# Alexander-H-Liu/End-to-end-ASR-Pytorch

Measured on AMD Instinct MI355X. Metric: audio frames/sec training (LAS+CTC, LibriSpeech 80-mel), higher is better.
Workload: dtype f32; 1 GPU; cfg3: {"B": 32, "T": 1600, "D": 80, "V": 5000, "L": 64}; global_batch=32, parallelism=dp1

## Files before the change

### end-to-end-asr-pytorch_amd/_lib.py

```python
import ctypes
import os

_HERE = os.path.dirname(os.path.abspath(__file__))
LIB_PATH = os.path.join(_HERE, "csrc", "libasrk.so")

c_int, c_i64, c_f32, c_vp, c_sz = (ctypes.c_int, ctypes.c_int64, ctypes.c_float, ctypes.c_void_p,
                                   ctypes.c_size_t)
c_f64 = ctypes.c_double

SIGNATURES = {
    "asrk_version": (c_int, []),
    "asrk_strerror": (ctypes.c_char_p, [c_int]),
    "asrk_init": (c_int, [c_int]),
    "asrk_profile_enable": (None, [c_int]),
    "asrk_profile_families": (None, [ctypes.c_uint]),
    "asrk_profile_reset": (None, []),
    "asrk_profile_get": (c_int, [c_int, ctypes.POINTER(ctypes.c_double), ctypes.POINTER(c_i64)]),
    "asrk_profile_get_work": (c_int, [c_int, ctypes.POINTER(ctypes.c_double)]),
    "asrk_gemm_f32": (c_int, [c_int, c_int, c_int, c_int, c_int, c_f32, c_vp, c_int, c_vp, c_int,
                              c_f32, c_vp, c_int, c_vp, c_vp, c_int, c_int, c_vp, c_sz, c_vp]),
    "asrk_gemm_ws_bytes": (c_sz, [c_int, c_int, c_int, c_int]),
    "asrk_gemm_takes_split": (c_int, [c_int, c_int, c_int, c_int]),
    "asrk_split_panel_bytes": (ctypes.c_size_t, [c_int, c_int, c_int]),
    "asrk_split_panel_f32": (c_int, [c_vp, c_int, c_int, c_int, c_int, c_vp, c_int, c_vp]),
    "asrk_gemm_panels_f32": (c_int, [c_int, c_int, c_int, c_f32, c_vp, c_int, c_int, c_int, c_int,
                                     c_vp, c_int, c_int, c_int, c_int, c_f32, c_vp, c_int, c_vp, c_vp, c_int, c_vp]),
    "asrk_copy3d_f32": (c_int, [c_vp, c_vp, c_int, c_int, c_int, c_i64, c_i64, c_i64, c_i64, c_int,
                                c_vp]),
    "asrk_colsum_f32": (c_int, [c_vp, c_int, c_int, c_int, c_vp, c_int, c_vp]),
    "asrk_tanh_fwd_f32": (c_int, [c_vp, c_vp, c_i64, c_vp]),
    "asrk_tanh_bwd_f32": (c_int, [c_vp, c_vp, c_vp, c_i64, c_vp]),
    "asrk_log_softmax_fwd_f32": (c_int, [c_vp, c_vp, c_int, c_int, c_int, c_vp]),
    "asrk_log_softmax_bwd_f32": (c_int, [c_vp, c_vp, c_vp, c_int, c_int, c_int, c_vp]),
    "asrk_cross_entropy_fwd_f32": (c_int, [c_vp, c_int, c_int, c_int, c_vp, c_int, c_vp, c_vp, c_vp]),
    "asrk_cross_entropy_bwd_f32": (c_int, [c_vp, c_int, c_int, c_int, c_vp, c_int, c_vp, c_vp, c_vp,
                                           c_vp]),
    "asrk_ctc_prefix_score_f32": (c_int, [c_vp, c_vp, c_vp, c_vp, c_vp, c_vp, c_vp, c_int, c_int, c_int,
                                          c_int, c_int, c_int, c_f32, c_vp]),
    "asrk_ctc_prefix_score_multi_f32": (c_int, [c_vp, c_vp, c_vp, c_vp, c_vp, c_vp, c_vp, c_vp, c_vp, c_int, c_int,
                                                c_int, c_int, c_int, c_int, c_int, c_f32, c_vp]),
    "asrk_ctc_prefix_beam_ws_bytes": (c_sz, [c_int, c_int]),
    "asrk_ctc_prefix_beam_ws_offsets": (c_int, [c_int, c_int, c_int] + [ctypes.POINTER(c_i64)] * 6),
    "asrk_ctc_prefix_beam_f32": (c_int, [c_vp, c_int, c_int, c_vp, c_int, c_int, c_vp, c_f32, c_int, c_int, c_int,
                                         c_int, c_int, c_vp, c_sz, c_vp]),
    "asrk_fbank_frames_f32": (c_int, [c_vp, c_i64, c_vp, c_vp, c_int, c_int, c_int, c_int, c_f32, c_int,
                                      c_vp]),
    "asrk_power_spectrum_f32": (c_int, [c_vp, c_vp, c_i64, c_int, c_vp]),
    "asrk_log_floor_f32": (c_int, [c_vp, c_i64, c_f32, c_vp]),
    "asrk_delta_f32": (c_int, [c_vp, c_vp, c_vp, c_int, c_int, c_int, c_int, c_vp]),
    "asrk_cmvn_f32": (c_int, [c_vp, c_vp, c_int, c_int, c_f32, c_vp]),
    "asrk_transpose_f32": (c_int, [c_vp, c_vp, c_int, c_int, c_vp]),
    "asrk_fbank_frames_batch_f32": (c_int, [c_vp, c_int, c_i64, c_vp, c_vp, c_int, c_int, c_vp, c_vp, c_int, c_int,
                                            c_int, c_f32, c_f32, c_int, c_vp]),
    "asrk_delta_cmvn_batch_f32": (c_int, [c_vp, c_vp, c_int, c_int, c_vp, c_int, c_int, c_int, c_f32, c_vp, c_int,
                                          c_vp]),
    "asrk_fbank_logmel_batch_f32": (c_int, [c_vp, c_int, c_i64, c_vp, c_vp, c_int, c_int, c_vp, c_vp, c_vp, c_vp, c_vp,
                                            c_int, c_int, c_vp, c_int, c_int, c_int, c_f32, c_f32, c_int, c_f32, c_vp]),
    "asrk_lstm_ws_bytes": (c_sz, []),
    "asrk_lstm_xchg_bytes": (c_sz, [c_int, c_int, c_int, c_int, c_int, c_int]),
    "asrk_lstm_plan_workgroups": (c_int, [c_int, c_int, c_int, c_int, c_int, c_int]),
    "asrk_lstm_rec_fwd_f32": (c_int, [c_vp, c_vp, c_vp, c_vp, c_vp, c_int, c_int, c_int, c_int,
                                      c_vp, c_int, c_vp, c_int, c_vp]),
    "asrk_lstm_rec_bwd_f32": (c_int, [c_vp, c_vp, c_vp, c_vp, c_vp, c_int, c_int, c_int, c_int,
                                      c_vp, c_int, c_vp, c_vp, c_int, c_vp]),
    "asrk_lstm_rec_fwd_pyr_f32": (c_int, [c_vp, c_vp, c_vp, c_vp, c_vp, c_int, c_int, c_int, c_int,
                                          c_vp, c_int, c_vp, c_vp, c_int, c_int, c_int, c_vp]),
    "asrk_lstm_rec_fwd_len_f32": (c_int, [c_vp, c_vp, c_vp, c_vp, c_vp, c_vp, c_int, c_int, c_int, c_int,
                                          c_vp, c_int, c_vp, c_vp, c_int, c_int, c_int, c_vp]),
    "asrk_lstm_rec_bwd_pyr_f32": (c_int, [c_vp, c_vp, c_vp, c_vp, c_vp, c_int, c_int, c_int, c_int,
                                          c_vp, c_int, c_vp, c_vp, c_int, c_int, c_int, c_vp]),
    "asrk_lstm_plan_is_bf": (c_int, [c_int, c_int, c_int, c_int, c_int, c_int]),
    "asrk_lstm_rec_fwd_pyr_panel_f32": (c_int, [c_vp, c_vp, c_vp, c_vp, c_vp, c_int, c_int, c_int, c_int,
                                                c_vp, c_int, c_vp, c_vp, c_int, c_int, c_vp, c_int, c_vp]),
    "asrk_lstm_rec_bwd_pyr_panel_f32": (c_int, [c_vp, c_vp, c_vp, c_vp, c_vp, c_int, c_int, c_int, c_int,
                                                c_vp, c_int, c_vp, c_vp, c_int, c_int, c_vp, c_vp, c_int, c_vp]),
    "asrk_gru_rec_fwd_f32": (c_int, [c_vp, c_vp, c_vp, c_vp, c_int, c_int, c_int, c_int,
                                     c_vp, c_int, c_vp, c_vp, c_int, c_int, c_int, c_vp]),
    "asrk_gru_rec_bwd_f32": (c_int, [c_vp, c_vp, c_vp, c_vp, c_vp, c_int, c_int, c_int, c_int,
                                     c_vp, c_int, c_vp, c_vp, c_int, c_int, c_int, c_vp]),
    "asrk_lstm_check_error": (c_int, [c_vp, c_vp]),
    "asrk_loc_conv_fwd_f32": (c_int, [c_vp, c_vp, c_vp, c_int, c_int, c_int, c_int, c_int, c_vp]),
    "asrk_loc_conv_bwd_f32": (c_int, [c_vp, c_vp, c_vp, c_vp, c_vp, c_int, c_int, c_int, c_int, c_int,
                                      c_vp]),
    "asrk_attn_energy_fwd_f32": (c_int, [c_int, c_vp, c_vp, c_vp, c_vp, c_vp, c_vp, c_vp, c_vp, c_vp,
                                         c_int, c_int, c_int, c_int, c_int, c_f32, c_vp]),
    "asrk_attn_energy_bwd_f32": (c_int, [c_int, c_vp, c_vp, c_vp, c_vp, c_vp, c_vp, c_vp, c_vp, c_vp,
                                         c_vp, c_vp, c_vp, c_vp, c_vp, c_int, c_int, c_int, c_int,
                                         c_int, c_f32, c_vp]),
    "asrk_attn_context_fwd_f32": (c_int, [c_vp, c_vp, c_vp, c_int, c_int, c_int, c_i64, c_vp]),
    "asrk_attn_context_bwd_f32": (c_int, [c_vp, c_vp, c_vp, c_int, c_int, c_int, c_i64, c_vp]),
    "asrk_lstm_cell_fwd_f32": (c_int, [c_vp, c_vp, c_vp, c_vp, c_int, c_int, c_vp]),
    "asrk_lstm_cell_bwd_f32": (c_int, [c_vp, c_vp, c_vp, c_vp, c_vp, c_vp, c_int, c_int, c_vp]),
    "asrk_gru_cell_fwd_f32": (c_int, [c_vp, c_vp, c_i64, c_i64, c_vp, c_i64, c_vp, c_i64, c_int, c_int, c_vp]),
    "asrk_gru_cell_bwd_f32": (c_int, [c_vp, c_vp, c_i64, c_i64, c_vp, c_i64, c_vp, c_i64, c_vp, c_vp, c_i64,
                                      c_int, c_int, c_vp]),
    "asrk_embedding_fwd_f32": (c_int, [c_vp, c_vp, c_vp, c_i64, c_int, c_int, c_vp]),
    "asrk_embedding_bwd_f32": (c_int, [c_vp, c_vp, c_vp, c_i64, c_int, c_int, c_vp]),
    "asrk_layer_norm_fwd_f32": (c_int, [c_vp, c_vp, c_vp, c_vp, c_vp, c_vp, c_int, c_int, c_f32, c_vp]),
    "asrk_layer_norm_bwd_f32": (c_int, [c_vp, c_vp, c_vp, c_vp, c_vp, c_vp, c_vp, c_vp, c_int, c_int,
                                        c_vp]),
    "asrk_dropout_f32": (c_int, [c_vp, c_vp, c_i64, c_f32, ctypes.c_uint64, ctypes.c_uint64, c_vp]),
    "asrk_adadelta_step_f32": (c_int, [c_vp, c_vp, c_vp, c_vp, c_i64, c_f64, c_f64, c_f64, c_vp, c_vp]),
    "asrk_adadelta_multi_f32": (c_int, [c_int, c_vp, c_vp, c_vp, c_vp, c_vp, c_f64, c_f64, c_f64, c_vp, c_vp]),
    "asrk_adam_multi_f32": (c_int, [c_int, c_vp, c_vp, c_vp, c_vp, c_vp, c_f64, c_f64, c_f64, c_f64, c_i64,
                                    c_vp, c_vp]),
    "asrk_adam_step_f32": (c_int, [c_vp, c_vp, c_vp, c_vp, c_i64, c_f64, c_f64, c_f64, c_f64, c_i64, c_vp,
                                   c_vp]),
    "asrk_token_crop_i64": (c_int, [c_vp, c_i64, c_int, c_int, c_i64, c_i64, c_int, c_vp, c_i64, c_vp, c_vp]),
    "asrk_edit_distance_i64": (c_int, [c_vp, c_i64, c_vp, c_vp, c_i64, c_vp, c_int, c_int, c_vp, c_vp]),
    "asrk_grad_norm_ws_bytes": (c_sz, [c_int, c_vp]),
    "asrk_grad_norm_multi_f32": (c_int, [c_int, c_vp, c_vp, c_f32, c_vp, c_vp, c_vp, c_sz, c_vp]),
    "asrk_fill_f32": (c_int, [c_vp, c_i64, c_f32, c_vp]),
    "asrk_topk_f32": (c_int, [c_vp, c_int, c_int, c_int, c_int, c_vp, c_vp, c_vp]),
    "asrk_beam_select_f32": (c_int, [c_vp] * 4 + [c_int] * 6 + [c_vp] * 19 + [c_vp]),
    "asrk_gather_rows_multi_f32": (c_int, [c_int, c_vp, c_vp, c_vp, c_vp, c_vp, c_vp, c_vp, c_int, c_vp]),
    "asrk_conv_out_size": (c_int, [c_int, c_int, c_int, c_int]),
    "asrk_im2col_f32": (c_int, [c_vp, c_vp] + [c_int] * 10 + [c_i64] * 4 + [c_vp]),
    "asrk_im2col_ld_f32": (c_int, [c_vp, c_vp] + [c_int] * 11 + [c_i64] * 4 + [c_vp]),
    "asrk_col2im_f32": (c_int, [c_vp, c_vp] + [c_int] * 10 + [c_i64] * 4 + [c_vp]),
    "asrk_im2col_cl_f32": (c_int, [c_vp, c_vp] + [c_int] * 10 + [c_i64] * 4 + [c_vp]),
    "asrk_col2im_cl_f32": (c_int, [c_vp, c_vp] + [c_int] * 10 + [c_i64] * 4 + [c_vp]),
    "asrk_conv_weight_reorder_f32": (c_int, [c_vp, c_vp, c_int, c_int, c_int, c_int, c_vp]),
    "asrk_conv3x3_supported": (c_int, [c_int] * 4),
    "asrk_conv3x3_weight_f32": (c_int, [c_vp, c_vp, c_int, c_int, c_int, c_vp]),
    "asrk_conv3x3_f32": (c_int, [c_vp] * 5 + [c_int] * 6 + [c_vp]),
    "asrk_conv3x3_wgrad_ws_bytes": (c_sz, [c_int] * 5),
    "asrk_conv3x3_wgrad_f32": (c_int, [c_vp] * 5 + [c_int] * 5 + [c_vp, c_sz, c_vp]),
    "asrk_conv3x3_first_supported": (c_int, [c_int] * 4),
    "asrk_conv3x3_first_f32": (c_int, [c_vp] * 4 + [c_int] * 5 + [c_i64] * 4 + [c_int, c_vp]),
    "asrk_conv3x3_first_wgrad_ws_bytes": (c_sz, [c_int] * 5),
    "asrk_conv3x3_first_wgrad_f32": (c_int, [c_vp] * 5 + [c_int] * 5 + [c_i64] * 4 + [c_vp, c_sz, c_vp]),
    "asrk_relu_fwd_f32": (c_int, [c_vp, c_i64, c_vp]),
    "asrk_relu_bwd_f32": (c_int, [c_vp, c_vp, c_vp, c_i64, c_vp]),
    "asrk_maxpool2x2_fwd_f32": (c_int, [c_vp, c_vp, c_vp] + [c_int] * 4 + [c_i64] * 4 + [c_vp]),
    "asrk_maxpool2x2_bwd_f32": (c_int, [c_vp, c_vp, c_vp] + [c_int] * 4 + [c_i64] * 4 + [c_vp]),
    "asrk_speller_plan": (c_int, [c_vp, ctypes.POINTER(c_int), ctypes.POINTER(c_int)]),
    "asrk_speller_fwd_f32": (c_int, [c_vp, c_vp]),
    "asrk_speller_bwd_f32": (c_int, [c_vp, c_vp, c_vp]),
    "asrk_speller_step_f32": (c_int, [c_vp, c_int, c_vp, c_i64, c_vp, c_vp]),
    "asrk_speller_dvalue_f32": (c_int, [c_vp, c_i64, c_i64, c_vp, c_i64, c_i64, c_vp, c_int, c_int, c_int,
                                        c_int, c_vp]),
    "asrk_joint_score_f32": (c_int, [c_vp, c_vp, c_vp, c_vp, c_vp, c_vp, c_int, c_int, c_int, c_f64, c_f64,
                                     c_f64, c_vp]),
    "asrk_lstm_cell_fused_f32": (c_int, [c_vp, c_i64, c_int, c_vp, c_vp, c_vp, c_vp, c_vp, c_vp, c_vp, c_vp, c_int,
                                         c_int, c_vp]),
    "asrk_transpose_ld_f32": (c_int, [c_vp, c_i64, c_vp, c_i64, c_int, c_int, c_vp]),
    "asrk_flac_info": (c_int, [ctypes.c_char_p, ctypes.POINTER(c_int), ctypes.POINTER(c_int), ctypes.POINTER(c_int),
                               ctypes.POINTER(c_i64), c_vp]),
    "asrk_flac_decode_i32": (c_int, [ctypes.c_char_p, c_vp, c_i64, ctypes.POINTER(c_i64)]),
    "asrk_ctc_loss_fwd_f32": (c_int, [c_vp, c_i64, c_i64, c_int, c_int, c_int, c_vp, c_i64, c_int,
                                      c_vp, c_vp, c_int, c_vp, c_vp, c_vp, c_vp, c_vp]),
    "asrk_ctc_loss_bwd_f32": (c_int, [c_vp, c_i64, c_i64, c_int, c_int, c_int, c_vp, c_i64, c_int,
                                      c_vp, c_vp, c_int, c_vp, c_vp, c_vp, c_vp, c_vp, c_vp, c_i64,
                                      c_i64, c_vp]),
}

_lib = None


class AsrkError(RuntimeError):
    pass


def load():
    global _lib
    if _lib is not None:
        return _lib
    if not os.path.exists(LIB_PATH):
        raise AsrkError(
            "libasrk.so not found at %s - build it with `python __graft_entry__.py` "
            "(hipcc --offload-arch=gfx950). There is no CPU fallback for the product path." % LIB_PATH)
    try:
        import torch
    except ImportError:
        pass
    lib = ctypes.CDLL(LIB_PATH)
    for name, (res, args) in SIGNATURES.items():
        fn = getattr(lib, name)
        fn.restype = res
        fn.argtypes = args
    _lib = lib
    return lib


def strerror(rc):
    return load().asrk_strerror(int(rc)).decode()


def check(rc, what=""):
    if rc != 0:
        raise AsrkError("%s failed: %s (rc=%d)" % (what or "asrk call", strerror(rc), rc))
```

### end-to-end-asr-pytorch_amd/csrc/gemm_split.hip

```cpp
#include "common.h"
#include "knobs.h"
#include <algorithm>

extern "C" int asrk_cu_count_(void);

namespace {

typedef __bf16 bf16x8 __attribute__((ext_vector_type(8)));

constexpr int PIECE = 1024;

struct SplitGemmArgs {
    const unsigned char *Ap, *Bp;
    float *C;
    const float *bias, *bias2;
    int M, N, ldc;
    int KC;
    size_t rb_stride_a, rb_stride_b;
    int nk;
    int tiles_m, tiles_n;
    float alpha, beta;
};

__device__ __forceinline__ void split8(const float (&v)[8], u32x4 (&w)[3]) {
    unsigned h[3][8];
#pragma unroll
    for (int e = 0; e < 8; ++e) {
        const float a = v[e];
        const __bf16 b0 = (__bf16)a;
        const float r1 = a - (float)b0;
        const __bf16 b1 = (__bf16)r1;
        const float r2 = r1 - (float)b1;
        const __bf16 b2 = (__bf16)r2;
        h[0][e] = __builtin_bit_cast(unsigned short, b0);
        h[1][e] = __builtin_bit_cast(unsigned short, b1);
        h[2][e] = __builtin_bit_cast(unsigned short, b2);
    }
#pragma unroll
    for (int p = 0; p < 3; ++p)
#pragma unroll
        for (int q = 0; q < 4; ++q) w[p][q] = h[p][2 * q] | (h[p][2 * q + 1] << 16);
}

template <bool VEC>
__global__ __launch_bounds__(256) void split_panel_kernel(const float *__restrict__ src, int ld, int R, int K,
                                                          unsigned char *__restrict__ dst, int KC, int RB,
                                                          size_t rb_stride) {
    constexpr int CHUNK = 3 * PIECE;
    const int lane = threadIdx.x & 63;
    const int KG = KC >> 2;
    const int64_t item = (int64_t)blockIdx.x * 4 + (threadIdx.x >> 6);
    if (item >= (int64_t)RB * KG) return;
    const int rb = (int)(item / KG), c0 = (int)(item - (int64_t)rb * KG) * 4;
    unsigned char *drb = dst + (size_t)rb * rb_stride;
    const int c = c0 + (lane & 3), k0 = c * 8;
#pragma unroll
    for (int it = 0; it < 4; ++it) {
        const int rl = it * 16 + (lane >> 2), row = rb * 64 + rl;
        float v[8];
        const float *s = src + (size_t)row * ld + k0;
        if (VEC && row < R && k0 + 8 <= K) {
            const f32x4 lo = *reinterpret_cast<const f32x4 *>(s), hi = *reinterpret_cast<const f32x4 *>(s + 4);
            v[0] = lo[0]; v[1] = lo[1]; v[2] = lo[2]; v[3] = lo[3];
            v[4] = hi[0]; v[5] = hi[1]; v[6] = hi[2]; v[7] = hi[3];
        } else {
#pragma unroll
            for (int e = 0; e < 8; ++e) v[e] = (row < R && k0 + e < K) ? s[e] : 0.f;
        }
        u32x4 w[3];
        split8(v, w);
        unsigned char *d = drb + (size_t)c * CHUNK + rl * 16;
#pragma unroll
        for (int p = 0; p < 3; ++p) *reinterpret_cast<u32x4 *>(d + p * PIECE) = w[p];
    }
}

template <int NCG>
__global__ __launch_bounds__(256) void split_panel_t_kernel(const float *__restrict__ src, int ld, int R, int K,
                                                            unsigned char *__restrict__ dst, int KC, int RB,
                                                            size_t rb_stride) {
    constexpr int CHUNK = 3 * PIECE;
    const int lane = threadIdx.x & 63, wave = __builtin_amdgcn_readfirstlane(threadIdx.x >> 6);
    const int64_t item = (int64_t)blockIdx.x * 4 + wave;
    const int KGn = KC / NCG;
    if (item >= (int64_t)RB * KGn) return;
    const int g = (int)(item / RB), rb = (int)(item - (int64_t)g * RB);
    const int c0 = g * NCG, k0 = c0 * 8, row = rb * 64 + lane;
    float v[NCG][8];
    const float *s = src + (size_t)k0 * ld + row;
    if (k0 + 8 * NCG <= K && rb * 64 + 64 <= R) {
#pragma unroll
        for (int cc = 0; cc < NCG; ++cc)
#pragma unroll
            for (int e = 0; e < 8; ++e) v[cc][e] = s[(size_t)(cc * 8 + e) * ld];
    } else {
#pragma unroll
        for (int cc = 0; cc < NCG; ++cc)
#pragma unroll
            for (int e = 0; e < 8; ++e)
                v[cc][e] = (row < R && k0 + cc * 8 + e < K) ? s[(size_t)(cc * 8 + e) * ld] : 0.f;
    }
    unsigned char *d = dst + (size_t)rb * rb_stride + (size_t)c0 * CHUNK + lane * 16;
#pragma unroll
    for (int cc = 0; cc < NCG; ++cc) {
        u32x4 w[3];
        split8(v[cc], w);
#pragma unroll
        for (int p = 0; p < 3; ++p) *reinterpret_cast<u32x4 *>(d + (size_t)cc * CHUNK + p * PIECE) = w[p];
    }
}

template <int N>
__device__ __forceinline__ void glds16_run(const unsigned char *g, unsigned voff, unsigned char *l) {
    static_assert(N >= 1 && N <= 4, "immediate offset range");
    const auto *gp = (const __attribute__((address_space(1))) unsigned char *)g + voff;
    auto *lp = (__attribute__((address_space(3))) void *)l;
    __builtin_amdgcn_global_load_lds(gp, lp, 16, 0, 0);
    if constexpr (N > 1) __builtin_amdgcn_global_load_lds(gp, lp, 16, PIECE, 0);
    if constexpr (N > 2) __builtin_amdgcn_global_load_lds(gp, lp, 16, 2 * PIECE, 0);
    if constexpr (N > 3) __builtin_amdgcn_global_load_lds(gp, lp, 16, 3 * PIECE, 0);
}

template <int N>
__device__ __forceinline__ void wait_vm() {
    static_assert(N >= 0 && N < 64, "vmcnt is a 6-bit field");
    __builtin_amdgcn_s_waitcnt((N & 15) | 0x70 | 0xF00 | (((N >> 4) & 3) << 14));
}
__device__ __forceinline__ void wait_lgkm0() { __builtin_amdgcn_s_waitcnt(0xC07F); }

template <int NC, int NST, bool SPEC, int WM>
__global__ __launch_bounds__(SPEC ? (WM == 2 ? 512 : 704) : 256) void gemm_bf16x6_kernel(SplitGemmArgs p) {
    extern __shared__ __attribute__((aligned(1024))) unsigned char lds[];
    static_assert(WM == 2 || (WM == 4 && SPEC), "256-row tiles only with DMA waves");
    constexpr int NPL = 3, CHUNK = NPL * PIECE;
    constexpr int NCW = 2 * WM;
    constexpr int NRG = WM + 2;
    constexpr int RPD = WM == 2 ? 1 : 2;
    constexpr int REGION = NC * CHUNK;
    constexpr int STAGE = NRG * REGION;
    constexpr int LPT = NC * NPL * RPD;
    const int tid = threadIdx.x, lane = tid & 63;
    const int wave = __builtin_amdgcn_readfirstlane(tid >> 6);
    const int ntiles = p.tiles_m * p.tiles_n, bid = blockIdx.x;
    const int q8 = ntiles >> 3, r8 = ntiles & 7, xcd = bid & 7, loc = bid >> 3;
    const int tile = (xcd < r8 ? xcd * (q8 + 1) : r8 * (q8 + 1) + (xcd - r8) * q8) + loc;
    constexpr int BAND = 8;
    const int band = tile / (BAND * p.tiles_m);
    const int band_w = min(BAND, p.tiles_n - band * BAND);
    const int in_band = tile - band * BAND * p.tiles_m;
    const int tm = in_band / band_w, tn = band * BAND + in_band % band_w;

    const bool loader = !SPEC || wave >= NCW, worker = !SPEC || wave < NCW;
    const int wr = worker ? wave >> 1 : 0, wc = wave & 1;
    const int ltm = tm, ltn = tn;
    const int r0 = (SPEC ? wave - NCW : wave) * RPD;
    const unsigned char *gsrc[RPD];
#pragma unroll
    for (int q = 0; q < RPD; ++q) {
        const int r = r0 + q;
        gsrc[q] = (r < WM ? p.Ap + (size_t)(ltm * WM + r) * p.rb_stride_a
                          : p.Bp + (size_t)(ltn * 2 + r - WM) * p.rb_stride_b);
    }
    const unsigned voff = lane * 16;
    unsigned char *ldst = lds + r0 * REGION;
    static_assert((NC * NPL) % 4 == 0, "a region is issued as runs of four pieces");
    auto issue = [&](int kt, int stage) {
        unsigned char *l = ldst + stage * STAGE;
#pragma unroll
        for (int q = 0; q < RPD; ++q) {
            const unsigned char *g = gsrc[q] + (size_t)kt * REGION;
#pragma unroll
            for (int j = 0; j < NC * NPL; j += 4) glds16_run<4>(g + j * PIECE, voff, l + q * REGION + j * PIECE);
        }
    };

    f32x16 acc[2][2];
#pragma unroll
    for (int i = 0; i < 2; ++i)
#pragma unroll
        for (int j = 0; j < 2; ++j)
#pragma unroll
            for (int r = 0; r < 16; ++r) acc[i][j][r] = 0.f;

    const int nk = p.nk;
    const int frag_off = ((lane >> 5) * NPL) * PIECE + (lane & 31) * 16;
    const unsigned char *abase = lds + wr * REGION + frag_off;
    const unsigned char *bbase = lds + (WM + wc) * REGION + frag_off;
    constexpr int S = NC / 2;

    bf16x8 fa[2][2][NPL], fb[2][2][NPL];
    auto load_frags = [&](int buf, int stage, int ks) {
        const unsigned char *a_st = abase + stage * STAGE + ks * 2 * NPL * PIECE;
        const unsigned char *b_st = bbase + stage * STAGE + ks * 2 * NPL * PIECE;
#pragma unroll
        for (int i = 0; i < 2; ++i)
#pragma unroll
            for (int pl = 0; pl < NPL; ++pl) {
                fa[buf][i][pl] = *reinterpret_cast<const bf16x8 *>(a_st + pl * PIECE + i * 512);
                fb[buf][i][pl] = *reinterpret_cast<const bf16x8 *>(b_st + pl * PIECE + i * 512);
            }
        __builtin_amdgcn_sched_barrier(0);
    };
    auto step = [&](int buf, bool load, int lstage, int lks) {
        constexpr int NT = 6;
        constexpr int PA[6] = {2, 1, 0, 1, 0, 0};
        constexpr int PB[6] = {0, 1, 2, 0, 1, 0};
        constexpr int RPL[6] = {2, 0, 1, 1, 0, 2};
        const unsigned char *a_st = abase + lstage * STAGE + lks * 2 * NPL * PIECE;
        const unsigned char *b_st = bbase + lstage * STAGE + lks * 2 * NPL * PIECE;
        const int nb = buf ^ 1;
#pragma unroll
        for (int m = 0; m < 4 * NT; ++m) {
            const int t = m >> 2, i = (m >> 1) & 1, j = m & 1;
            acc[i][j] = __builtin_amdgcn_mfma_f32_32x32x16_bf16(fa[buf][i][PA[t]], fb[buf][j][PB[t]], acc[i][j], 0, 0, 0);
            __builtin_amdgcn_sched_barrier(0);
            if (load && m < 4 * NPL) {
                const int g = m >> 1, h = m & 1, pl = RPL[g];
                if ((g & 1) == 0) fa[nb][h][pl] = *reinterpret_cast<const bf16x8 *>(a_st + pl * PIECE + h * 512);
                else fb[nb][h][pl] = *reinterpret_cast<const bf16x8 *>(b_st + pl * PIECE + h * 512);
                __builtin_amdgcn_sched_barrier(0);
            }
        }
    };

    if (loader) {
#pragma unroll
        for (int s = 0; s < NST; ++s)
            if (s < nk) issue(s, s);
        const int later = min(NST - 1, nk - 1);
        if (NST > 3 && later >= 3) wait_vm<(NST > 3 ? 3 * LPT : 0)>();
        else if (NST > 2 && later == 2) wait_vm<(NST > 2 ? 2 * LPT : 0)>();
        else if (later == 1) wait_vm<LPT>();
        else wait_vm<0>();
    }
    __builtin_amdgcn_s_barrier();
    if (SPEC && !worker) {
        int stage = 0;
        for (int kt = 0; kt + 1 < nk; ++kt) {
            const int later = min(NST - 2, nk - 2 - kt);
            if (NST > 3 && later >= 2) wait_vm<(NST > 3 ? 2 * LPT : 0)>();
            else if (NST > 2 && later == 1) wait_vm<(NST > 2 ? LPT : 0)>();
            else wait_vm<0>();
            __builtin_amdgcn_s_barrier();
            if (kt + NST < nk) issue(kt + NST, stage);
            if (++stage == NST) stage = 0;
        }
        return;
    }
    load_frags(0, 0, 0);

    int stage = 0;
    static_assert(S >= 2 && S % 2 == 0, "fragment double buffer assumes an even number of steps per tile");
    for (int kt = 0; kt + 1 < nk; ++kt) {
#pragma unroll
        for (int ks = 0; ks < S - 1; ++ks) {
            wait_lgkm0();
            step(ks & 1, true, stage, ks + 1);
        }
        int nstage = stage + 1;
        if (nstage == NST) nstage = 0;
        const int later = min(NST - 2, nk - 2 - kt);
        wait_lgkm0();
        if (!SPEC) {
            if (NST > 3 && later >= 2) wait_vm<(NST > 3 ? 2 * LPT : 0)>();
            else if (NST > 2 && later == 1) wait_vm<(NST > 2 ? LPT : 0)>();
            else wait_vm<0>();
        }
        __builtin_amdgcn_s_barrier();
        if (!SPEC && kt + NST < nk) issue(kt + NST, stage);
        step((S - 1) & 1, true, nstage, 0);
        stage = nstage;
    }
    {
#pragma unroll
        for (int ks = 0; ks < S - 1; ++ks) {
            wait_lgkm0();
            step(ks & 1, true, stage, ks + 1);
        }
        wait_lgkm0();
        step((S - 1) & 1, false, 0, 0);
    }

    const int row0 = tm * 64 * WM + wr * 64 + 4 * (lane >> 5), col0 = tn * 128 + wc * 64 + (lane & 31);
#pragma unroll
    for (int j = 0; j < 2; ++j) {
        const int col = col0 + j * 32;
        if (col >= p.N) continue;
        float bsum = 0.f;
        if (p.bias) bsum += p.bias[col];
        if (p.bias2) bsum += p.bias2[col];
#pragma unroll
        for (int i = 0; i < 2; ++i)
#pragma unroll
            for (int r = 0; r < 16; ++r) {
                const int row = row0 + i * 32 + (r & 3) + 8 * (r >> 2);
                if (row >= p.M) continue;
                float *c = p.C + (size_t)row * p.ldc + col;
                float v = p.alpha * acc[i][j][r] + bsum;
                if (p.beta != 0.f) v += p.beta * *c;
                *c = v;
            }
    }
}

template <int NST, int NDW>
__global__ __launch_bounds__((4 + NDW) * 64) void gemm_bf16x6_w256_kernel(SplitGemmArgs p, int rb_b, int BAND) {
    extern __shared__ __attribute__((aligned(1024))) unsigned char lds[];
    constexpr int NPL = 3, NC = 2, CHUNK = NPL * PIECE;
    constexpr int REGION = NC * CHUNK;
    constexpr int NRG = 6;
    constexpr int STAGE = NRG * REGION;
    constexpr int LPT = NRG * NC * NPL / NDW;
    static_assert(LPT * NDW == NRG * NC * NPL && (NDW == 3 || NDW == 4), "36 pieces per stage over 3 or 4 DMA waves");
    const int tid = threadIdx.x, lane = tid & 63;
    const int wave = __builtin_amdgcn_readfirstlane(tid >> 6);
    const int ntiles = p.tiles_m * p.tiles_n, bid = blockIdx.x;
    const int q8 = ntiles >> 3, r8 = ntiles & 7, xcd = bid & 7, loc = bid >> 3;
    const int tile = (xcd < r8 ? xcd * (q8 + 1) : r8 * (q8 + 1) + (xcd - r8) * q8) + loc;
    const int band = tile / (BAND * p.tiles_m);
    const int band_w = min(BAND, p.tiles_n - band * BAND);
    const int in_band = tile - band * BAND * p.tiles_m;
    const int tm = in_band / band_w, tn = band * BAND + in_band % band_w;
    const int nk = p.nk;

    if (wave >= 4) {
        const int d = wave - 4, first = d * LPT;
        constexpr int NRUN = LPT / 3;
        static_assert(NRUN * 3 == LPT, "runs of three pieces");
        const unsigned char *run_g[NRUN];
#pragma unroll
        for (int k = 0; k < NRUN; ++k) {
            const int idx = first + 3 * k, r = idx / (NC * NPL), j = idx - r * (NC * NPL);
            run_g[k] = (r < 2 ? p.Ap + (size_t)(tm * 2 + r) * p.rb_stride_a
                              : p.Bp + (size_t)min(tn * 4 + r - 2, rb_b - 1) * p.rb_stride_b) + j * PIECE;
        }
        const unsigned voff = lane * 16;
        unsigned char *ldst = lds + first * PIECE;
        auto issue = [&](int kt, int stage) {
            unsigned char *l = ldst + stage * STAGE;
            const size_t gk = (size_t)kt * REGION;
#pragma unroll
            for (int k = 0; k < NRUN; ++k) glds16_run<3>(run_g[k] + gk, voff, l + 3 * k * PIECE);
        };
#pragma unroll
        for (int s = 0; s < NST; ++s)
            if (s < nk) issue(s, s);
        {
            const int later = min(NST - 2, nk - 2);
            if (later >= 2) wait_vm<2 * LPT>();
            else if (later == 1) wait_vm<LPT>();
            else wait_vm<0>();
        }
        __builtin_amdgcn_s_barrier();
        int stage = 0;
        for (int kt = 0; kt < nk; ++kt) {
            const int later = min(NST - 2, nk - 2 - kt);
            if (later >= 2) wait_vm<2 * LPT>();
            else if (later == 1) wait_vm<LPT>();
            else wait_vm<0>();
            __builtin_amdgcn_s_barrier();
            if (kt + NST < nk) issue(kt + NST, stage);
            if (++stage == NST) stage = 0;
        }
        return;
    }

    const int wr = wave >> 1, wc = wave & 1;
    f32x16 acc[2][4];
#pragma unroll
    for (int i = 0; i < 2; ++i)
#pragma unroll
        for (int j = 0; j < 4; ++j)
#pragma unroll
            for (int r = 0; r < 16; ++r) acc[i][j][r] = 0.f;
    const int frag_off = ((lane >> 5) * NPL) * PIECE + (lane & 31) * 16;
    const unsigned char *abase = lds + wr * REGION + frag_off;
    const unsigned char *bbase = lds + (2 + wc * 2) * REGION + frag_off;
    bf16x8 fa1[2], fa2[2], fb1[4], fb2[4], fa0[2][2], fb0[2][4];
    auto rd_a1 = [&](bf16x8 &dst, int stage, int pl, int i) {
        dst = *reinterpret_cast<const bf16x8 *>(abase + stage * STAGE + pl * PIECE + i * 512);
    };
    auto rd_b1 = [&](bf16x8 &dst, int stage, int pl, int j) {
        dst = *reinterpret_cast<const bf16x8 *>(bbase + stage * STAGE + (j >> 1) * REGION + pl * PIECE + (j & 1) * 512);
    };
    auto rd_a = [&](bf16x8 (&dst)[2], int stage, int pl) {
#pragma unroll
        for (int i = 0; i < 2; ++i) rd_a1(dst[i], stage, pl, i);
    };
    auto rd_b = [&](bf16x8 (&dst)[4], int stage, int pl) {
#pragma unroll
        for (int j = 0; j < 4; ++j) rd_b1(dst[j], stage, pl, j);
    };
#define ASRK_TERM8(FA, FB)                                                                                 \
    do {                                                                                                   \
        _Pragma("unroll") for (int i = 0; i < 2; ++i) _Pragma("unroll") for (int j = 0; j < 4; ++j)         \
            acc[i][j] = __builtin_amdgcn_mfma_f32_32x32x16_bf16(FA[i], FB[j], acc[i][j], 0, 0, 0);          \
        __builtin_amdgcn_sched_barrier(0);                                                                 \
    } while (0)
#define ASRK_TERM8_RD(FA, FB, RD)                                                                          \
    do {                                                                                                   \
        _Pragma("unroll") for (int m = 0; m < 8; ++m) {                                                    \
            acc[m >> 2][m & 3] =                                                                           \
                __builtin_amdgcn_mfma_f32_32x32x16_bf16(FA[m >> 2], FB[m & 3], acc[m >> 2][m & 3], 0, 0, 0); \
            __builtin_amdgcn_sched_barrier(0);                                                             \
            RD(m);                                                                                         \
            __builtin_amdgcn_sched_barrier(0);                                                             \
        }                                                                                                  \
    } while (0)
#define ASRK_STEP(P)                                                                                       \
    do {                                                                                                   \
        int nstage = stage + 1;                                                                            \
        if (nstage == NST) nstage = 0;                                                                     \
        ASRK_TERM8(fa2, fb0[P]);                                                                           \
        wait_lgkm0();                                                                                      \
        __builtin_amdgcn_s_barrier();                                           \
        auto rd2 = [&](int m) {                                                                            \
            if (m == 0) rd_a1(fa2[0], nstage, 2, 0);                                                       \
            else if (m == 2) rd_a1(fa2[1], nstage, 2, 1);                                                  \
            else if (m == 4) rd_b1(fb0[1 - (P)][0], nstage, 0, 0);                                         \
            else if (m == 6) rd_b1(fb0[1 - (P)][1], nstage, 0, 1);                                         \
        };                                                                                                 \
        ASRK_TERM8_RD(fa0[P], fb2, rd2);                                                                   \
        auto rd3 = [&](int m) {                                                                            \
            if ((m & 1) == 0) rd_b1(fb2[m >> 1], nstage, 2, m >> 1);                                       \
        };                                                                                                 \
        ASRK_TERM8_RD(fa0[P], fb1, rd3);                                                                   \
        auto rd4 = [&](int m) {                                                                            \
            if (m == 0) rd_b1(fb0[1 - (P)][2], nstage, 0, 2);                                              \
            else if (m == 2) rd_b1(fb0[1 - (P)][3], nstage, 0, 3);                                         \
            else if (m == 4) rd_a1(fa0[1 - (P)][0], nstage, 0, 0);                                         \
            else if (m == 6) rd_a1(fa0[1 - (P)][1], nstage, 0, 1);                                         \
        };                                                                                                 \
        ASRK_TERM8_RD(fa1, fb1, rd4);                                                                      \
        auto rd5 = [&](int m) {                                                                            \
            if ((m & 1) == 0) rd_b1(fb1[m >> 1], nstage, 1, m >> 1);                                       \
        };                                                                                                 \
        ASRK_TERM8_RD(fa1, fb0[P], rd5);                                                                   \
        auto rd6 = [&](int m) {                                                                            \
            if (m == 1) rd_a1(fa1[0], nstage, 1, 0);                                                       \
            else if (m == 4) rd_a1(fa1[1], nstage, 1, 1);                                                  \
        };                                                                                                 \
        ASRK_TERM8_RD(fa0[P], fb0[P], rd6);                                                                \
        stage = nstage;                                                                                    \
    } while (0)

    __builtin_amdgcn_s_barrier();
    rd_a(fa2, 0, 2); rd_b(fb0[0], 0, 0); rd_a(fa0[0], 0, 0); rd_b(fb2, 0, 2); rd_b(fb1, 0, 1); rd_a(fa1, 0, 1);
    int stage = 0;
    for (int kt = 0; kt < nk; kt += 2) {
        ASRK_STEP(0);
        ASRK_STEP(1);
    }
#undef ASRK_STEP
#undef ASRK_TERM8_RD
#undef ASRK_TERM8

    const int row0 = tm * 128 + wr * 64 + 4 * (lane >> 5), col0 = tn * 256 + wc * 128 + (lane & 31);
#pragma unroll
    for (int j = 0; j < 4; ++j) {
        const int col = col0 + j * 32;
        if (col >= p.N) continue;
        float bsum = 0.f;
        if (p.bias) bsum += p.bias[col];
        if (p.bias2) bsum += p.bias2[col];
#pragma unroll
        for (int i = 0; i < 2; ++i)
#pragma unroll
            for (int r = 0; r < 16; ++r) {
                const int row = row0 + i * 32 + (r & 3) + 8 * (r >> 2);
                if (row >= p.M) continue;
                float *c = p.C + (size_t)row * p.ldc + col;
                float v = p.alpha * acc[i][j][r] + bsum;
                if (p.beta != 0.f) v += p.beta * *c;
                *c = v;
            }
    }
}

template <int NST, int NDW>
int launch_split_gemm_w256(const SplitGemmArgs &a, int rb_b, hipStream_t s) {
    constexpr int lds = NST * 6 * 2 * 3 * PIECE;
    auto kern = gemm_bf16x6_w256_kernel<NST, NDW>;
    static AsrkLdsLatch latch;
    ASRK_HIP(asrk_max_lds_once(latch, reinterpret_cast<const void *>(kern), lds));
    const int band = 2;
    hipLaunchKernelGGL(kern, dim3(a.tiles_m * a.tiles_n), dim3((4 + NDW) * 64), lds, s, a, rb_b, band);
    ASRK_LAUNCH_CHECK();
    return ASRK_OK;
}

template <int NC, int NST, bool SPEC, int WM>
int launch_split_gemm(const SplitGemmArgs &a, hipStream_t s) {
    constexpr int lds = NST * (WM + 2) * NC * 3 * PIECE;
    auto kern = gemm_bf16x6_kernel<NC, NST, SPEC, WM>;
    static AsrkLdsLatch latch;
    ASRK_HIP(asrk_max_lds_once(latch, reinterpret_cast<const void *>(kern), lds));
    hipLaunchKernelGGL(kern, dim3(a.tiles_m * a.tiles_n), dim3(SPEC ? (WM == 2 ? 512 : 704) : 256), lds, s, a);
    ASRK_LAUNCH_CHECK();
    return ASRK_OK;
}

}

namespace {
constexpr int SPLIT_NC = 4;
constexpr int NPL = 3;

struct PanelGeom {
    int KC, rb;
    size_t rb_stride, bytes;
};
PanelGeom panel_geom(int rows, int K, bool slack = false) {
    PanelGeom g;
    g.KC = (asrk_div_up(K, 8 * SPLIT_NC) + (slack ? 1 : 0)) * SPLIT_NC;
    g.rb = asrk_div_up(rows, 128) * 2;
    g.rb_stride = (size_t)g.KC * NPL * PIECE + 4352;
    g.bytes = (size_t)g.rb * g.rb_stride;
    return g;
}

int run_split(const float *src, int ld, int rows, int K, bool trans, unsigned char *dstp, const PanelGeom &g,
              hipStream_t s) {
    const dim3 grid((unsigned)asrk_div_up64((int64_t)g.rb * (g.KC / 4), 4));
    asrk_prof_work_(PROF_SPLIT, 4.0 * (double)rows * (double)K + 6.0 * (double)g.rb * 64.0 * (double)g.KC * 8.0);
    asrk_prof_begin_(PROF_SPLIT, s);
    if (trans) {
        hipLaunchKernelGGL((split_panel_t_kernel<4>), grid, dim3(256), 0, s, src, ld, rows, K, dstp, g.KC, g.rb, g.rb_stride);
    } else {
        const bool vec = (reinterpret_cast<uintptr_t>(src) & 15) == 0 && ld % 4 == 0;
        if (vec) hipLaunchKernelGGL((split_panel_kernel<true>), grid, dim3(256), 0, s, src, ld, rows, K, dstp, g.KC, g.rb, g.rb_stride);
        else hipLaunchKernelGGL((split_panel_kernel<false>), grid, dim3(256), 0, s, src, ld, rows, K, dstp, g.KC, g.rb, g.rb_stride);
    }
    asrk_prof_end_(PROF_SPLIT, s);
    ASRK_LAUNCH_CHECK();
    return ASRK_OK;
}

int run_panel_gemm(int M, int N, int nk, float alpha, const unsigned char *Ap, size_t stride_a,
                   const unsigned char *Bp, size_t stride_b, float beta, float *C, int ldc, const float *bias,
                   const float *bias2, hipStream_t s) {
    const AsrkKnobs &kn = asrk_knobs_();
    SplitGemmArgs a;
    a.Ap = Ap; a.Bp = Bp; a.C = C; a.bias = bias; a.bias2 = bias2;
    a.M = M; a.N = N; a.ldc = ldc; a.KC = 0; a.nk = nk; a.rb_stride_a = stride_a; a.rb_stride_b = stride_b;
    a.tiles_m = asrk_div_up(M, 128); a.tiles_n = asrk_div_up(N, 128);
    a.alpha = alpha; a.beta = beta;
    const int w256 = kn.get(kn.split_w256, 1);
    if (w256 && N >= 512) {
        const int tm = asrk_div_up(M, 128), tn = asrk_div_up(N, 256);
        const int ncu = asrk_cu_count_() > 0 ? asrk_cu_count_() : 256;
        if (w256 == 2 || (long)tm * tn >= 2L * ncu) {
            SplitGemmArgs b = a;
            b.tiles_m = tm; b.tiles_n = tn; b.nk = 2 * nk;
            const long tiles = (long)tm * tn, rem = tiles % ncu;
            const int tm1 = (int)((tiles - rem) / tn);
            if (w256 == 1 && rem > 0 && rem * 10 < 6L * ncu && tm1 > 0 && tm1 < tm && kn.get(kn.split_tail, 1)) {
                b.tiles_m = tm1; b.M = tm1 * 128;
                int rc = launch_split_gemm_w256<4, 4>(b, 2 * asrk_div_up(N, 128), s);
                if (rc != ASRK_OK) return rc;
                SplitGemmArgs c = a;
                c.Ap = a.Ap + (size_t)tm1 * 2 * a.rb_stride_a;
                c.C = a.C + (size_t)tm1 * 128 * ldc;
                c.M = M - tm1 * 128;
                c.tiles_m = asrk_div_up(c.M, 128);
                return launch_split_gemm<4, 3, true, 2>(c, s);
            }
            return launch_split_gemm_w256<4, 4>(b, 2 * asrk_div_up(N, 128), s);
        }
    }
    return launch_split_gemm<4, 3, true, 2>(a, s);
}
}

extern "C" size_t asrk_split_panel_stride_(int rows, int K) { return panel_geom(rows, K, true).rb_stride; }

extern "C" int asrk_gemm_takes_split(int M, int N, int K, int flags) {
    const int mode = flags & 3;
    if (mode == ASRK_GEMM_SPLIT_OFF || mode == 3 || K < 8 || M < 1 || N < 1) return 0;
    if (mode == ASRK_GEMM_SPLIT_AUTO) {
        const double hm = 2.0 * (double)M * (double)N / ((double)M + (double)N);
        const bool shallow_ok = K >= 64 && (double)M * (double)N >= 134217728.0;
        if (hm < 1500.0 || (K < 256 && !shallow_ok) || M < 256 || N < 256) return 0;
    }
    return 1;
}

extern "C" size_t asrk_gemm_ws_bytes(int M, int N, int K, int flags) {
    if (!asrk_gemm_takes_split(M, N, K, flags)) return 0;
    return panel_geom(M, K).bytes + panel_geom(N, K).bytes;
}

extern "C" int asrk_gemm_split_run_(int transA, int transB, int M, int N, int K, float alpha, const float *A,
                                    int lda, const float *B, int ldb, float beta, float *C, int ldc,
                                    const float *bias, const float *bias2, void *wsp, int flags, hipStream_t s) {
    const PanelGeom ga = panel_geom(M, K), gb = panel_geom(N, K);
    unsigned char *ws = reinterpret_cast<unsigned char *>(wsp);
    unsigned char *Ap = ws, *Bp = ws + ga.bytes;
    int rc = run_split(A, lda, M, K, transA != 0, Ap, ga, s);
    if (rc != ASRK_OK) return rc;
    rc = run_split(B, ldb, N, K, transB == 0, Bp, gb, s);
    if (rc != ASRK_OK) return rc;
    return run_panel_gemm(M, N, ga.KC / SPLIT_NC, alpha, Ap, ga.rb_stride, Bp, gb.rb_stride, beta, C, ldc, bias,
                          bias2, s);
}

extern "C" size_t asrk_split_panel_bytes(int rows, int K, int flags) {
    if (rows <= 0 || K <= 0 || flags != 0) return 0;
    return panel_geom(rows, K, true).bytes;
}

extern "C" int asrk_split_panel_f32(const float *src, int ld, int rows, int K, int trans, void *panel, int flags,
                                    void *stream) {
    if (!src || !panel || rows <= 0 || K <= 0 || ld < (trans ? rows : K) || flags != 0) return ASRK_EINVAL;
    if ((reinterpret_cast<uintptr_t>(panel) & 15) != 0) return ASRK_EINVAL;
    asrk_prof_begin_(PROF_GEMM, (hipStream_t)stream);
    const int rc = run_split(src, ld, rows, K, trans != 0, reinterpret_cast<unsigned char *>(panel),
                             panel_geom(rows, K, true), (hipStream_t)stream);
    asrk_prof_end_(PROF_GEMM, (hipStream_t)stream);
    return rc;
}

extern "C" int asrk_gemm_panels_f32(int M, int N, int K, float alpha, const void *A_panel, int a_rows, int a_K,
                                    int a_row0, int a_k0, const void *B_panel, int b_rows, int b_K, int b_row0,
                                    int b_k0, float beta, float *C, int ldc, const float *bias,
                                    const float *bias2, int flags, void *stream) {
    if (M <= 0 || N <= 0 || K <= 0 || !A_panel || !B_panel || !C || ldc < N || flags != 0) return ASRK_EINVAL;
    if (a_row0 < 0 || b_row0 < 0 || a_k0 < 0 || b_k0 < 0 || a_row0 % 128 || b_row0 % 128 || a_k0 % 8 || b_k0 % 8)
        return ASRK_EINVAL;
    if (a_row0 + M > a_rows || b_row0 + N > b_rows || a_k0 + K > a_K || b_k0 + K > b_K) return ASRK_EINVAL;
    if (K % 32 != 0 && a_k0 + K != a_K && b_k0 + K != b_K) return ASRK_ESHAPE;
    const PanelGeom ga = panel_geom(a_rows, a_K, true), gb = panel_geom(b_rows, b_K, true);
    const int nk = asrk_div_up(K, 32);
    if (a_k0 / 8 + nk * SPLIT_NC > ga.KC || b_k0 / 8 + nk * SPLIT_NC > gb.KC) return ASRK_ESHAPE;
    hipStream_t s = (hipStream_t)stream;
    asrk_prof_work_(PROF_GEMM, 2.0 * (double)M * (double)N * (double)K);
    asrk_prof_begin_(PROF_GEMM, s);
    const unsigned char *A0 = reinterpret_cast<const unsigned char *>(A_panel);
    const unsigned char *B0 = reinterpret_cast<const unsigned char *>(B_panel);
    const unsigned char *Ap = A0 + (size_t)(a_row0 / 64) * ga.rb_stride + (size_t)(a_k0 / 8) * NPL * PIECE;
    const unsigned char *Bp = B0 + (size_t)(b_row0 / 64) * gb.rb_stride + (size_t)(b_k0 / 8) * NPL * PIECE;
    const int rc = run_panel_gemm(M, N, nk, alpha, Ap, ga.rb_stride, Bp, gb.rb_stride, beta, C, ldc, bias, bias2, s);
    asrk_prof_end_(PROF_GEMM, s);
    return rc;
}
```

### end-to-end-asr-pytorch_amd/csrc/lstm_rec.hip

```cpp
#include "lstm_rec_common.h"

extern "C" int asrk_cu_count_(void);
extern "C" size_t asrk_split_panel_stride_(int rows, int K);

using namespace asrk_rec;

namespace {

__global__ __launch_bounds__(256) void sentinel_fill_kernel(u32x4 *__restrict__ p, size_t n16) {
    const u32x4 v = {0xFFFFFFFFu, 0xFFFFFFFFu, 0xFFFFFFFFu, 0xFFFFFFFFu};
    for (size_t base = (size_t)blockIdx.x * 1024; base < n16; base += (size_t)gridDim.x * 1024) {
#pragma unroll
        for (int u = 0; u < 4; ++u) {
            const size_t i = base + u * 256 + threadIdx.x;
            if (i < n16) p[i] = v;
        }
    }
}

inline int sentinel_fill(void *xchg, size_t floats, hipStream_t s) {
    const size_t n16 = floats / 4;
    if (n16 * 4 != floats || (reinterpret_cast<uintptr_t>(xchg) & 15) != 0)
        return (int)hipMemsetAsync(xchg, 0xFF, floats * 4, s);
    hipLaunchKernelGGL(sentinel_fill_kernel, dim3(2048), dim3(256), 0, s, reinterpret_cast<u32x4 *>(xchg), n16);
    return (int)hipGetLastError();
}

__global__ __launch_bounds__(256) void sentinel_fill_tail_kernel(u32x4 *__restrict__ x, int groups, int T, int r0,
                                                                 unsigned step16) {
    const u32x4 v = {0xFFFFFFFFu, 0xFFFFFFFFu, 0xFFFFFFFFu, 0xFFFFFFFFu};
    const unsigned n = (unsigned)(T - r0) * step16;
    const int g = blockIdx.y;
    u32x4 *q = x + ((size_t)g * T + r0) * step16;
    for (unsigned i = blockIdx.x * 256 + threadIdx.x; i < n; i += gridDim.x * 256) q[i] = v;
}

inline int sentinel_fill_tail(void *xchg, int groups, int T, size_t step_floats, hipStream_t s) {
    const int r0 = std::max(0, T - 2);
    const unsigned step16 = (unsigned)(step_floats / 4);
    const unsigned n = (unsigned)(T - r0) * step16;
    hipLaunchKernelGGL(sentinel_fill_tail_kernel, dim3(std::max(1u, std::min(64u, (n + 1023) / 1024)), groups), dim3(256),
                       0, s, reinterpret_cast<u32x4 *>(xchg), groups, T, r0, step16);
    return (int)hipGetLastError();
}

inline int canary_words(int nwg) { return ((4 * nwg + 63) / 64) * 64; }

unsigned long long *g_dbg_buf = nullptr;
int g_dbg_steps = 0;

inline void chunk_groups(int ndir, int nbg, int gmax, int &ndir_l, int &nbg_l, int &launches) {
    ndir_l = gmax >= ndir ? ndir : 1;
    nbg_l = std::max(1, std::min(nbg, gmax / ndir_l));
    launches = ((ndir + ndir_l - 1) / ndir_l) * ((nbg + nbg_l - 1) / nbg_l);
}

FwdPlan plan_fwd(int T, int B, int H, int ndir, int ncu, int flags) {
    const AsrkKnobs &kn = asrk_knobs_();
    FwdPlan best{};
    best.ok = false;
    long best_cost = -1;
    const int kg = (H + 15) / 16;
    const int kgw_need = (kg + 3) / 4;
    const int KGW = kgw_need <= 4 ? 4 : kgw_need <= 8 ? 8 : kgw_need <= 16 ? 16 : 0;
    if (!KGW) return best;
    const int HP = KGW * 4 * 16 + 8;
    static const int combos[6][2] = {{1, 1}, {1, 2}, {2, 1}, {2, 2}, {1, 4}, {4, 1}};
    const int oc = 1;
    for (auto &c : combos) {
        const int MT = c[0], NT = c[1];
        if (kn.is_set(kn.fwd_mt) && kn.fwd_mt != MT) continue;
        if (kn.is_set(kn.fwd_nt) && kn.fwd_nt != NT) continue;
        const int U = 4 * MT, BG = 16 * NT;
        const int nwg = (H + U - 1) / U, nbg = (B + BG - 1) / BG;
        const long wgs = (long)ndir * nbg * nwg;
        if (wgs > (long)ncu * oc) continue;
        const size_t red1 = (size_t)4 * MT * NT * RED_PITCH * 16;
        size_t lds = (size_t)MT * 16 * HP * 4 + 2 * red1 + 16;
        int db = 1;
        const size_t lds_cap = (size_t)158 * 1024 / (wgs > ncu ? oc : 1);
        if (lds > lds_cap) {
            lds -= red1;
            db = 0;
        }
        if (lds > lds_cap) continue;
        const long cost = (long)MT * NT * 1000 - nbg;
        if (best_cost < 0 || cost < best_cost) {
            best_cost = cost;
            best = FwdPlan{MT, NT, KGW, U, nwg, nbg, BG, HP, kg, db, lds,
                           (size_t)ndir * nbg * T * ((size_t)kg * NT * 256 + canary_words(nwg)), true,
                           ndir, nbg};
        }
    }
    if (best.ok) {
        const bool no_bf = (flags & ASRK_REC_F32_MFMA) != 0;
        if (!no_bf && best.MT == 2 && (H == 512 || H == 1024)) {
            const size_t wl = (size_t)2 * 2 * (H / 32) * 1024;
            const size_t red1 = (size_t)4 * 2 * best.NT * RED_PITCH * 16;
            size_t lds = wl + 2 * red1 + 16;
            int db = 1;
            if (lds > (size_t)158 * 1024) { lds -= red1; db = 0; }
            if (lds <= (size_t)158 * 1024) {
                best.bf = 1;
                best.db = db;
                best.lds = lds;
                best.xfloats = (size_t)ndir * best.nbg * T *
                               ((size_t)(H / 32) * best.NT * 3 * 256 + canary_words(best.nwg));
            }
            const bool no16 = kn.get(kn.rec_bf_mt4, 1) == 0;
            const int nbg16 = (B + 15) / 16;
            if (best.bf && !no16 && H == 1024 && (long)ndir * nbg16 * (H / 16) <= ncu) {
                best.MT = 4; best.NT = 1; best.U = 16; best.BG = 16;
                best.nwg = H / 16; best.nbg = nbg16; best.ndir_l = ndir; best.nbg_l = nbg16;
                best.db = 0;
                best.lds = (size_t)4 * (H / 32) * 1024 + (size_t)4 * 4 * RED_PITCH * 16 + 16;
                best.xfloats = (size_t)ndir * nbg16 * T * ((size_t)(H / 32) * 3 * 256 + canary_words(best.nwg));
            }
        }
        return best;
    }
    for (auto &c : combos) {
        const int MT = c[0], NT = c[1];
        const int U = 4 * MT, BG = 16 * NT;
        const int nwg = (H + U - 1) / U, nbg = (B + BG - 1) / BG;
        if (nwg > ncu) continue;
        const size_t red1 = (size_t)4 * MT * NT * RED_PITCH * 16;
        size_t lds = (size_t)MT * 16 * HP * 4 + 2 * red1 + 16;
        int db = 1;
        if (lds > (size_t)158 * 1024) { lds -= red1; db = 0; }
        if (lds > (size_t)158 * 1024) continue;
        int ndir_l, nbg_l, launches;
        chunk_groups(ndir, nbg, ncu / nwg, ndir_l, nbg_l, launches);
        const long cost = (long)launches * MT * NT * 1000;
        if (best_cost < 0 || cost < best_cost) {
            best_cost = cost;
            best = FwdPlan{MT, NT, KGW, U, nwg, nbg, BG, HP, kg, db, lds,
                           (size_t)ndir_l * nbg_l * T * ((size_t)kg * NT * 256 + canary_words(nwg)), true,
                           ndir_l, nbg_l};
        }
    }
    return best;
}


inline size_t bwd_lds(int kg, int UB, int NT, int RK, int &HPb, int &KP) {
    const int CH = bwd_ring_kgroups(NT, RK);
    HPb = ((kg - RK + CH - 1) / CH) * CH * 16;
    KP = 4 * HPb + 8;
    return (size_t)UB * KP * 4 + (size_t)HPb * 4 + (size_t)2 * 4 * NT * RED_PITCH * 16 + 16;
}
inline int bwd_rk_options(int kg, int H, int NT, int (&opts)[2]) {
    opts[0] = 0;
    const int kg_plain = (H & 15) ? kg - 1 : kg;
    if (NT == 1 && 32 + bwd_ring_kgroups(1, 32) <= kg_plain) {
        opts[1] = 32;
        return 2;
    }
    return 1;
}

BwdPlan plan_bwd(int T, int B, int H, int ndir, int ncu, int flags) {
    const AsrkKnobs &kn = asrk_knobs_();
    BwdPlan best{};
    best.ok = false;
    const int kg = (H + 15) / 16;
    static const int ubs[3] = {16, 8, 4};
    static const int nts[3] = {1, 2, 4};
    const int oc = 1;
    for (int UB : ubs) {
        if (kn.is_set(kn.bwd_ub) && kn.bwd_ub != UB) continue;
        for (int NT : nts) {
            if (kn.is_set(kn.bwd_nt) && kn.bwd_nt != NT) continue;
            int rks[2];
            const int nrk = bwd_rk_options(kg, H, NT, rks);
            for (int ri = 0; ri < nrk; ++ri) {
                const int RK = rks[ri];
                int HPb, KP;
                const size_t lds = bwd_lds(kg, UB, NT, RK, HPb, KP);
                const int BG = 16 * NT;
                const int nwg = (H + UB - 1) / UB, nbg = (B + BG - 1) / BG;
                const long wgs = (long)ndir * nbg * nwg;
                if (wgs > (long)ncu * oc) continue;
                if (lds > (size_t)158 * 1024 / (wgs > ncu ? oc : 1)) continue;
                best = BwdPlan{NT, UB, nwg, nbg, BG, HPb, KP, kg, lds,
                               (size_t)ndir * nbg * T * ((size_t)4 * kg * NT * 256 + canary_words(nwg)),
                               true, ndir, nbg, RK};
                const bool no_bf = (flags & ASRK_REC_F32_MFMA) != 0;
                if (!no_bf && NT == 1 && UB == 16 && BG == 16 && (H == 512 || H == 1024)) {
                    const int KS = H / 32, KL = H == 1024 ? 11 : 0;
                    best.bf = 1;
                    best.lds = (size_t)4 * KL * 3 * 1024 + (size_t)2 * 4 * RED_PITCH * 16 + 2 * 6144 + 16;
                    best.xfloats = (size_t)ndir * nbg * T * ((size_t)4 * KS * 3 * 256 + canary_words(nwg));
                }
                return best;
            }
        }
    }
    long best_cost = -1;
    for (int UB : ubs) {
        for (int NT : nts) {
            int rks[2];
            const int nrk = bwd_rk_options(kg, H, NT, rks);
            for (int ri = 0; ri < nrk; ++ri) {
                const int RK = rks[ri];
                int HPb, KP;
                const size_t lds = bwd_lds(kg, UB, NT, RK, HPb, KP);
                const int BG = 16 * NT;
                const int nwg = (H + UB - 1) / UB, nbg = (B + BG - 1) / BG;
                if (nwg > ncu || lds > (size_t)158 * 1024) continue;
                int ndir_l, nbg_l, launches;
                chunk_groups(ndir, nbg, ncu / nwg, ndir_l, nbg_l, launches);
                const long cost = (long)launches * NT * 1000 + (16 / UB);
                if (best_cost < 0 || cost < best_cost) {
                    best_cost = cost;
                    best = BwdPlan{NT, UB, nwg, nbg, BG, HPb, KP, kg, lds,
                                   (size_t)ndir_l * nbg_l * T * ((size_t)4 * kg * NT * 256 + canary_words(nwg)),
                                   true, ndir_l, nbg_l, RK};
                }
            }
        }
    }
    return best;
}

int rec_fwd_impl(bool gru, float *G, const float *whh_f, const float *whh_r, float *Y, float *C, int T, int B,
                 int H, int ndir, void *xchg, int xchg_prefilled, void *ws, float *Y2, int pyr_mode,
                 int pyr_rate, int flags, void *stream, const int64_t *lens = nullptr, void *x2_panel = nullptr);
int rec_bwd_impl(bool gru, float *gates, const float *whh_f, const float *whh_r, const float *C,
                 const float *dY, int T, int B, int H, int ndir, void *xchg, int xchg_prefilled, void *ws,
                 float *db, int pyr_mode, int pyr_rate, int flags, void *stream, void *dg_panel = nullptr,
                 void *dgt_panel = nullptr);

}


extern "C" void asrk_lstm_set_debug_(void *buf, int steps) {
    g_dbg_buf = reinterpret_cast<unsigned long long *>(buf);
    g_dbg_steps = steps;
}

extern "C" size_t asrk_lstm_ws_bytes(void) { return WS_WORDS * sizeof(unsigned); }

extern "C" int asrk_lstm_plan_workgroups(int T, int B, int H, int ndir, int backward, int flags) {
    if (flags < 0 || T <= 0 || B <= 0 || H <= 0 || (ndir != 1 && ndir != 2) || H % 4 != 0) return 0;
    const int ncu = asrk_cu_count_();
    if (ncu <= 0) return 0;
    if (backward) {
        BwdPlan pl = plan_bwd(T, B, H, ndir, ncu, flags);
        return pl.ok ? pl.ndir_l * pl.nbg_l * pl.nwg : 0;
    }
    FwdPlan pl = plan_fwd(T, B, H, ndir, ncu, flags);
    return pl.ok ? pl.ndir_l * pl.nbg_l * pl.nwg : 0;
}

extern "C" size_t asrk_lstm_xchg_bytes(int T, int B, int H, int ndir, int backward, int flags) {
    if (flags < 0 || T <= 0 || B <= 0 || H <= 0 || (ndir != 1 && ndir != 2)) return 0;
    const int ncu = asrk_cu_count_();
    if (ncu <= 0) return 0;
    if (backward) {
        BwdPlan pl = plan_bwd(T, B, H, ndir, ncu, flags);
        return pl.ok ? pl.xfloats * 4 : 0;
    }
    FwdPlan pl = plan_fwd(T, B, H, ndir, ncu, flags);
    return pl.ok ? pl.xfloats * 4 : 0;
}

extern "C" int asrk_lstm_rec_fwd_f32(float *G, const float *whh_f, const float *whh_r, float *Y,
                                     float *C, int T, int B, int H, int ndir, void *xchg,
                                     int xchg_prefilled, void *ws, int flags, void *stream) {
    return asrk_lstm_rec_fwd_pyr_f32(G, whh_f, whh_r, Y, C, T, B, H, ndir, xchg, xchg_prefilled, ws, nullptr,
                                     0, 1, flags, stream);
}

extern "C" int asrk_lstm_rec_fwd_pyr_f32(float *G, const float *whh_f, const float *whh_r, float *Y,
                                         float *C, int T, int B, int H, int ndir, void *xchg,
                                         int xchg_prefilled, void *ws, float *Y2, int pyr_mode,
                                         int pyr_rate, int flags, void *stream) {
    if (!C) return ASRK_EINVAL;
    return rec_fwd_impl(false, G, whh_f, whh_r, Y, C, T, B, H, ndir, xchg, xchg_prefilled, ws, Y2, pyr_mode,
                        pyr_rate, flags, stream);
}

extern "C" int asrk_lstm_rec_fwd_pyr_panel_f32(float *G, const float *whh_f, const float *whh_r, float *Y,
                                               float *C, int T, int B, int H, int ndir, void *xchg,
                                               int xchg_prefilled, void *ws, float *Y2, int pyr_mode,
                                               int pyr_rate, void *x2_panel, int flags, void *stream) {
    if (!C || !x2_panel) return ASRK_EINVAL;
    return rec_fwd_impl(false, G, whh_f, whh_r, Y, C, T, B, H, ndir, xchg, xchg_prefilled, ws, Y2, pyr_mode,
                        pyr_rate, flags, stream, nullptr, x2_panel);
}

extern "C" int asrk_lstm_plan_is_bf(int T, int B, int H, int ndir, int backward, int flags) {
    if (flags < 0 || T <= 0 || B <= 0 || H <= 0 || (ndir != 1 && ndir != 2) || H % 4 != 0) return 0;
    const int ncu = asrk_cu_count_();
    if (ncu <= 0) return 0;
    if (backward) {
        BwdPlan pl = plan_bwd(T, B, H, ndir, ncu, flags);
        return pl.ok && pl.bf ? 1 : 0;
    }
    FwdPlan pl = plan_fwd(T, B, H, ndir, ncu, flags);
    return pl.ok && pl.bf ? 1 : 0;
}

extern "C" int asrk_lstm_rec_fwd_len_f32(float *G, const float *whh_f, const float *whh_r, float *Y,
                                         float *C, const int64_t *lens, int T, int B, int H, int ndir, void *xchg,
                                         int xchg_prefilled, void *ws, float *Y2, int pyr_mode,
                                         int pyr_rate, int flags, void *stream) {
    if (!C || !lens) return ASRK_EINVAL;
    return rec_fwd_impl(false, G, whh_f, whh_r, Y, C, T, B, H, ndir, xchg, xchg_prefilled, ws, Y2, pyr_mode,
                        pyr_rate, flags, stream, lens);
}

extern "C" int asrk_gru_rec_fwd_f32(float *G, const float *whh_f, const float *whh_r, float *Y, int T, int B,
                                    int H, int ndir, void *xchg, int xchg_prefilled, void *ws, float *Y2,
                                    int pyr_mode, int pyr_rate, int flags, void *stream) {
    return rec_fwd_impl(true, G, whh_f, whh_r, Y, nullptr, T, B, H, ndir, xchg, xchg_prefilled, ws, Y2,
                        pyr_mode, pyr_rate, flags, stream);
}

extern "C" int asrk_gru_rec_bwd_f32(float *gates, const float *whh_f, const float *whh_r, const float *Y,
                                    const float *dY, int T, int B, int H, int ndir, void *xchg,
                                    int xchg_prefilled, void *ws, float *db, int pyr_mode, int pyr_rate,
                                    int flags, void *stream) {
    return rec_bwd_impl(true, gates, whh_f, whh_r, Y, dY, T, B, H, ndir, xchg, xchg_prefilled, ws, db,
                        pyr_mode, pyr_rate, flags, stream);
}

namespace {
int rec_fwd_impl(bool gru, float *G, const float *whh_f, const float *whh_r, float *Y, float *C, int T, int B,
                 int H, int ndir, void *xchg, int xchg_prefilled, void *ws, float *Y2, int pyr_mode,
                 int pyr_rate, int flags, void *stream, const int64_t *lens, void *x2_panel) {
    const AsrkKnobs &kn = asrk_knobs_();
    if (flags < 0 || pyr_mode < 0 || pyr_mode > 2 || pyr_rate < 1) return ASRK_EINVAL;
    const bool y2_empty = pyr_mode == 1 && T / pyr_rate == 0;
    if (pyr_mode != 0 && !Y2 && !y2_empty) return ASRK_EINVAL;
    if (T < 0 || B <= 0 || H <= 0 || (ndir != 1 && ndir != 2)) return ASRK_EINVAL;
    if (T == 0) return ASRK_OK;
    if (!G || !whh_f || (ndir == 2 && !whh_r) || !Y || (!gru && !C) || !ws || !xchg) return ASRK_EINVAL;
    if (H % 4 != 0) return ASRK_ESHAPE;
    if ((reinterpret_cast<uintptr_t>(xchg) & 15) != 0) return ASRK_EINVAL;
    const int ncu = asrk_cu_count_();
    if (ncu <= 0) return ASRK_EDEVICE;
    FwdPlan pl = plan_fwd(T, B, H, ndir, ncu, flags);
    if (!pl.ok) return ASRK_ESHAPE;
    hipStream_t s = (hipStream_t)stream;
    RecFwdArgs a;
    a.G = G; a.whh[0] = whh_f; a.whh[1] = ndir == 2 ? whh_r : whh_f;
    a.Y = Y; a.C = C; a.X = reinterpret_cast<float *>(xchg);
    a.err = reinterpret_cast<unsigned *>(ws);
    a.T = T; a.B = B; a.H = H; a.ldg = ndir * 4 * H; a.ldy = ndir * H;
    a.U = pl.U; a.nwg = pl.nwg; a.BG = pl.BG; a.HP = pl.HP; a.kgp = pl.kgp;
    a.canw = canary_words(pl.nwg);
    a.poll_mode = kn.get(kn.fwd_poll, 0);
    a.poll_mode |= (kn.get(kn.fwd_presleep, 8) & 0xff) << 8;
    a.dbg = g_dbg_buf; a.dbg_steps = kn.is_set(kn.dbg_noload) ? -1 : g_dbg_steps;
    a.Y2 = pyr_mode ? Y2 : nullptr; a.pyr_mode = pyr_mode; a.pyr_rate = pyr_rate;
    a.lens = lens;
    a.P2 = nullptr; a.p2_stride = 0;
    if (x2_panel) {
        if (!pl.bf || pyr_mode == 2 || lens || (ndir * H) % 8 != 0 || (reinterpret_cast<uintptr_t>(x2_panel) & 15))
            return ASRK_ESHAPE;
        const int r = pyr_mode == 1 ? pyr_rate : 1;
        a.P2 = reinterpret_cast<unsigned char *>(x2_panel);
        a.p2_stride = asrk_split_panel_stride_((T / r) * B, r * ndir * H);
        if (pyr_mode == 0) { a.pyr_rate = 1; }
    }
    const bool one_launch = pl.ndir_l >= ndir && pl.nbg_l >= pl.nbg;
    a.rearm = (flags & ASRK_REC_REARM) && one_launch ? 1 : 0;
    asrk_prof_begin_(PROF_LSTM_FWD, s);
    int rc = ASRK_OK;
    bool first = true;
    for (int d0 = 0; d0 < ndir && rc == ASRK_OK; d0 += pl.ndir_l)
        for (int g0 = 0; g0 < pl.nbg && rc == ASRK_OK; g0 += pl.nbg_l) {
            a.ndir = std::min(pl.ndir_l, ndir - d0);
            a.nbg = std::min(pl.nbg_l, pl.nbg - g0);
            a.dir0 = d0; a.bg0 = g0;
            if (!(first && xchg_prefilled)) { const int frc = sentinel_fill(xchg, pl.xfloats, s); if (frc) return frc; }
            first = false;
            const int grid = a.ndir * a.nbg * pl.nwg;
            rc = pl.bf ? launch_fwd_bf(gru, a, pl, H, grid, s) : launch_fwd_f32(gru, a, pl, grid, s);
        }
    if (rc == ASRK_OK && (flags & ASRK_REC_REARM)) {
        const int frc = a.rearm ? sentinel_fill_tail(xchg, ndir * pl.nbg, T, pl.xfloats / ((size_t)ndir * pl.nbg * T), s)
                                : sentinel_fill(xchg, pl.xfloats, s);
        if (frc) rc = frc;
    }
    asrk_prof_end_(PROF_LSTM_FWD, s);
    return rc;
}
}

extern "C" int asrk_lstm_rec_bwd_f32(float *gates, const float *whh_f, const float *whh_r,
                                     const float *C, const float *dY, int T, int B, int H, int ndir,
                                     void *xchg, int xchg_prefilled, void *ws, float *db, int flags, void *stream) {
    return asrk_lstm_rec_bwd_pyr_f32(gates, whh_f, whh_r, C, dY, T, B, H, ndir, xchg, xchg_prefilled, ws, db,
                                     0, 1, flags, stream);
}

extern "C" int asrk_lstm_rec_bwd_pyr_f32(float *gates, const float *whh_f, const float *whh_r,
                                         const float *C, const float *dY, int T, int B, int H, int ndir,
                                         void *xchg, int xchg_prefilled, void *ws, float *db,
                                         int pyr_mode, int pyr_rate, int flags, void *stream) {
    return rec_bwd_impl(false, gates, whh_f, whh_r, C, dY, T, B, H, ndir, xchg, xchg_prefilled, ws, db,
                        pyr_mode, pyr_rate, flags, stream);
}

extern "C" int asrk_lstm_rec_bwd_pyr_panel_f32(float *gates, const float *whh_f, const float *whh_r,
                                               const float *C, const float *dY, int T, int B, int H, int ndir,
                                               void *xchg, int xchg_prefilled, void *ws, float *db,
                                               int pyr_mode, int pyr_rate, void *dg_panel, void *dgt_panel, int flags,
                                               void *stream) {
    if (!dg_panel && !dgt_panel) return ASRK_EINVAL;
    return rec_bwd_impl(false, gates, whh_f, whh_r, C, dY, T, B, H, ndir, xchg, xchg_prefilled, ws, db,
                        pyr_mode, pyr_rate, flags, stream, dg_panel, dgt_panel);
}

namespace {
int rec_bwd_impl(bool gru, float *gates, const float *whh_f, const float *whh_r, const float *C,
                 const float *dY, int T, int B, int H, int ndir, void *xchg, int xchg_prefilled, void *ws,
                 float *db, int pyr_mode, int pyr_rate, int flags, void *stream, void *dg_panel, void *dgt_panel) {
    const AsrkKnobs &kn = asrk_knobs_();
    if (flags < 0 || pyr_mode < 0 || pyr_mode > 2 || pyr_rate < 1) return ASRK_EINVAL;
    const bool dy_empty = pyr_mode == 1 && T / pyr_rate == 0;
    if (T < 0 || B <= 0 || H <= 0 || (ndir != 1 && ndir != 2)) return ASRK_EINVAL;
    if (T == 0) return ASRK_OK;
    if (!gates || !whh_f || (ndir == 2 && !whh_r) || !C || (!dY && !dy_empty) || !ws || !xchg) return ASRK_EINVAL;
    if (H % 4 != 0) return ASRK_ESHAPE;
    if ((reinterpret_cast<uintptr_t>(xchg) & 15) != 0) return ASRK_EINVAL;
    const int ncu = asrk_cu_count_();
    if (ncu <= 0) return ASRK_EDEVICE;
    BwdPlan pl = plan_bwd(T, B, H, ndir, ncu, flags);
    if (!pl.ok) return ASRK_ESHAPE;
    hipStream_t s = (hipStream_t)stream;
    RecBwdArgs a;
    a.G = gates; a.whh[0] = whh_f; a.whh[1] = ndir == 2 ? whh_r : whh_f;
    a.C = C; a.dY = dY; a.X = reinterpret_cast<float *>(xchg);
    a.err = reinterpret_cast<unsigned *>(ws);
    a.T = T; a.B = B; a.H = H; a.ldg = ndir * 4 * H; a.ldy = ndir * H;
    a.UB = pl.UB; a.nwg = pl.nwg; a.BG = pl.BG; a.HPb = pl.HPb; a.KP = pl.KP;
    a.kgp = pl.kgp; a.canw = canary_words(pl.nwg);
    a.poll_mode = kn.get(kn.bwd_poll, 1);
    if (kn.is_set(kn.bwd_presleep)) a.poll_mode |= (kn.bwd_presleep & 0xff) << 8;
    a.dbg = g_dbg_buf; a.dbg_steps = kn.is_set(kn.dbg_noload) ? -1 : g_dbg_steps;
    a.db = db;
    a.pyr_mode = pyr_mode; a.pyr_rate = pyr_rate;
    a.PG = nullptr; a.pg_stride = 0;
    if (dg_panel) {
        if (!pl.bf || gru || (reinterpret_cast<uintptr_t>(dg_panel) & 15)) return ASRK_ESHAPE;
        a.PG = reinterpret_cast<unsigned char *>(dg_panel);
        a.pg_stride = asrk_split_panel_stride_(T * B, ndir * 4 * H);
    }
    a.PT = nullptr; a.pt_stride = 0;
    if (dgt_panel) {
        if (!pl.bf || gru || B % 16 != 0 || (reinterpret_cast<uintptr_t>(dgt_panel) & 15)) return ASRK_ESHAPE;
        a.PT = reinterpret_cast<unsigned char *>(dgt_panel);
        a.pt_stride = asrk_split_panel_stride_(ndir * 4 * H, T * B);
    }
    const bool one_launch = pl.ndir_l >= ndir && pl.nbg_l >= pl.nbg;
    a.rearm = (flags & ASRK_REC_REARM) && one_launch ? 1 : 0;
    if (db) ASRK_HIP(hipMemsetAsync(db, 0, (size_t)ndir * 4 * H * sizeof(float), s));
    asrk_prof_begin_(PROF_LSTM_BWD, s);
    int rc = ASRK_OK;
    bool first = true;
    for (int d0 = 0; d0 < ndir && rc == ASRK_OK; d0 += pl.ndir_l)
        for (int g0 = 0; g0 < pl.nbg && rc == ASRK_OK; g0 += pl.nbg_l) {
            a.ndir = std::min(pl.ndir_l, ndir - d0);
            a.nbg = std::min(pl.nbg_l, pl.nbg - g0);
            a.dir0 = d0; a.bg0 = g0;
            if (!(first && xchg_prefilled)) { const int frc = sentinel_fill(xchg, pl.xfloats, s); if (frc) return frc; }
            first = false;
            const int grid = a.ndir * a.nbg * pl.nwg;
            rc = pl.bf ? launch_bwd_bf(gru, a, pl, grid, s) : launch_bwd_f32(gru, a, pl, grid, s);
        }
    if (rc == ASRK_OK && (flags & ASRK_REC_REARM)) {
        const int frc = a.rearm ? sentinel_fill_tail(xchg, ndir * pl.nbg, T, pl.xfloats / ((size_t)ndir * pl.nbg * T), s)
                                : sentinel_fill(xchg, pl.xfloats, s);
        if (frc) rc = frc;
    }
    asrk_prof_end_(PROF_LSTM_BWD, s);
    return rc;
}
}

extern "C" int asrk_lstm_check_error(void *ws, void *stream) {
    if (!ws) return ASRK_EINVAL;
    hipStream_t s = (hipStream_t)stream;
    unsigned e = 0;
    unsigned *errp = reinterpret_cast<unsigned *>(ws);
    ASRK_HIP(hipMemcpyAsync(&e, errp, sizeof(unsigned), hipMemcpyDeviceToHost, s));
    ASRK_HIP(hipStreamSynchronize(s));
    if (e != 0) {
        ASRK_HIP(hipMemsetAsync(errp, 0, sizeof(unsigned), s));
        return ASRK_ETIMEOUT;
    }
    return ASRK_OK;
}
```

### end-to-end-asr-pytorch_amd/csrc/lstm_rec_bwd_bf.hip

```cpp
#include "lstm_rec_common.h"

namespace asrk_rec {
namespace {

template <bool GRU, int KS, int NREG>
__global__ __launch_bounds__(256) void lstm_rec_bwd_bf_kernel(RecBwdArgs p) {
    extern __shared__ __attribute__((aligned(16))) float smem[];
    constexpr int CH = 8;
    constexpr int KL = KS - NREG;
    static_assert(KS >= CH, "ring longer than the slice");
    const int tid = threadIdx.x, lane = tid & 63, wave = __builtin_amdgcn_readfirstlane(tid >> 6);
    const int ngroups = p.ndir * p.nbg;
    const int group = blockIdx.x % ngroups, wg = blockIdx.x / ngroups;
    const int dir = p.dir0 + group % p.ndir, bg = p.bg0 + group / p.ndir;
    const int u0 = wg * 16, b0 = bg * 16;
    const int nb = min(16, p.B - b0);
    const int H = p.H;

    unsigned char *Wl = reinterpret_cast<unsigned char *>(smem);
    f32x4 *red = reinterpret_cast<f32x4 *>(Wl + (size_t)4 * KL * 3 * 1024);
    unsigned char *stage = reinterpret_cast<unsigned char *>(red + 2 * 4 * RED_PITCH);
    unsigned char *stage_t = stage + 4 * 3 * 2 * 16 * 16;
    int *abort_flag = reinterpret_cast<int *>(stage_t + 4 * 3 * 2 * 16 * 16);

    const int m16 = lane & 15, q4 = lane >> 4;
    bf16x8_t areg[NREG > 0 ? NREG : 1][3];
    {
        const float *W = p.whh[dir];
        const bool live = !GRU || wave < 3;
#pragma unroll
        for (int js = 0; js < KS; ++js) {
            unsigned h0[8], h1[8], h2[8];
#pragma unroll
            for (int e = 0; e < 8; ++e) {
                const int j = js * 32 + q4 * 8 + e;
                split3(live ? W[((size_t)wave * H + j) * H + u0 + m16] : 0.f, h0[e], h1[e], h2[e]);
            }
            u32x4 w0, w1, w2;
#pragma unroll
            for (int q = 0; q < 4; ++q) {
                w0[q] = h0[2 * q] | (h0[2 * q + 1] << 16);
                w1[q] = h1[2 * q] | (h1[2 * q + 1] << 16);
                w2[q] = h2[2 * q] | (h2[2 * q + 1] << 16);
            }
            if (js < NREG) {
                areg[js][0] = __builtin_bit_cast(bf16x8_t, w0);
                areg[js][1] = __builtin_bit_cast(bf16x8_t, w1);
                areg[js][2] = __builtin_bit_cast(bf16x8_t, w2);
            } else {
                unsigned char *d = Wl + ((size_t)((wave * KL + (js - NREG)) * 3) * 64 + lane) * 16;
                *reinterpret_cast<u32x4 *>(d) = w0;
                *reinterpret_cast<u32x4 *>(d + 1024) = w1;
                *reinterpret_cast<u32x4 *>(d + 2048) = w2;
            }
        }
        if (tid == 0) *abort_flag = 0;
    }
    __syncthreads();
    const unsigned char *a_lds = Wl + ((size_t)(wave * KL * 3) * 64 + lane) * 16;

    const int ul = tid & 15, bl = tid >> 4;
    const int c_unit = u0 + ul, c_b = b0 + bl;
    const bool c_valid = bl < nb;
    const int c_red = (red_slot((ul >> 2) * 16 + bl)) * 4 + (ul & 3);
    float dc_carry = 0.f;
    float dbsum[4] = {0.f, 0.f, 0.f, 0.f};

    const size_t gate_floats = (size_t)KS * 3 * 256;
    const size_t data_floats = 4 * gate_floats;
    const size_t step_floats = data_floats + (size_t)p.canw;
    float *xgroup = p.X + (size_t)group * p.T * step_floats;
    const unsigned voff = (m16 < nb && p.dbg_steps != -1) ? (unsigned)(lane * 16) : 0x7ff00000u;
    const unsigned gate_base = (unsigned)(wave * gate_floats * 4);
    unsigned char *st_w = stage + (ul >> 3) * 256 + bl * 16 + (ul & 7) * 2;
    unsigned char *st_t = stage_t + (bl >> 3) * 256 + ul * 16 + (bl & 7) * 2;
    int pt_src[2];
    size_t pt_dst[2];
    int pt_half[2];
    bool pt_on[2];
#pragma unroll
    for (int i = 0; i < 2; ++i) {
        const int idx = tid + 256 * i;
        const int u = idx & 15, rest = idx >> 4, hb = rest & 1, gp = rest >> 1;
        const int r = gp / 3, pl = gp - r * 3;
        pt_on[i] = idx < 384;
        pt_src[i] = ((gp * 2 + hb) * 16 + u) * 16;
        const int row = (dir * 4 + r) * H + u0 + u;
        pt_dst[i] = (size_t)(row >> 6) * p.pt_stride + (size_t)pl * 1024 + (row & 63) * 16;
        pt_half[i] = hb;
    }
    const int xks = u0 >> 5, xq4 = (u0 & 31) >> 3;
    int ch_src[2], pg_row[2];
    unsigned ch_dst[2];
    size_t pg_col[2];
    bool ch_on[2];
#pragma unroll
    for (int i = 0; i < 2; ++i) {
        const int idx = lane + 64 * i;
        const int nl = idx / 24, c = idx - nl * 24, n = wave * 4 + nl;
        const int r = c / 6, pl = (c % 6) >> 1, half = c & 1;
        ch_on[i] = idx < 96 && n < nb;
        ch_src[i] = ((r * 3 + pl) * 2 + half) * 256 + n * 16;
        ch_dst[i] = (unsigned)((((r * KS + xks) * 3 + pl) * 64 + (xq4 + half) * 16 + n) * 16);
        pg_row[i] = b0 + n;
        pg_col[i] = (size_t)((((dir * 4 + r) * H + u0 + half * 8) >> 3) * 3 + pl) * 1024;
    }

    for (int s = 0; s < p.T; ++s) {
        const int t = dir == 0 ? p.T - 1 - s : s;
        const int tp = dir == 0 ? t - 1 : t + 1;

        float vi = 0.f, vf = 0.f, vg = 0.f, vo = 0.f, vc = 0.f, vcp = 0.f, vdy = 0.f;
        if (c_valid) {
            const size_t row = (size_t)t * p.B + c_b;
            const float *g = p.G + row * p.ldg + dir * 4 * H + c_unit;
            vi = g[0];
            vf = g[(size_t)H];
            vg = g[(size_t)2 * H];
            vo = g[(size_t)3 * H];
            vc = p.C[row * p.ldy + dir * H + c_unit];
            if (p.pyr_mode == 0) {
                vdy = p.dY[row * p.ldy + dir * H + c_unit];
            } else {
                const int r = p.pyr_rate, tq = t / r, tr = t - tq * r;
                if (p.pyr_mode == 1 ? tq < p.T / r : tr == 0) {
                    const size_t ld2 = p.pyr_mode == 1 ? (size_t)r * p.ldy : (size_t)p.ldy;
                    const size_t off = p.pyr_mode == 1 ? (size_t)tr * p.ldy : 0;
                    vdy = p.dY[((size_t)tq * p.B + c_b) * ld2 + off + dir * H + c_unit];
                }
            }
            if (tp >= 0 && tp < p.T) vcp = p.C[((size_t)tp * p.B + c_b) * p.ldy + dir * H + c_unit];
        }

        f32x4 acc[3];
        acc[0] = acc[1] = acc[2] = f32x4{0.f, 0.f, 0.f, 0.f};

        auto mfma6 = [&](const bf16x8_t (&a)[3], const u32x4 (&b)[3]) {
            acc[0] = __builtin_amdgcn_mfma_f32_16x16x32_bf16(a[2], __builtin_bit_cast(bf16x8_t, b[0]), acc[0], 0, 0, 0);
            acc[1] = __builtin_amdgcn_mfma_f32_16x16x32_bf16(a[1], __builtin_bit_cast(bf16x8_t, b[1]), acc[1], 0, 0, 0);
            acc[2] = __builtin_amdgcn_mfma_f32_16x16x32_bf16(a[0], __builtin_bit_cast(bf16x8_t, b[2]), acc[2], 0, 0, 0);
            acc[0] = __builtin_amdgcn_mfma_f32_16x16x32_bf16(a[1], __builtin_bit_cast(bf16x8_t, b[0]), acc[0], 0, 0, 0);
            acc[1] = __builtin_amdgcn_mfma_f32_16x16x32_bf16(a[0], __builtin_bit_cast(bf16x8_t, b[1]), acc[1], 0, 0, 0);
            acc[2] = __builtin_amdgcn_mfma_f32_16x16x32_bf16(a[0], __builtin_bit_cast(bf16x8_t, b[0]), acc[2], 0, 0, 0);
        };
        auto a_frag = [&](bf16x8_t (&a)[3], int js) {
            if (js < NREG) {
                a[0] = areg[js][0]; a[1] = areg[js][1]; a[2] = areg[js][2];
            } else {
                const unsigned char *q = a_lds + (size_t)(js - NREG) * 3 * 1024;
                a[0] = *reinterpret_cast<const bf16x8_t *>(q);
                a[1] = *reinterpret_cast<const bf16x8_t *>(q + 1024);
                a[2] = *reinterpret_cast<const bf16x8_t *>(q + 2048);
            }
        };

        REC_STAMP(0);
        if (s > 0) {
            __amdgpu_buffer_rsrc_t rs = __builtin_amdgcn_make_buffer_rsrc(
                (void *)(xgroup + (size_t)(s - 1) * step_floats), 0, (int)(step_floats * 4), 0x00020000);
            u32x4 bf[CH][3];
            unsigned spins = 0;
            unsigned long long t0 = 0;
            bool ok = true;
            for (int z = (p.poll_mode >> 8) & 0xff; z > 0; z -= 8) __builtin_amdgcn_s_sleep(8);
            ok = wait_canaries(reinterpret_cast<const unsigned *>(
                                   xgroup + (size_t)(s - 1) * step_floats + data_floats),
                               4 * p.nwg, p.err, lane, p.poll_mode);
            REC_STAMP(7);
            bool bad = false;
            if (ok) {
#pragma unroll
                for (int c = 0; c < CH; ++c)
#pragma unroll
                    for (int pl = 0; pl < 3; ++pl)
                        bf[c][pl] = __builtin_amdgcn_raw_buffer_load_b128(
                            rs, voff, gate_base + (unsigned)((c * 3 + pl) * 1024), 0);
                __builtin_amdgcn_sched_barrier(0);
                REC_STAMP(1);
#pragma unroll
                for (int js = 0; js < KS; ++js) {
                    bf16x8_t a[3];
                    a_frag(a, js);
                    mfma6(a, bf[js % CH]);
                    __builtin_amdgcn_sched_barrier(0);
                    if (js + CH < KS) {
#pragma unroll
                        for (int pl = 0; pl < 3; ++pl)
                            bf[js % CH][pl] = __builtin_amdgcn_raw_buffer_load_b128(
                                rs, voff, gate_base + (unsigned)(((js + CH) * 3 + pl) * 1024), 0);
                        __builtin_amdgcn_sched_barrier(0);
                    }
                }
            }
            bad = any_nan(acc[0] + acc[1] + acc[2]);
            if (ok && __any(bad)) {
                acc[0] = acc[1] = acc[2] = f32x4{0.f, 0.f, 0.f, 0.f};
#pragma unroll
                for (int c0 = 0; c0 < KS; c0 += CH) {
                    while (ok) {
#pragma unroll
                        for (int c = 0; c < CH; ++c)
#pragma unroll
                            for (int pl = 0; pl < 3; ++pl)
                                bf[c][pl] = __builtin_amdgcn_raw_buffer_load_b128(
                                    rs, voff, gate_base + (unsigned)(((c0 + c) * 3 + pl) * 1024), 16);
                        __builtin_amdgcn_sched_barrier(0);
                        bool b2 = false;
#pragma unroll
                        for (int c = 0; c < CH; ++c)
#pragma unroll
                            for (int pl = 0; pl < 3; ++pl) b2 |= has_sentinel(__builtin_bit_cast(f32x4, bf[c][pl]));
                        if (!__any(b2)) break;
                        if (!spin_ok(spins, t0, p.err, lane)) ok = false;
                    }
                    if (ok) {
#pragma unroll
                        for (int c = 0; c < CH; ++c) {
                            bf16x8_t a[3];
                            a_frag(a, c0 + c);
                            mfma6(a, bf[c]);
                        }
                    }
                }
            }
            if (!ok && lane == 0) *abort_flag = 1;
        }
        REC_STAMP(2);
        f32x4 *redw = red + (s & 1) * 4 * RED_PITCH;
        redw[wave * RED_PITCH + red_slot(lane)] = acc[0] + acc[1] + acc[2];
        REC_STAMP(3);
        __syncthreads();
        if (*abort_flag) break;
        REC_STAMP(4);

        const float *redf = reinterpret_cast<const float *>(redw);
        float *xstep = xgroup + (size_t)s * step_floats;
        float dgs[4] = {0.f, 0.f, 0.f, 0.f}, xg[4] = {0.f, 0.f, 0.f, 0.f};
        if (c_valid) {
            float rec = 0.f;
#pragma unroll
            for (int w = 0; w < 4; ++w) rec += redf[w * RED_PITCH * 4 + c_red];
            if (GRU) {
                const float dh = vdy + rec + dc_carry;
                const float r = vi, z = vf, n = vg, hn = vo, hp = vcp;
                const float dn = dh * (1.f - z) * (1.f - n * n);
                const float dz = dh * (hp - n) * z * (1.f - z);
                const float dr = dn * hn * r * (1.f - r);
                dc_carry = dh * z;
                dgs[0] = dr; dgs[1] = dz; dgs[2] = dn; dgs[3] = dn * r;
                xg[0] = dr; xg[1] = dz; xg[2] = dn * r; xg[3] = 0.f;
            } else {
                const float dh = vdy + rec;
                const float tc = fast_tanh(vc);
                const float dcell = dh * vo * (1.f - tc * tc) + dc_carry;
                dc_carry = dcell * vf;
                dgs[0] = dcell * vg * vi * (1.f - vi);
                dgs[1] = dcell * vcp * vf * (1.f - vf);
                dgs[2] = dcell * vi * (1.f - vg * vg);
                dgs[3] = dh * tc * vo * (1.f - vo);
#pragma unroll
                for (int r = 0; r < 4; ++r) xg[r] = dgs[r];
            }
#pragma unroll
            for (int r = 0; r < 4; ++r) dbsum[r] += dgs[r];
        }
#pragma unroll
        for (int r = 0; r < 4; ++r) {
            unsigned h0, h1, h2;
            split3(xg[r], h0, h1, h2);
            *reinterpret_cast<unsigned short *>(st_w + (r * 3 + 0) * 512) = (unsigned short)h0;
            *reinterpret_cast<unsigned short *>(st_w + (r * 3 + 1) * 512) = (unsigned short)h1;
            *reinterpret_cast<unsigned short *>(st_w + (r * 3 + 2) * 512) = (unsigned short)h2;
            if (!GRU && p.PT) {
                *reinterpret_cast<unsigned short *>(st_t + (r * 3 + 0) * 512) = (unsigned short)h0;
                *reinterpret_cast<unsigned short *>(st_t + (r * 3 + 1) * 512) = (unsigned short)h1;
                *reinterpret_cast<unsigned short *>(st_t + (r * 3 + 2) * 512) = (unsigned short)h2;
            }
        }
        __builtin_amdgcn_fence(__ATOMIC_RELEASE, "wavefront");
        __builtin_amdgcn_wave_barrier();
        __builtin_amdgcn_fence(__ATOMIC_ACQUIRE, "wavefront");
        {
            __amdgpu_buffer_rsrc_t xrs = __builtin_amdgcn_make_buffer_rsrc(
                (void *)xstep, 0, (int)(step_floats * 4), 0x00020000);
            u32x4 v[2];
#pragma unroll
            for (int i = 0; i < 2; ++i)
                if (ch_on[i]) {
                    v[i] = *reinterpret_cast<const u32x4 *>(stage + ch_src[i]);
                    __builtin_amdgcn_raw_buffer_store_b128(v[i], xrs, ch_dst[i], 0, 16);
                }
            if (lane == 0)
                __hip_atomic_store(reinterpret_cast<unsigned *>(xstep + data_floats) + 4 * wg + wave,
                                   (unsigned)(s + 1), RLX_AGENT);
            if (!GRU && p.PG) {
#pragma unroll
                for (int i = 0; i < 2; ++i)
                    if (ch_on[i]) {
                        const int m = t * p.B + pg_row[i];
                        *reinterpret_cast<u32x4 *>(p.PG + (size_t)(m >> 6) * p.pg_stride + pg_col[i] + (m & 63) * 16) = v[i];
                    }
            }
        }
        REC_STAMP(5);
        if (c_valid) {
            float *g = p.G + ((size_t)t * p.B + c_b) * p.ldg + dir * 4 * H + c_unit;
#pragma unroll
            for (int r = 0; r < 4; ++r) g[(size_t)r * H] = dgs[r];
        }
        if (!GRU && p.PT) {
            __syncthreads();
#pragma unroll
            for (int i = 0; i < 2; ++i)
                if (pt_on[i]) {
                    const int c = (t * p.B + b0 + pt_half[i] * 8) >> 3;
                    *reinterpret_cast<u32x4 *>(p.PT + pt_dst[i] + (size_t)c * 3072) =
                        *reinterpret_cast<const u32x4 *>(stage_t + pt_src[i]);
                }
        }
        if (p.rearm && s >= 2)
            rearm_region(xgroup + (size_t)(s - 2) * step_floats, step_floats, wg, p.nwg, tid, (int)blockDim.x);
        REC_STAMP(6);
    }
    if (p.db && !*abort_flag) {
        __syncthreads();
        float *sdb = reinterpret_cast<float *>(red);
#pragma unroll
        for (int r = 0; r < 4; ++r) sdb[tid * 4 + r] = c_valid ? dbsum[r] : 0.f;
        __syncthreads();
        if (tid < 64) {
            const int u = tid & 15, r = tid >> 4;
            float a = 0.f;
            for (int b = 0; b < 16; ++b) a += sdb[(b * 16 + u) * 4 + r];
            unsafeAtomicAdd(p.db + (size_t)dir * 4 * H + (size_t)r * H + u0 + u, a);
        }
    }
}

template <bool GRU, int KS, int NREG>
int launch_bwd_bf(const RecBwdArgs &a, int grid, size_t lds, hipStream_t s) {
    auto kern = lstm_rec_bwd_bf_kernel<GRU, KS, NREG>;
    ASRK_HIP(hipFuncSetAttribute(reinterpret_cast<const void *>(kern),
                                 hipFuncAttributeMaxDynamicSharedMemorySize, (int)lds));
    hipLaunchKernelGGL(kern, dim3(grid), dim3(256), lds, s, a);
    ASRK_LAUNCH_CHECK();
    return ASRK_OK;
}

}

int launch_bwd_bf(bool gru, const RecBwdArgs &a, const BwdPlan &pl, int grid, hipStream_t s) {
    if (a.H == 1024) return gru ? launch_bwd_bf<true, 32, 21>(a, grid, pl.lds, s) : launch_bwd_bf<false, 32, 21>(a, grid, pl.lds, s);
    return gru ? launch_bwd_bf<true, 16, 16>(a, grid, pl.lds, s) : launch_bwd_bf<false, 16, 16>(a, grid, pl.lds, s);
}

}
```

### end-to-end-asr-pytorch_amd/csrc/lstm_rec_common.h

```cpp
#pragma once
#include "common.h"
#include "knobs.h"
#include <algorithm>
#include <cstdlib>

namespace asrk_rec {

constexpr int WS_WORDS = 1024;
constexpr unsigned SENT = 0xFFFFFFFFu;
constexpr unsigned long long TIMEOUT_TICKS = 300000000ull;

struct RecFwdArgs {
    float *G;
    const float *whh[2];
    float *Y, *C;
    float *X;
    unsigned *err;
    int T, B, H, ndir, ldg, ldy;
    int U, nwg, nbg, BG, HP, kgp, canw, poll_mode;
    int dir0, bg0;
    unsigned long long *dbg;
    int dbg_steps;
    float *Y2;
    int pyr_mode, pyr_rate;
    const int64_t *lens;
    int rearm;
    unsigned char *P2;
    size_t p2_stride;
};

struct RecBwdArgs {
    float *G;
    const float *whh[2];
    const float *C, *dY;
    float *X;
    unsigned *err;
    int T, B, H, ndir, ldg, ldy;
    int UB, nwg, nbg, BG, HPb, KP, kgp, canw, poll_mode;
    int dir0, bg0;
    unsigned long long *dbg;
    int dbg_steps;
    float *db;
    int pyr_mode, pyr_rate;
    int rearm;
    unsigned char *PG;
    size_t pg_stride;
    unsigned char *PT;
    size_t pt_stride;
};

#define REC_STAMP_W(ph)                                                                       \
    do {                                                                                      \
        if (p.dbg && blockIdx.x == 0 && lane == 0 && s < p.dbg_steps && wave < 4)             \
            p.dbg[((size_t)s * 4 + wave) * 8 + (ph)] = __builtin_readcyclecounter();          \
    } while (0)
#define REC_STAMP(ph)                                                                         \
    do {                                                                                      \
        if (p.dbg && blockIdx.x == 0 && lane == 0 && s < p.dbg_steps)                         \
            p.dbg[((size_t)s * 4 + wave) * 8 + (ph)] = __builtin_readcyclecounter();          \
    } while (0)

__device__ __forceinline__ bool has_sentinel(const f32x4 &v) {
    const u32x4 u = __builtin_bit_cast(u32x4, v);
    return (u[0] == SENT) | (u[1] == SENT) | (u[2] == SENT) | (u[3] == SENT);
}

__device__ __forceinline__ bool any_nan(const f32x4 &v) {
    return (v[0] != v[0]) | (v[1] != v[1]) | (v[2] != v[2]) | (v[3] != v[3]);
}

__device__ __forceinline__ bool spin_ok(unsigned &spins, unsigned long long &t0, unsigned *err,
                                        int lane) {
    __builtin_amdgcn_s_sleep(1);
    if ((++spins & 127u) == 0) {
        const unsigned long long now = wall_clock64();
        if (t0 == 0) t0 = now;
        const unsigned e = __hip_atomic_load(err, RLX_AGENT);
        if (e != 0 || now - t0 > TIMEOUT_TICKS) {
            if (lane == 0) __hip_atomic_store(err, 1u, RLX_AGENT);
            return false;
        }
    }
    return true;
}

__device__ __forceinline__ bool wait_canaries(const unsigned *cb, int cnt, unsigned *err, int lane,
                                              int mode) {
    const bool pipelined = mode & 1;
    unsigned spins = 0;
    unsigned long long t0 = 0;
    if (cnt > 128 || !pipelined) {
        for (;;) {
            bool good = true;
            for (int j = lane; j < cnt; j += 64) good &= (__hip_atomic_load(cb + j, RLX_AGENT) != SENT);
            if (__all(good)) return true;
            if (!spin_ok(spins, t0, err, lane)) return false;
        }
    }
    const bool a0 = lane < cnt, a1 = lane + 64 < cnt;
    const unsigned *p0 = cb + (a0 ? lane : 0), *p1 = cb + (a1 ? lane + 64 : 0);
    unsigned x0 = a0 ? __hip_atomic_load(p0, RLX_AGENT) : 0u, y0 = a1 ? __hip_atomic_load(p1, RLX_AGENT) : 0u;
    __builtin_amdgcn_s_sleep(3);
    unsigned x1 = a0 ? __hip_atomic_load(p0, RLX_AGENT) : 0u, y1 = a1 ? __hip_atomic_load(p1, RLX_AGENT) : 0u;
    __builtin_amdgcn_s_sleep(3);
    unsigned x2 = a0 ? __hip_atomic_load(p0, RLX_AGENT) : 0u, y2 = a1 ? __hip_atomic_load(p1, RLX_AGENT) : 0u;
    for (;;) {
        const bool good = (x0 != SENT) & (y0 != SENT);
        if (__all(good)) return true;
        x0 = x1; y0 = y1; x1 = x2; y1 = y2;
        if (!spin_ok(spins, t0, err, lane)) return false;
        __builtin_amdgcn_s_sleep(2);
        x2 = a0 ? __hip_atomic_load(p0, RLX_AGENT) : 0u;
        y2 = a1 ? __hip_atomic_load(p1, RLX_AGENT) : 0u;
    }
}

__host__ __device__ constexpr int bwd_ring_kgroups(int NT, int RK = 0) { return NT == 1 ? 8 : 16 / NT; }


__device__ __forceinline__ void rearm_region(float *region, size_t floats, int wg, int nwg, int tid, int nthreads) {
    const unsigned n16 = (unsigned)(floats >> 2);
    const unsigned per = (n16 + (unsigned)nwg - 1u) / (unsigned)nwg;
    const unsigned lo = (unsigned)wg * per, hi = min(lo + per, n16);
    u32x4 *q = reinterpret_cast<u32x4 *>(region);
    const u32x4 v = {SENT, SENT, SENT, SENT};
    for (unsigned i = lo + (unsigned)tid; i < hi; i += (unsigned)nthreads) q[i] = v;
}

__device__ __forceinline__ float fast_sigmoid(float x) {
    return __builtin_amdgcn_rcpf(1.0f + __expf(-x));
}
__device__ __forceinline__ float fast_tanh(float x) {
    return 1.0f - 2.0f * __builtin_amdgcn_rcpf(__expf(2.0f * x) + 1.0f);
}

constexpr int RED_PITCH = 72;
__device__ __forceinline__ int red_slot(int lane) { return lane + 2 * (lane >> 4); }

template <int ACC>
__device__ __forceinline__ f32x4 acc_sum(const f32x4 (&a)[ACC]) {
    f32x4 r = a[0];
#pragma unroll
    for (int i = 1; i < ACC; ++i) r += a[i];
    return r;
}


typedef __bf16 bf16x8_t __attribute__((ext_vector_type(8)));
typedef unsigned int u32x2 __attribute__((ext_vector_type(2)));

__device__ __forceinline__ void split3(float a, unsigned &b0, unsigned &b1, unsigned &b2) {
    const __bf16 h0 = (__bf16)a;
    const float r1 = a - (float)h0;
    const __bf16 h1 = (__bf16)r1;
    const __bf16 h2 = (__bf16)(r1 - (float)h1);
    b0 = __builtin_bit_cast(unsigned short, h0);
    b1 = __builtin_bit_cast(unsigned short, h1);
    b2 = __builtin_bit_cast(unsigned short, h2);
}

struct FwdPlan {
    int MT, NT, KGW, U, nwg, nbg, BG, HP, kgp, db;
    size_t lds, xfloats;
    bool ok;
    int ndir_l, nbg_l;
    int bf;
};


struct BwdPlan {
    int NT, UB, nwg, nbg, BG, HPb, KP, kgp;
    size_t lds, xfloats;
    bool ok;
    int ndir_l, nbg_l;
    int RK;
    int bf;
};


int launch_fwd_f32(bool gru, const RecFwdArgs &a, const FwdPlan &pl, int grid, hipStream_t s);
int launch_fwd_bf(bool gru, const RecFwdArgs &a, const FwdPlan &pl, int H, int grid, hipStream_t s);
int launch_bwd_f32(bool gru, const RecBwdArgs &a, const BwdPlan &pl, int grid, hipStream_t s);
int launch_bwd_bf(bool gru, const RecBwdArgs &a, const BwdPlan &pl, int grid, hipStream_t s);

}
```

### end-to-end-asr-pytorch_amd/ops.py

```python
import ctypes

import torch
from torch.autograd import Function

from . import _lib

_ws_cache = {}


def _L():
    return _lib.load()


def _require_gpu(t):
    if not t.is_cuda:
        raise _lib.AsrkError("asrk ops need tensors on the MI355X (got %s); the product path has no "
                             "CPU fallback" % t.device)


def _p(t):
    return ctypes.c_void_p(t.data_ptr()) if t is not None else ctypes.c_void_p(0)


_raw_stream = getattr(torch._C, "_cuda_getCurrentRawStream", None)
_raw_device = getattr(torch._C, "_cuda_getDevice", None)


def _stream():
    if _raw_stream is not None and _raw_device is not None:
        return ctypes.c_void_p(_raw_stream(_raw_device()))
    return ctypes.c_void_p(torch.cuda.current_stream().cuda_stream)


def _f32c(t):
    if t.dtype != torch.float32:
        t = t.float()
    return t if t.is_contiguous() else t.contiguous()


def lstm_workspace(device):
    key = (device.type, device.index if device.index is not None else torch.cuda.current_device())
    ws = _ws_cache.get(key)
    if ws is None:
        ws = torch.zeros(int(_L().asrk_lstm_ws_bytes()), dtype=torch.uint8, device=device)
        _ws_cache[key] = ws
    return ws


import os as _os
_GEMM_SPLIT_FLAG = {0: 1, 1: 0, 2: 2}
_gemm_state = {"split": max(0, min(2, int(_os.environ.get("ASRK_GEMM_SPLIT", "1")))), "lds_hint": 0}


def set_gemm_split(mode):
    _gemm_state["split"] = max(0, min(2, int(mode)))


def get_gemm_split():
    return _gemm_state["split"]


def gemm_flags():
    return _GEMM_SPLIT_FLAG[_gemm_state["split"]] | ((_gemm_state["lds_hint"] & 0xff) << 8)


def gemm_takes_split(M, N, K):
    return bool(_L().asrk_gemm_takes_split(M, N, K, gemm_flags()))


def rec_flags(backward):
    return 1 if _os.environ.get("ASRK_REC_BF_BWD" if backward else "ASRK_REC_BF", "1") == "0" else 0


ASRK_REC_REARM = 2
_XCHG_REARM = _os.environ.get("ASRK_XCHG_REARM", "1") != "0"
_XCHG_POOL_CAP = int(float(_os.environ.get("ASRK_XCHG_POOL_GB", "24")) * (1 << 30))
_xchg_pool = {"free": {}, "bytes": 0, "tick": 0, "stats": {"hit": 0, "miss": 0, "evicted": 0}}


def _size_class(n):
    if n <= 4096:
        return 4096
    q = 1 << (int(n - 1).bit_length() - 3)
    return (n + q - 1) // q * q


def _pool_evict(pool, need):
    while pool["bytes"] + need > _XCHG_POOL_CAP:
        victim = None
        for key, lst in pool["free"].items():
            for i, e in enumerate(lst):
                if victim is None or e[2] < victim[2][2]:
                    victim = (key, i, e)
        if victim is None:
            return
        key, i, e = victim
        pool["free"][key].pop(i)
        pool["bytes"] -= e[0].numel()
        pool["stats"]["evicted"] += 1


class _Exchange:

    __slots__ = ("buf", "prefilled", "flags", "key", "need", "armed")

    def __init__(self, L, T, B, H, ndir, backward, device):
        base = rec_flags(backward)
        n = int(L.asrk_lstm_xchg_bytes(T, B, H, ndir, backward, base))
        if n == 0:
            raise _lib.AsrkError("LSTM shape T=%d B=%d H=%d ndir=%d is not supported by the persistent "
                                 "gfx950 recurrence kernels" % (T, B, H, ndir))
        self.flags = base | (ASRK_REC_REARM if _XCHG_REARM else 0)
        self.need = n
        self.key = (device.index, torch.cuda.current_stream(device).cuda_stream)
        if not _XCHG_REARM:
            self.buf, self.prefilled, self.armed = torch.empty(n, dtype=torch.uint8, device=device), 0, 0
            return
        free = _xchg_pool["free"].get(self.key, ())
        best = None
        for i, e in enumerate(free):
            if e[0].numel() >= n:
                rank = (e[1] < n, e[0].numel())
                if best is None or rank < best[0]:
                    best = (rank, i)
        if best is not None:
            e = free.pop(best[1])
            _xchg_pool["bytes"] -= e[0].numel()
            self.buf, self.armed = e[0], e[1]
        else:
            self.buf, self.armed = torch.empty(_size_class(n), dtype=torch.uint8, device=device), 0
        self.prefilled = 1 if self.armed >= n else 0
        _xchg_pool["stats"]["hit" if self.prefilled else "miss"] += 1

    def done(self):
        if not _XCHG_REARM:
            return
        n = self.buf.numel()
        if n > _XCHG_POOL_CAP:
            return
        _pool_evict(_xchg_pool, n)
        _xchg_pool["tick"] += 1
        _xchg_pool["free"].setdefault(self.key, []).append([self.buf, max(self.armed, self.need), _xchg_pool["tick"]])
        _xchg_pool["bytes"] += n


def drop_exchange_pool():
    _xchg_pool["free"].clear()
    _xchg_pool["bytes"] = 0


def pool_stats():
    return {"exchange": dict(_xchg_pool["stats"], held_bytes=_xchg_pool["bytes"]),
            "panels": dict(_panel_pool["stats"], held_bytes=_panel_pool["bytes"])}


def check_errors(device=None):
    for key, ws in list(_ws_cache.items()):
        rc = _L().asrk_lstm_check_error(_p(ws), _stream())
        if rc != 0:
            drop_exchange_pool()
        _lib.check(rc, "lstm grid sync")


_defer = {"enabled": True, "side": {}, "pending": {}, "cb_armed": False, "release": []}


def set_deferred_weight_grads(flag):
    join_deferred()
    _defer["enabled"] = bool(flag)


def join_deferred():
    for dev, ev in list(_defer["pending"].items()):
        torch.cuda.current_stream(dev).wait_event(ev)
    _defer["pending"].clear()


def deferred_stream(device):
    dev = torch.device(device)
    if dev.index is None:
        dev = torch.device(dev.type, torch.cuda.current_device())
    return _defer["side"].get(dev) if dev in _defer["pending"] else None


def _end_of_backward():
    _defer["cb_armed"] = False
    join_deferred()
    rel, _defer["release"] = _defer["release"], []
    for pnl in rel:
        pnl.release()


def _can_defer(*weights):
    return _defer["enabled"] and all(w is None or (w.is_leaf and w.grad is None) for w in weights)


_BG_FORCED = _os.environ.get("ASRK_SIDE_BG")
_BG_HINT = int(_BG_FORCED) if _BG_FORCED is not None else 0


_gemm_phase_hooks = []


def on_gemm_phase(fn):
    _gemm_phase_hooks.append(fn)
    return fn


def remove_gemm_phase_hook(fn):
    if fn in _gemm_phase_hooks:
        _gemm_phase_hooks.remove(fn)


def _gemm_phase_begins():
    for fn in list(_gemm_phase_hooks):
        fn()


def _defer_beside_bptt():
    return _BG_HINT > 0 or _os.environ.get("ASRK_DEFER_WIDE", "0") == "1"


def _note_bptt_plan(L, T, B, H, ndir):
    global _BG_HINT
    if _BG_FORCED is None:
        wgs = int(L.asrk_lstm_plan_workgroups(T, B, H, ndir, 1, rec_flags(1)))
        cus = torch.cuda.get_device_properties(torch.cuda.current_device()).multi_processor_count
        _BG_HINT = 96 if 0 < 2 * wgs <= cus else 0


class _SideStream:

    def __init__(self, device, inputs, background=True):
        self.device = torch.device(device)
        self.inputs = inputs
        self.hint = _BG_HINT if background else 0

    def __enter__(self):
        dev = self.device
        side = _defer["side"].get(dev)
        if side is None:
            side = torch.cuda.Stream(device=dev)
            _defer["side"][dev] = side
        main = torch.cuda.current_stream(dev)
        ev = torch.cuda.Event()
        ev.record(main)
        side.wait_event(ev)
        for t in self.inputs:
            if t is not None:
                t.record_stream(side)
        self.main, self.side = main, side
        self.ctx = torch.cuda.stream(side)
        self.ctx.__enter__()
        self.prev_hint = _gemm_state["lds_hint"]
        if self.hint:
            _gemm_state["lds_hint"] = self.hint
        return self

    def keep(self, *outs):
        for t in outs:
            if t is not None:
                t.record_stream(self.main)

    def __exit__(self, *exc):
        _gemm_state["lds_hint"] = self.prev_hint
        self.ctx.__exit__(*exc)
        done = torch.cuda.Event()
        done.record(self.side)
        _defer["pending"][self.device] = done
        if not _defer["cb_armed"]:
            try:
                torch.autograd.Variable._execution_engine.queue_callback(_end_of_backward)
                _defer["cb_armed"] = True
            except RuntimeError:
                join_deferred()
        return False


_grad_dest = {"fn": None}


def set_grad_destination(fn):
    _grad_dest["fn"] = fn


def grad_out(weight, shape, device):
    fn = _grad_dest["fn"]
    if fn is not None and weight is not None:
        t = fn(weight, tuple(shape))
        if t is not None:
            return t
    return torch.empty(shape, dtype=torch.float32, device=device)


def grad_has_destination(*weights):
    fn = _grad_dest["fn"]
    return fn is not None and all(w is not None and fn(w, tuple(w.shape)) is not None for w in weights)


def gemm(transA, transB, M, N, K, A, lda, B, ldb, C, ldc, alpha=1.0, beta=0.0, bias=None, bias2=None,
         splitk=0):
    _require_gpu(C)
    ra, ca = (K, M) if transA else (M, K)
    rb, cb = (N, K) if transB else (K, N)
    for name, t, r, c, ld in (("A", A, ra, ca, lda), ("B", B, rb, cb, ldb), ("C", C, M, N, ldc)):
        avail = t.untyped_storage().nbytes() // t.element_size() - t.storage_offset()
        if r > 0 and c > 0 and (ld < c or avail < (r - 1) * ld + c):
            raise _lib.AsrkError("gemm: operand {} ({} elements behind the pointer) too small for {}x{} "
                                 "with ld {}".format(name, avail, r, c, ld))
    L = _L()
    flags = gemm_flags()
    nws = int(L.asrk_gemm_ws_bytes(M, N, K, flags)) if splitk <= 0 else 0
    ws = torch.empty((nws,), dtype=torch.uint8, device=C.device) if nws else None
    _lib.check(L.asrk_gemm_f32(int(transA), int(transB), M, N, K, alpha, _p(A), lda, _p(B), ldb,
                               beta, _p(C), ldc, _p(bias), _p(bias2), splitk, flags, _p(ws), nws, _stream()),
               "gemm")


class SplitPanel:

    def __init__(self, src, ld, rows, K, trans):
        _require_gpu(src)
        L = _L()
        need = (K - 1) * ld + rows if trans else (rows - 1) * ld + K
        avail = src.untyped_storage().nbytes() // src.element_size() - src.storage_offset()
        if ld < (rows if trans else K) or avail < need:
            raise _lib.AsrkError("split panel: source too small for {}x{} (trans={}) with ld {}".format(
                rows, K, trans, ld))
        self.rows, self.K = rows, K
        self.flags = 0
        self.buf = torch.empty((L.asrk_split_panel_bytes(rows, K, self.flags),), dtype=torch.uint8,
                               device=src.device)
        _lib.check(L.asrk_split_panel_f32(_p(src), ld, rows, K, int(trans), _p(self.buf), self.flags, _stream()),
                   "split_panel")


import weakref as _weakref
_REC_PANELS = _os.environ.get("ASRK_REC_PANELS", "1") != "0"
_panel_pool = {"free": {}, "bytes": 0, "tick": 0, "seen": {}, "stats": {"hit": 0, "miss": 0, "skipped": 0, "evicted": 0}}
_panel_state = {"hint": False, "handover": None, "stats": {"emitted": 0, "consumed": 0, "dg": 0}}


class _BlankPanel:
    __slots__ = ("buf", "rows", "K", "flags", "key")

    @staticmethod
    def take(rows, K, device):
        key = (device.index, torch.cuda.current_stream(device).cuda_stream, rows, K)
        free = _panel_pool["free"].get(key)
        if free:
            e = free.pop()
            _panel_pool["bytes"] -= e[0].numel()
            _panel_pool["stats"]["hit"] += 1
            return _BlankPanel(rows, K, key, e[0])
        seen = _panel_pool["seen"]
        if key not in seen:
            if len(seen) > 4096:
                seen.clear()
            seen[key] = 1
            _panel_pool["stats"]["skipped"] += 1
            return None
        _panel_pool["stats"]["miss"] += 1
        n = int(_L().asrk_split_panel_bytes(rows, K, 0))
        buf = torch.empty((n,), dtype=torch.uint8, device=device)
        _lib.check(_L().asrk_fill_f32(_p(buf), n // 4, 0.0, _stream()), "fill")
        return _BlankPanel(rows, K, key, buf)

    def __init__(self, rows, K, key, buf):
        self.rows, self.K, self.flags, self.key, self.buf = rows, K, 0, key, buf

    def release(self):
        n = self.buf.numel()
        if n > _XCHG_POOL_CAP:
            return
        _pool_evict(_panel_pool, n)
        _panel_pool["tick"] += 1
        _panel_pool["free"].setdefault(self.key, []).append([self.buf, 0, _panel_pool["tick"]])
        _panel_pool["bytes"] += n


def set_panel_hint(flag):
    _panel_state["hint"] = bool(flag)


def _take_handover(x):
    h, _panel_state["handover"] = _panel_state["handover"], None
    if h is None:
        return None
    ref, version, panel = h
    if ref() is x and x._version == version and panel.rows == x.shape[0] * x.shape[1] and panel.K == x.shape[2]:
        return panel
    panel.release()
    return None


def gemm_panels(M, N, K, A, a_row0, a_k0, B, b_row0, b_k0, C, ldc, alpha=1.0, beta=0.0, bias=None, bias2=None):
    _require_gpu(C)
    avail = C.untyped_storage().nbytes() // C.element_size() - C.storage_offset()
    if ldc < N or avail < (M - 1) * ldc + N:
        raise _lib.AsrkError("gemm_panels: C too small for {}x{} with ld {}".format(M, N, ldc))
    if A.flags != B.flags:
        raise _lib.AsrkError("gemm_panels: the two panels were built in different layouts")
    _lib.check(_L().asrk_gemm_panels_f32(M, N, K, alpha, _p(A.buf), A.rows, A.K, a_row0, a_k0, _p(B.buf), B.rows,
                                         B.K, b_row0, b_k0, beta, _p(C), ldc, _p(bias), _p(bias2), A.flags,
                                         _stream()), "gemm_panels")


def zeros(shape, device):
    t = torch.empty(shape, dtype=torch.float32, device=device)
    if t.numel():
        _lib.check(_L().asrk_fill_f32(_p(t), t.numel(), 0.0, _stream()), "fill")
    return t


def copy_flat(dst, src):
    n = src.numel()
    if n:
        copy3d(src, dst, 1, 1, n, 0, 0, 0, 0)


def copy3d(src, dst, n0, n1, n2, ss0, ss1, ds0, ds1, accumulate=False):
    _require_gpu(dst)
    _lib.check(_L().asrk_copy3d_f32(_p(src), _p(dst), n0, n1, n2, ss0, ss1, ds0, ds1,
                                    int(accumulate), _stream()), "copy3d")


def colsum(X, M, N, ldx, out, accumulate=False):
    _lib.check(_L().asrk_colsum_f32(_p(X), M, N, ldx, _p(out), int(accumulate), _stream()), "colsum")


class LinearFn(Function):

    @staticmethod
    def forward(ctx, x, weight, bias):
        _require_gpu(x)
        x2 = _f32c(x).reshape(-1, x.shape[-1])
        w = _f32c(weight)
        M, K = x2.shape
        N = w.shape[0]
        if w.dim() != 2 or w.shape[1] != K or (bias is not None and bias.numel() != N):
            raise RuntimeError("linear: input [..., {}] cannot be multiplied with weight {} (bias {})".format(
                K, tuple(w.shape), None if bias is None else tuple(bias.shape)))
        y = torch.empty((M, N), dtype=torch.float32, device=x.device)
        gemm(0, 1, M, N, K, x2, K, w, K, y, N, bias=bias)
        ctx.save_for_backward(x2, w)
        ctx.has_bias = bias is not None
        ctx.bias_ref = bias
        ctx.in_shape = x.shape
        return y.reshape(*x.shape[:-1], N)

    @staticmethod
    def backward(ctx, dy):
        x2, w = ctx.saved_tensors
        M, K = x2.shape
        N = w.shape[0]
        dy2 = _f32c(dy).reshape(M, N)
        dx = dw = db = None
        if ctx.needs_input_grad[0]:
            dx = torch.empty((M, K), dtype=torch.float32, device=dy.device)
            gemm(0, 0, M, K, N, dy2, N, w, K, dx, K)
            dx = dx.reshape(ctx.in_shape)
        def param_grads():
            dw_ = db_ = None
            if ctx.needs_input_grad[1]:
                dw_ = grad_out(w, (N, K), dy.device)
                gemm(1, 0, N, K, M, dy2, N, x2, K, dw_, K)
            if ctx.has_bias and ctx.needs_input_grad[2]:
                db_ = torch.empty((N,), dtype=torch.float32, device=dy.device)
                colsum(dy2, M, N, N, db_)
            return dw_, db_

        if M >= 1024 and _can_defer(w, ctx.bias_ref) and _defer_beside_bptt():
            with _SideStream(dy.device, (dy2, x2)) as side:
                dw, db = param_grads()
                side.keep(dw, db)
        else:
            dw, db = param_grads()
        return dx, dw, db


def linear(x, weight, bias=None):
    if not torch.is_grad_enabled():
        _require_gpu(x)
        x2 = _f32c(x).reshape(-1, x.shape[-1])
        w = _f32c(weight)
        M, K = x2.shape
        N = w.shape[0]
        if w.dim() != 2 or w.shape[1] != K or (bias is not None and bias.numel() != N):
            raise RuntimeError("linear: input [..., {}] cannot be multiplied with weight {} (bias {})".format(
                K, tuple(w.shape), None if bias is None else tuple(bias.shape)))
        y = torch.empty((M, N), dtype=torch.float32, device=x.device)
        gemm(0, 1, M, N, K, x2, K, w, K, y, N, bias=bias)
        return y.reshape(*x.shape[:-1], N)
    return LinearFn.apply(x, weight, bias)


class TanhFn(Function):
    @staticmethod
    def forward(ctx, x):
        _require_gpu(x)
        xc = _f32c(x)
        y = torch.empty_like(xc)
        _lib.check(_L().asrk_tanh_fwd_f32(_p(xc), _p(y), xc.numel(), _stream()), "tanh")
        ctx.save_for_backward(y)
        return y

    @staticmethod
    def backward(ctx, dy):
        (y,) = ctx.saved_tensors
        dyc = _f32c(dy)
        dx = torch.empty_like(y)
        _lib.check(_L().asrk_tanh_bwd_f32(_p(y), _p(dyc), _p(dx), y.numel(), _stream()), "tanh_bwd")
        return dx


def tanh(x):
    return TanhFn.apply(x)


def tanh_(x):
    _require_gpu(x)
    assert x.is_contiguous() and x.dtype == torch.float32
    _lib.check(_L().asrk_tanh_fwd_f32(_p(x), _p(x), x.numel(), _stream()), "tanh")
    return x


class LogSoftmaxFn(Function):

    @staticmethod
    def forward(ctx, x):
        _require_gpu(x)
        xc = _f32c(x)
        V = xc.shape[-1]
        rows = xc.numel() // V
        y = torch.empty_like(xc)
        _lib.check(_L().asrk_log_softmax_fwd_f32(_p(xc), _p(y), rows, V, V, _stream()), "log_softmax")
        ctx.save_for_backward(y)
        return y

    @staticmethod
    def backward(ctx, dy):
        (y,) = ctx.saved_tensors
        V = y.shape[-1]
        rows = y.numel() // V
        dyc = _f32c(dy)
        dx = torch.empty_like(y)
        _lib.check(_L().asrk_log_softmax_bwd_f32(_p(y), _p(dyc), _p(dx), rows, V, V, _stream()),
                   "log_softmax_bwd")
        return dx


def log_softmax(x):
    if not torch.is_grad_enabled():
        _require_gpu(x)
        xc = _f32c(x)
        V = xc.shape[-1]
        y = torch.empty_like(xc)
        _lib.check(_L().asrk_log_softmax_fwd_f32(_p(xc), _p(y), xc.numel() // V, V, V, _stream()), "log_softmax")
        return y
    return LogSoftmaxFn.apply(x)


def topk(x, k):
    _require_gpu(x)
    xc = _f32c(x.detach())
    V = xc.shape[-1]
    rows = xc.numel() // V
    vals = torch.empty(xc.shape[:-1] + (k,), dtype=torch.float32, device=x.device)
    idx = torch.empty(xc.shape[:-1] + (k,), dtype=torch.int64, device=x.device)
    _lib.check(_L().asrk_topk_f32(_p(xc), rows, V, V, k, _p(vals), _p(idx), _stream()), "topk")
    return vals, idx


def argmax(x):
    return topk(x, 1)[1].squeeze(-1)


def token_crop(ids, pad_idx=0, eos_idx=1, ignore_repeat=False):
    _require_gpu(ids)
    x = ids.to(torch.int64)
    if x.dim() != 2:
        raise _lib.AsrkError("token_crop expects [B, T] ids")
    if x.stride(1) != 1:
        x = x.contiguous()
    B, T = x.shape
    out = torch.zeros((B, max(T, 1)), dtype=torch.int64, device=x.device)
    n = torch.zeros((B,), dtype=torch.int32, device=x.device)
    _lib.check(_L().asrk_token_crop_i64(_p(x), x.stride(0) if B else T, B, T, pad_idx, eos_idx, int(ignore_repeat),
                                        _p(out), out.stride(0), _p(n), _stream()), "token_crop")
    return out, n


def edit_distance(a, a_len, b, b_len):
    _require_gpu(a)
    a, b = a.to(torch.int64).contiguous(), b.to(torch.int64).contiguous()
    a_len, b_len = a_len.to(torch.int32).contiguous(), b_len.to(torch.int32).contiguous()
    B = a.shape[0]
    if b.shape[0] != B or a_len.numel() != B or b_len.numel() != B:
        raise _lib.AsrkError("edit_distance: batch sizes differ")
    if b.shape[1] > 4096 and a.shape[1] <= 4096:
        a, a_len, b, b_len = b, b_len, a, a_len
    d = torch.empty((B,), dtype=torch.int32, device=a.device)
    _lib.check(_L().asrk_edit_distance_i64(_p(a), a.shape[1], _p(a_len), _p(b), b.shape[1], _p(b_len), B,
                                           b.shape[1], _p(d), _stream()), "edit_distance")
    return d


class SwapBTFn(Function):

    @staticmethod
    def forward(ctx, x):
        _require_gpu(x)
        xc = _f32c(x)
        A, B, F = xc.shape
        y = torch.empty((B, A, F), dtype=torch.float32, device=x.device)
        copy3d(xc, y, A, B, F, B * F, F, F, A * F)
        return y

    @staticmethod
    def backward(ctx, dy):
        return SwapBTFn.apply(dy)


def swap_bt(x):
    return SwapBTFn.apply(x)


class PyramidFn(Function):

    @staticmethod
    def forward(ctx, x, rate, style):
        _require_gpu(x)
        xc = _f32c(x)
        T, B, F = xc.shape
        ctx.meta = (T, B, F, rate, style)
        if style == "concat":
            To = T // rate
            y = torch.empty((To, B, rate * F), dtype=torch.float32, device=x.device)
            for j in range(rate):
                copy3d(xc[j:], y[:, :, j * F:], To, B, F, rate * B * F, F, B * rate * F, rate * F)
        else:
            To = (T + rate - 1) // rate
            y = torch.empty((To, B, F), dtype=torch.float32, device=x.device)
            copy3d(xc, y, To, B, F, rate * B * F, F, B * F, F)
        return y

    @staticmethod
    def backward(ctx, dy):
        T, B, F, rate, style = ctx.meta
        dyc = _f32c(dy)
        if style == "concat" and T % rate == 0:
            dx = torch.empty((T, B, F), dtype=torch.float32, device=dy.device)
        else:
            dx = zeros((T, B, F), dy.device)
        if style == "concat":
            To = T // rate
            for j in range(rate):
                copy3d(dyc[:, :, j * F:], dx[j:], To, B, F, B * rate * F, rate * F, rate * B * F, F)
        else:
            To = (T + rate - 1) // rate
            copy3d(dyc, dx, To, B, F, B * F, F, rate * B * F, F)
        return dx, None, None


def pyramid(x_tm, rate, style):
    return PyramidFn.apply(x_tm, rate, style)


class LSTMLayerFn(Function):

    @staticmethod
    def forward(ctx, x, w_ih_f, w_hh_f, b_ih_f, b_hh_f, w_ih_r, w_hh_r, b_ih_r, b_hh_r, pyr_rate=1,
                pyr_style=None):
        _require_gpu(x)
        L = _L()
        xc = _f32c(x)
        T, B, Din = xc.shape
        H = w_hh_f.shape[1]
        ndir = 2 if w_ih_r is not None else 1
        dev = x.device
        M = T * B
        G = torch.empty((M, ndir * 4 * H), dtype=torch.float32, device=dev)
        w_ih_f, w_hh_f = _f32c(w_ih_f), _f32c(w_hh_f)
        w_stack = None
        if ndir == 2:
            w_ih_r, w_hh_r = _f32c(w_ih_r), _f32c(w_hh_r)
        if ndir == 2 and H >= 768 and _os.environ.get("ASRK_STACK_DIRS", "1") != "0":
            if (w_ih_f.untyped_storage().data_ptr() == w_ih_r.untyped_storage().data_ptr()
                    and w_ih_r.storage_offset() == w_ih_f.storage_offset() + 4 * H * Din):
                w_stack = w_ih_f.as_strided((8 * H, Din), (Din, 1))
            else:
                w_stack = torch.empty((8 * H, Din), dtype=torch.float32, device=dev)
                copy_flat(w_stack[:4 * H], w_ih_f)
                copy_flat(w_stack[4 * H:], w_ih_r)
            if b_ih_f is not None:
                b1 = torch.empty((2, 8 * H), dtype=torch.float32, device=dev)
                for row, (bf_, br_) in enumerate(((b_ih_f, b_ih_r), (b_hh_f, b_hh_r))):
                    copy_flat(b1[row, :4 * H], _f32c(bf_.detach()))
                    copy_flat(b1[row, 4 * H:], _f32c(br_.detach()))
                b1, b2 = b1[0], b1[1]
            else:
                b1 = b2 = None
            x_panel = _take_handover(x) if x is xc else None
            if x_panel is not None and gemm_takes_split(M, 8 * H, Din):
                pW = SplitPanel(w_stack, Din, 8 * H, Din, False)
                gemm_panels(M, 8 * H, Din, x_panel, 0, 0, pW, 0, 0, G, 8 * H, bias=b1, bias2=b2)
                del pW
                _panel_state["stats"]["consumed"] += 1
            else:
                gemm(0, 1, M, 8 * H, Din, xc, Din, w_stack, Din, G, 8 * H, bias=b1, bias2=b2)
            if x_panel is not None:
                x_panel.release()
        else:
            gemm(0, 1, M, 4 * H, Din, xc, Din, w_ih_f, Din, G, ndir * 4 * H, bias=b_ih_f, bias2=b_hh_f)
            if ndir == 2:
                gemm(0, 1, M, 4 * H, Din, xc, Din, w_ih_r, Din, G[:, 4 * H:], ndir * 4 * H, bias=b_ih_r,
                     bias2=b_hh_r)
        Y = torch.empty((M, ndir * H), dtype=torch.float32, device=dev)
        C = torch.empty((M, ndir * H), dtype=torch.float32, device=dev)
        ws = lstm_workspace(dev)
        xc_ = _Exchange(L, T, B, H, ndir, 0, dev)
        mode = {None: 0, 'concat': 1, 'drop': 2}[pyr_style if pyr_rate > 1 else None]
        Y2 = None
        if mode == 1:
            Y2 = torch.empty((T // pyr_rate, B, pyr_rate * ndir * H), dtype=torch.float32, device=dev)
        elif mode == 2:
            Y2 = torch.empty(((T + pyr_rate - 1) // pyr_rate, B, ndir * H), dtype=torch.float32, device=dev)
        rate = max(1, pyr_rate)
        out_panel = None
        if (_REC_PANELS and _panel_state["hint"] and mode in (0, 1) and (mode == 0 or T // rate > 0) and
                (ndir * H) % 8 == 0 and L.asrk_lstm_plan_is_bf(T, B, H, ndir, 0, rec_flags(0))):
            r_ = rate if mode == 1 else 1
            out_panel = _BlankPanel.take((T // r_) * B, r_ * ndir * H, dev)
        if out_panel is not None:
            _panel_state["stats"]["emitted"] += 1
            _lib.check(L.asrk_lstm_rec_fwd_pyr_panel_f32(_p(G), _p(w_hh_f), _p(w_hh_r), _p(Y), _p(C), T, B, H, ndir,
                                                         _p(xc_.buf), xc_.prefilled, _p(ws), _p(Y2), mode, rate,
                                                         _p(out_panel.buf), xc_.flags, _stream()), "lstm_rec_fwd")
        else:
            _lib.check(L.asrk_lstm_rec_fwd_pyr_f32(_p(G), _p(w_hh_f), _p(w_hh_r), _p(Y), _p(C), T, B, H, ndir,
                                                   _p(xc_.buf), xc_.prefilled, _p(ws), _p(Y2), mode, rate,
                                                   xc_.flags, _stream()), "lstm_rec_fwd")
        xc_.done()
        ctx.pyr = (mode, max(1, pyr_rate))
        ctx.dims = (T, B, Din, H, ndir)
        ctx.has_bias = b_ih_f is not None
        ctx.bias_refs = (b_ih_f, b_hh_f, b_ih_r, b_hh_r)
        ctx.save_for_backward(xc, w_ih_f, w_hh_f, w_ih_r, w_hh_r, G, C, Y, w_stack)
        ctx.consumed = False
        out = Y2 if mode else Y.view(T, B, ndir * H)
        if _panel_state["handover"] is not None:
            _panel_state["handover"][2].release()
            _panel_state["handover"] = None
        if out_panel is not None:
            _panel_state["handover"] = (_weakref.ref(out), out._version, out_panel)
        return out

    @staticmethod
    def backward(ctx, dY):
        L = _L()
        xc, w_ih_f, w_hh_f, w_ih_r, w_hh_r, G, C, Y, w_stack = ctx.saved_tensors
        if ctx.consumed:
            raise RuntimeError("LSTMLayerFn: backward twice (the gate buffer is reused in place)")
        ctx.consumed = True
        T, B, Din, H, ndir = ctx.dims
        dev = dY.device
        M = T * B
        ldg, ldy = ndir * 4 * H, ndir * H
        mode, rate = ctx.pyr
        dYc = _f32c(dY)
        ws = lstm_workspace(dev)
        _note_bptt_plan(L, T, B, H, ndir)
        xc_ = _Exchange(L, T, B, H, ndir, 1, dev)
        db_all = torch.empty((ndir, 4 * H), dtype=torch.float32, device=dev) if ctx.has_bias else None
        db_in_kernel = ctx.has_bias and B <= 32
        bf_bwd = bool(_REC_PANELS and L.asrk_lstm_plan_is_bf(T, B, H, ndir, 1, rec_flags(1)))
        pG = pGT = None
        if (bf_bwd and ctx.needs_input_grad[0] and w_stack is not None and ndir * 4 * H == 8 * H and
                gemm_takes_split(M, Din, 8 * H)):
            pG = _BlankPanel.take(M, 8 * H, dev)
            _panel_state["stats"]["dg"] += pG is not None
        share0 = (_os.environ.get("ASRK_SHARE_PANELS", "1") != "0" and T > 1 and H % 128 == 0 and B % 8 == 0 and
                  gemm_takes_split(4 * H, H, (T - 1) * B))
        if bf_bwd and share0 and B % 16 == 0 and not _defer_beside_bptt() and ldg == ndir * 4 * H:
            pGT = _BlankPanel.take(ndir * 4 * H, M, dev)
            _panel_state["stats"]["dgt"] = _panel_state["stats"].get("dgt", 0) + (pGT is not None)
        if pG is not None or pGT is not None:
            _lib.check(L.asrk_lstm_rec_bwd_pyr_panel_f32(_p(G), _p(w_hh_f), _p(w_hh_r), _p(C), _p(dYc), T, B, H,
                                                         ndir, _p(xc_.buf), xc_.prefilled, _p(ws),
                                                         _p(db_all if db_in_kernel else None), mode, rate,
                                                         _p(pG.buf if pG is not None else None),
                                                         _p(pGT.buf if pGT is not None else None), xc_.flags, _stream()),
                       "lstm_rec_bwd")
        else:
            _lib.check(L.asrk_lstm_rec_bwd_pyr_f32(_p(G), _p(w_hh_f), _p(w_hh_r), _p(C), _p(dYc), T, B, H,
                                                   ndir, _p(xc_.buf), xc_.prefilled, _p(ws),
                                                   _p(db_all if db_in_kernel else None), mode, rate,
                                                   xc_.flags, _stream()), "lstm_rec_bwd")
        xc_.done()
        if ctx.has_bias and not db_in_kernel:
            colsum(G, M, ndir * 4 * H, ndir * 4 * H, db_all)
        _gemm_phase_begins()
        dG = G
        f32 = dict(dtype=torch.float32, device=dev)
        dx = None
        if ctx.needs_input_grad[0]:
            dx = torch.empty((M, Din), **f32)
            if pG is not None:
                pWT = SplitPanel(w_stack, Din, Din, 8 * H, True)
                gemm_panels(M, Din, 8 * H, pG, 0, 0, pWT, 0, 0, dx, Din)
                del pWT
                pG.release()
            elif w_stack is not None:
                gemm(0, 0, M, Din, 8 * H, dG, ldg, w_stack, Din, dx, Din)
            else:
                gemm(0, 0, M, Din, 4 * H, dG, ldg, w_ih_f, Din, dx, Din)
                if ndir == 2:
                    gemm(0, 0, M, Din, 4 * H, dG[:, 4 * H:], ldg, w_ih_r, Din, dx, Din, beta=1.0)
            dx = dx.view(T, B, Din)
        dw_ih_stack = [None]
        share = [share0, False]
        panels = {}
        if pGT is not None:
            panels["dGT"] = pGT

        def panel(name, src, ld, rows):
            if name not in panels:
                panels[name] = SplitPanel(src, ld, rows, M, True)
            return panels[name]

        def dg_gemm(Mo, No, Ko, m0, k0, pB, b_row0, b_k0, out, ldo):
            gemm_panels(Mo, No, Ko, panel("dGT", dG, ldg, ndir * 4 * H), m0, k0, pB, b_row0, b_k0, out, ldo)

        def param_grads_panels(d):
            pY = panel("YT", Y, ldy, ndir * H)
            Mh = (T - 1) * B
            dw_hh = grad_out(w_hh[d], (4 * H, H), dev)
            dg_gemm(4 * H, H, Mh, d * 4 * H, B if d == 0 else 0, pY, d * H, 0 if d == 0 else B, dw_hh, H)
            rows_ih = 8 * H if (w_stack is not None and stack_dw) else 4 * H
            if gemm_takes_split(rows_ih, Din, M) and Din % 4 == 0:
                pX = panel("XT", xc, Din, Din)
                if rows_ih == 8 * H:
                    if dw_ih_stack[0] is None:
                        dw_ih_stack[0] = torch.empty((8 * H, Din), **f32)
                        dg_gemm(8 * H, Din, M, 0, 0, pX, 0, 0, dw_ih_stack[0], Din)
                    dw_ih = dw_ih_stack[0][d * 4 * H:(d + 1) * 4 * H]
                else:
                    dw_ih = grad_out(w_ih[d], (4 * H, Din), dev)
                    dg_gemm(4 * H, Din, M, d * 4 * H, 0, pX, 0, 0, dw_ih, Din)
            elif rows_ih == 8 * H:
                if dw_ih_stack[0] is None:
                    dw_ih_stack[0] = torch.empty((8 * H, Din), **f32)
                    gemm(1, 0, 8 * H, Din, M, dG, ldg, xc, Din, dw_ih_stack[0], Din)
                dw_ih = dw_ih_stack[0][d * 4 * H:(d + 1) * 4 * H]
            else:
                dw_ih = grad_out(w_ih[d], (4 * H, Din), dev)
                gemm(1, 0, 4 * H, Din, M, dG[:, d * 4 * H:], ldg, xc, Din, dw_ih, Din)
            db = db2 = None
            if ctx.has_bias:
                db = db_all[d]
                db2 = db.clone()
            return dw_ih, dw_hh, db, db2

        def param_grads(d):
            if share[0] and share[1]:
                return param_grads_panels(d)
            dGd = dG[:, d * 4 * H:]
            if w_stack is not None and stack_dw:
                if dw_ih_stack[0] is None:
                    dw_ih_stack[0] = torch.empty((8 * H, Din), **f32)
                    gemm(1, 0, 8 * H, Din, M, dG, ldg, xc, Din, dw_ih_stack[0], Din)
                dw_ih = dw_ih_stack[0][d * 4 * H:(d + 1) * 4 * H]
            else:
                dw_ih = grad_out(w_ih[d], (4 * H, Din), dev)
                gemm(1, 0, 4 * H, Din, M, dGd, ldg, xc, Din, dw_ih, Din)
            dw_hh = zeros((4 * H, H), dev) if T <= 1 else grad_out(w_hh[d], (4 * H, H), dev)
            if T > 1:
                Mh = (T - 1) * B
                if d == 0:
                    gemm(1, 0, 4 * H, H, Mh, dGd[B:], ldg, Y, ldy, dw_hh, H)
                else:
                    gemm(1, 0, 4 * H, H, Mh, dGd, ldg, Y[B:, H:], ldy, dw_hh, H)
            db = db2 = None
            if ctx.has_bias:
                db = db_all[d]
                db2 = db.clone()
            return dw_ih, dw_hh, db, db2

        w_ih, w_hh = (w_ih_f, w_ih_r), (w_hh_f, w_hh_r)
        stack_dw = ((ctx.needs_input_grad[0] or not _can_defer(w_ih_f, w_hh_f, w_ih_r, w_hh_r, *ctx.bias_refs))
                    and not grad_has_destination(*w_ih[:ndir]))
        beside = _defer_beside_bptt() or not ctx.needs_input_grad[0]
        if _can_defer(w_ih_f, w_hh_f, w_ih_r, w_hh_r, *ctx.bias_refs) and beside:
            if ctx.needs_input_grad[0] or ndir == 1:
                with _SideStream(dev, (dG, xc, Y, db_all)) as side:
                    share[1] = True
                    grads = [param_grads(d) for d in range(ndir)]
                    side.keep(*[t for g in grads for t in g])
            elif pGT is not None and gemm_takes_split(4 * H, Din, M) and Din % 4 == 0:
                share[1] = True
                grads = [param_grads(d) for d in range(ndir)]
            elif pGT is not None:
                pY = panel("YT", Y, ldy, ndir * H)
                share[1] = True
                with _SideStream(dev, (dG, xc, Y, db_all, pGT.buf, pY.buf), background=False) as side:
                    g1 = param_grads(1)
                    side.keep(*g1)
                grads = [param_grads(0), g1]
                _defer["release"].append(pGT)
                pGT = None
            else:
                with _SideStream(dev, (dG, xc, Y, db_all), background=False) as side:
                    g1 = param_grads(1)
                    side.keep(*g1)
                grads = [param_grads(0), g1]
        else:
            share[1] = True
            grads = [param_grads(d) for d in range(ndir)]
        if pGT is not None:
            if share[1] and not _defer["pending"]:
                pGT.release()
            else:
                _defer["release"].append(pGT)
        if ndir == 1:
            grads.append((None, None, None, None))
        return (dx,) + grads[0] + grads[1] + (None, None)


class Copy3dFn(Function):

    @staticmethod
    def forward(ctx, src, out_shape, n0, n1, n2, ss0, ss1, ds0, ds1):
        _require_gpu(src)
        s = _f32c(src)
        dst = zeros(out_shape, src.device)
        copy3d(s, dst, n0, n1, n2, ss0, ss1, ds0, ds1)
        ctx.meta = (tuple(src.shape), n0, n1, n2, ss0, ss1, ds0, ds1)
        return dst

    @staticmethod
    def backward(ctx, g):
        shape, n0, n1, n2, ss0, ss1, ds0, ds1 = ctx.meta
        gs = zeros(shape, g.device)
        copy3d(_f32c(g), gs, n0, n1, n2, ds0, ds1, ss0, ss1)
        return (gs,) + (None,) * 8


def _pad_lstm_params(params, H, Hp):
    w_ih, w_hh, b_ih, b_hh = params
    Din = w_ih.shape[1]
    w_ih_p = Copy3dFn.apply(w_ih, (4 * Hp, Din), 4, H, Din, H * Din, Din, Hp * Din, Din)
    w_hh_p = Copy3dFn.apply(w_hh, (4 * Hp, Hp), 4, H, H, H * H, H, Hp * Hp, Hp)
    b_ih_p = Copy3dFn.apply(b_ih, (4 * Hp,), 1, 4, H, 0, H, 0, Hp)
    b_hh_p = Copy3dFn.apply(b_hh, (4 * Hp,), 1, 4, H, 0, H, 0, Hp)
    return w_ih_p, w_hh_p, b_ih_p, b_hh_p


def lstm_layer(x_tm, params_f, params_r=None, pyramid=None):
    H = params_f[1].shape[1]
    if pyramid is not None and pyramid[0] > 1:
        if H % 4 != 0 or _os.environ.get("ASRK_FUSE_PYRAMID", "1") == "0":
            return PyramidFn.apply(lstm_layer(x_tm, params_f, params_r), pyramid[0], pyramid[1])
        pr = params_r if params_r is not None else (None, None, None, None)
        return LSTMLayerFn.apply(x_tm, *params_f, *pr, pyramid[0], pyramid[1])
    if H % 4 != 0:
        Hp = (H + 3) // 4 * 4
        ndir = 2 if params_r is not None else 1
        pf = _pad_lstm_params(params_f, H, Hp)
        pr = _pad_lstm_params(params_r, H, Hp) if params_r is not None else (None,) * 4
        T, B = x_tm.shape[0], x_tm.shape[1]
        yp = LSTMLayerFn.apply(x_tm, *pf, *pr)
        return Copy3dFn.apply(yp, (T, B, ndir * H), T * B, ndir, H, ndir * Hp, Hp, ndir * H, H)
    pr = params_r if params_r is not None else (None, None, None, None)
    return LSTMLayerFn.apply(x_tm, *params_f, *pr)


def lstm_layer_packed(x_tm, params_f, params_r, lens, pyramid=None):
    _require_gpu(x_tm)
    if torch.is_grad_enabled() and x_tm.requires_grad:
        raise _lib.AsrkError("lstm_layer_packed is inference-only")
    L = _L()
    xc = _f32c(x_tm)
    T, B, Din = xc.shape
    w_ih_f, w_hh_f, b_ih_f, b_hh_f = (None if t is None else _f32c(t.detach()) for t in params_f)
    H = w_hh_f.shape[1]
    if H % 4 != 0:
        raise _lib.AsrkError("lstm_layer_packed: hidden size must be a multiple of 4")
    ndir = 2 if params_r is not None else 1
    dev = xc.device
    M = T * B
    G = torch.empty((M, ndir * 4 * H), dtype=torch.float32, device=dev)
    gemm(0, 1, M, 4 * H, Din, xc, Din, w_ih_f, Din, G, ndir * 4 * H, bias=b_ih_f, bias2=b_hh_f)
    w_hh_r = None
    if ndir == 2:
        w_ih_r, w_hh_r, b_ih_r, b_hh_r = (None if t is None else _f32c(t.detach()) for t in params_r)
        gemm(0, 1, M, 4 * H, Din, xc, Din, w_ih_r, Din, G[:, 4 * H:], ndir * 4 * H, bias=b_ih_r, bias2=b_hh_r)
    lens_d = torch.as_tensor(lens).to(device=dev, dtype=torch.int64).contiguous()
    Y = zeros((M, ndir * H), dev)
    C = torch.empty((M, ndir * H), dtype=torch.float32, device=dev)
    rate, style = pyramid if pyramid is not None else (1, None)
    mode = {None: 0, 'concat': 1, 'drop': 2}[style if rate > 1 else None]
    Y2 = None
    if mode == 1:
        Y2 = zeros((T // rate, B, rate * ndir * H), dev)
    elif mode == 2:
        Y2 = zeros(((T + rate - 1) // rate, B, ndir * H), dev)
    ws = lstm_workspace(dev)
    xc_ = _Exchange(L, T, B, H, ndir, 0, dev)
    _lib.check(L.asrk_lstm_rec_fwd_len_f32(_p(G), _p(w_hh_f), _p(w_hh_r), _p(Y), _p(C), _p(lens_d), T, B, H, ndir,
                                           _p(xc_.buf), xc_.prefilled, _p(ws), _p(Y2), mode, max(1, rate), xc_.flags,
                                           _stream()), "lstm_rec_fwd_len")
    xc_.done()
    return Y2 if mode else Y.view(T, B, ndir * H)


class CTCLossFn(Function):

    @staticmethod
    def forward(ctx, log_probs, targets, input_lengths, target_lengths, blank, reduction):
        _require_gpu(log_probs)
        L = _L()
        if log_probs.dtype != torch.float32:
            log_probs = log_probs.float()
        if log_probs.stride(2) != 1:
            log_probs = log_probs.contiguous()
        T, B, V = log_probs.shape
        dev = log_probs.device
        targets = torch.as_tensor(targets).to(device=dev, dtype=torch.int64)
        if targets.dim() != 2:
            raise _lib.AsrkError("CTCLoss: only padded 2-D targets [B, L] are supported "
                                 "(reference passes txt [B,L], bin/train_asr.py:123)")
        targets = targets.contiguous()
        il = torch.as_tensor(input_lengths).to(device=dev, dtype=torch.int64).contiguous()
        tl = torch.as_tensor(target_lengths).to(device=dev, dtype=torch.int64).contiguous()
        Lmax = targets.shape[1]
        S = 2 * Lmax + 1
        alpha = torch.empty((B, T, S), dtype=torch.float32, device=dev)
        lpg = torch.empty((B, T, S), dtype=torch.float32, device=dev)
        beta = torch.empty((B, T, S), dtype=torch.float32, device=dev) if ctx.needs_input_grad[0] else None
        nll = torch.empty((B,), dtype=torch.float32, device=dev)
        _lib.check(L.asrk_ctc_loss_fwd_f32(_p(log_probs), log_probs.stride(0), log_probs.stride(1), T,
                                           B, V, _p(targets), targets.stride(0), Lmax, _p(il),
                                           _p(tl), blank, _p(alpha), _p(beta), _p(lpg), _p(nll),
                                           _stream()), "ctc_fwd")
        ctx.save_for_backward(log_probs, targets, il, tl, alpha, beta, lpg, nll)
        ctx.meta = (T, B, V, Lmax, blank, reduction)
        if reduction == "mean":
            return (nll / tl.clamp(min=1).to(torch.float32)).mean()
        if reduction == "sum":
            return nll.sum()
        return nll

    @staticmethod
    def backward(ctx, gout):
        L = _L()
        log_probs, targets, il, tl, alpha, beta, lpg, nll = ctx.saved_tensors
        T, B, V, Lmax, blank, reduction = ctx.meta
        dev = log_probs.device
        if reduction == "mean":
            gscale = gout.to(torch.float32) / (tl.clamp(min=1).to(torch.float32) * B)
        elif reduction == "sum":
            gscale = gout.to(torch.float32).expand(B)
        else:
            gscale = gout.to(torch.float32)
        gscale = gscale.contiguous()
        if log_probs.stride(1) > log_probs.stride(0):
            grad = torch.empty((B, T, V), dtype=torch.float32, device=dev).transpose(0, 1)
        else:
            grad = torch.empty((T, B, V), dtype=torch.float32, device=dev)
        _lib.check(L.asrk_ctc_loss_bwd_f32(_p(log_probs), log_probs.stride(0), log_probs.stride(1), T,
                                           B, V, _p(targets), targets.stride(0), Lmax, _p(il),
                                           _p(tl), blank, _p(alpha), _p(beta), _p(lpg), _p(nll), _p(gscale),
                                           _p(grad), grad.stride(0), grad.stride(1), _stream()),
                   "ctc_bwd")
        return grad, None, None, None, None, None


class CTCLoss(torch.nn.Module):

    def __init__(self, blank=0, reduction="mean", zero_infinity=False):
        super().__init__()
        if zero_infinity:
            raise NotImplementedError("zero_infinity=True is not used by the reference "
                                      "(bin/train_asr.py:49)")
        self.blank = blank
        self.reduction = reduction

    def forward(self, log_probs, targets, input_lengths, target_lengths):
        return CTCLossFn.apply(log_probs, targets, input_lengths, target_lengths, self.blank,
                               self.reduction)


class CrossEntropyFn(Function):

    @staticmethod
    def forward(ctx, logits, targets, ignore_index):
        _require_gpu(logits)
        x = _f32c(logits)
        R, V = x.shape
        tg = targets.to(device=x.device, dtype=torch.int64).contiguous()
        lse = torch.empty((R,), dtype=torch.float32, device=x.device)
        sums = torch.empty((2,), dtype=torch.float32, device=x.device)
        _lib.check(_L().asrk_cross_entropy_fwd_f32(_p(x), R, V, V, _p(tg), ignore_index, _p(lse),
                                                   _p(sums), _stream()), "cross_entropy")
        ctx.save_for_backward(x, tg, lse, sums)
        ctx.ignore_index = ignore_index
        return sums[0] / sums[1]

    @staticmethod
    def backward(ctx, gout):
        x, tg, lse, sums = ctx.saved_tensors
        R, V = x.shape
        gscale = (gout.to(torch.float32) / sums[1]).reshape(1).contiguous()
        dx = torch.empty_like(x)
        _lib.check(_L().asrk_cross_entropy_bwd_f32(_p(x), R, V, V, _p(tg), ctx.ignore_index, _p(lse),
                                                   _p(gscale), _p(dx), _stream()), "cross_entropy_bwd")
        return dx, None, None


class CrossEntropyLoss(torch.nn.Module):

    def __init__(self, ignore_index=-100, reduction="mean"):
        super().__init__()
        assert reduction == "mean"
        self.ignore_index = ignore_index

    def forward(self, logits, targets):
        return CrossEntropyFn.apply(logits, targets, self.ignore_index)


class LayerNormFn(Function):

    @staticmethod
    def forward(ctx, x, weight, bias, eps):
        _require_gpu(x)
        xc = _f32c(x)
        D = xc.shape[-1]
        if weight.numel() != D or bias.numel() != D:
            raise RuntimeError("layer_norm: normalized_shape {} does not match input [..., {}]".format(
                tuple(weight.shape), D))
        rows = xc.numel() // D
        w, b = _f32c(weight), _f32c(bias)
        y = torch.empty_like(xc)
        mean = torch.empty((rows,), dtype=torch.float32, device=x.device)
        rstd = torch.empty((rows,), dtype=torch.float32, device=x.device)
        _lib.check(_L().asrk_layer_norm_fwd_f32(_p(xc), _p(w), _p(b), _p(y), _p(mean), _p(rstd), rows, D,
                                                float(eps), _stream()), "layer_norm")
        ctx.save_for_backward(xc, w, mean, rstd)
        return y

    @staticmethod
    def backward(ctx, dy):
        xc, w, mean, rstd = ctx.saved_tensors
        D = xc.shape[-1]
        rows = xc.numel() // D
        dyc = _f32c(dy)
        dx = torch.empty_like(xc) if ctx.needs_input_grad[0] else None
        want_p = ctx.needs_input_grad[1] or ctx.needs_input_grad[2]
        dw = torch.empty((D,), dtype=torch.float32, device=dy.device) if want_p else None
        db = torch.empty((D,), dtype=torch.float32, device=dy.device) if want_p else None
        _lib.check(_L().asrk_layer_norm_bwd_f32(_p(xc), _p(w), _p(dyc), _p(mean), _p(rstd), _p(dx), _p(dw),
                                                _p(db), rows, D, _stream()), "layer_norm_bwd")
        return dx, dw, db, None


def layer_norm(x, weight, bias, eps):
    return LayerNormFn.apply(x, weight, bias, eps)


class DropoutFn(Function):

    @staticmethod
    def forward(ctx, x, p, seed):
        _require_gpu(x)
        xc = _f32c(x)
        y = torch.empty_like(xc)
        _lib.check(_L().asrk_dropout_f32(_p(xc), _p(y), xc.numel(), float(p), seed, 0, _stream()), "dropout")
        ctx.p, ctx.seed = float(p), seed
        return y

    @staticmethod
    def backward(ctx, dy):
        dyc = _f32c(dy)
        dx = torch.empty_like(dyc)
        _lib.check(_L().asrk_dropout_f32(_p(dyc), _p(dx), dyc.numel(), ctx.p, ctx.seed, 0, _stream()),
                   "dropout_bwd")
        return dx, None, None


def dropout(x, p, training, seed=None):
    if not training or p == 0:
        return x
    if p >= 1:
        raise ValueError("dropout probability has to be in [0, 1), got {}".format(p))
    if seed is None:
        seed = int(torch.randint(0, 2 ** 62, (1,)).item())
    return DropoutFn.apply(x, p, seed)
```

### include/asrk.h

```cpp
#ifndef ASRK_H
#define ASRK_H

#include <stddef.h>
#include <stdint.h>

#ifdef __cplusplus
extern "C" {
#endif

#define ASRK_OK 0
#define ASRK_EINVAL (-1)
#define ASRK_ESHAPE (-2)
#define ASRK_EWORKSPACE (-3)
#define ASRK_EDEVICE (-4)
#define ASRK_ETIMEOUT (-5)

int asrk_version(void);
const char *asrk_strerror(int rc);
int asrk_init(int device);

void asrk_profile_enable(int on);
void asrk_profile_families(unsigned mask);
void asrk_profile_reset(void);
int asrk_profile_get(int id, double *total_ms, int64_t *launches);
int asrk_profile_get_work(int id, double *flops);
#define ASRK_PROF_GEMM 0
#define ASRK_PROF_LSTM_FWD 1
#define ASRK_PROF_LSTM_BWD 2
#define ASRK_PROF_CTC 3
#define ASRK_PROF_ROWOPS 4
#define ASRK_PROF_ATTN 5
#define ASRK_PROF_CELL 6
#define ASRK_PROF_FBANK 7
#define ASRK_PROF_GEMM_BG 8
#define ASRK_PROF_SPELLER 9
#define ASRK_PROF_CONV 10
#define ASRK_PROF_SPLIT 11
#define ASRK_PROF_OPTIM 12

int asrk_gemm_f32(int transA, int transB, int M, int N, int K, float alpha,
                  const float *A, int lda, const float *B, int ldb, float beta,
                  float *C, int ldc, const float *bias, const float *bias2, int splitk,
                  int flags, void *ws, size_t ws_bytes, void *stream);

#define ASRK_GEMM_SPLIT_AUTO 0
#define ASRK_GEMM_SPLIT_OFF 1
#define ASRK_GEMM_SPLIT_ALWAYS 2
#define ASRK_GEMM_LDS_HINT(kib) (((kib) & 0xff) << 8)
size_t asrk_gemm_ws_bytes(int M, int N, int K, int flags);
int asrk_gemm_takes_split(int M, int N, int K, int flags);

size_t asrk_split_panel_bytes(int rows, int K, int flags);
int asrk_split_panel_f32(const float *src, int ld, int rows, int K, int trans, void *panel, int flags, void *stream);
int asrk_gemm_panels_f32(int M, int N, int K, float alpha, const void *A_panel, int a_rows, int a_K,
                         int a_row0, int a_k0, const void *B_panel, int b_rows, int b_K, int b_row0, int b_k0,
                         float beta, float *C, int ldc, const float *bias, const float *bias2, int flags,
                         void *stream);

int asrk_copy3d_f32(const float *src, float *dst, int n0, int n1, int n2,
                    int64_t s_stride0, int64_t s_stride1, int64_t d_stride0, int64_t d_stride1,
                    int accumulate, void *stream);

int asrk_colsum_f32(const float *X, int M, int N, int ldx, float *out, int accumulate,
                    void *stream);

int asrk_tanh_fwd_f32(const float *x, float *y, int64_t n, void *stream);
int asrk_tanh_bwd_f32(const float *y, const float *dy, float *dx, int64_t n, void *stream);

int asrk_log_softmax_fwd_f32(const float *x, float *y, int rows, int cols, int ld,
                             void *stream);
int asrk_log_softmax_bwd_f32(const float *y, const float *dy, float *dx, int rows, int cols,
                             int ld, void *stream);

int asrk_topk_f32(const float *x, int rows, int cols, int ld, int k, float *values,
                  int64_t *indices, void *stream);

int asrk_token_crop_i64(const int64_t *ids, int64_t ld, int B, int T, int64_t pad_idx, int64_t eos_idx,
                        int ignore_repeat, int64_t *out, int64_t ld_out, int32_t *out_len, void *stream);
int asrk_edit_distance_i64(const int64_t *a, int64_t lda, const int32_t *a_len, const int64_t *b, int64_t ldb,
                           const int32_t *b_len, int B, int max_b_len, int32_t *dist, void *stream);

int asrk_cross_entropy_fwd_f32(const float *logits, int rows, int V, int ld,
                               const int64_t *targets, int ignore_index, float *row_lse,
                               float *sums, void *stream);
int asrk_cross_entropy_bwd_f32(const float *logits, int rows, int V, int ld,
                               const int64_t *targets, int ignore_index, const float *row_lse,
                               const float *gscale, float *dlogits, void *stream);

size_t asrk_lstm_ws_bytes(void);
#define ASRK_REC_F32_MFMA 1
#define ASRK_REC_REARM 2
size_t asrk_lstm_xchg_bytes(int T, int B, int H, int ndir, int backward, int flags);
int asrk_lstm_plan_workgroups(int T, int B, int H, int ndir, int backward, int flags);
int asrk_lstm_rec_fwd_f32(float *G, const float *whh_f, const float *whh_r, float *Y, float *C,
                          int T, int B, int H, int ndir, void *xchg, int xchg_prefilled, void *ws,
                          int flags, void *stream);
int asrk_lstm_rec_fwd_pyr_f32(float *G, const float *whh_f, const float *whh_r, float *Y, float *C,
                              int T, int B, int H, int ndir, void *xchg, int xchg_prefilled, void *ws,
                              float *Y2, int pyr_mode, int pyr_rate, int flags, void *stream);
int asrk_lstm_rec_bwd_pyr_f32(float *gates, const float *whh_f, const float *whh_r, const float *C,
                              const float *dY, int T, int B, int H, int ndir, void *xchg,
                              int xchg_prefilled, void *ws, float *db, int pyr_mode, int pyr_rate,
                              int flags, void *stream);
int asrk_lstm_plan_is_bf(int T, int B, int H, int ndir, int backward, int flags);
int asrk_lstm_rec_fwd_pyr_panel_f32(float *G, const float *whh_f, const float *whh_r, float *Y, float *C,
                                    int T, int B, int H, int ndir, void *xchg, int xchg_prefilled, void *ws,
                                    float *Y2, int pyr_mode, int pyr_rate, void *x2_panel, int flags, void *stream);
int asrk_lstm_rec_bwd_pyr_panel_f32(float *gates, const float *whh_f, const float *whh_r, const float *C,
                                    const float *dY, int T, int B, int H, int ndir, void *xchg,
                                    int xchg_prefilled, void *ws, float *db, int pyr_mode, int pyr_rate,
                                    void *dg_panel, void *dgt_panel, int flags, void *stream);
int asrk_lstm_rec_fwd_len_f32(float *G, const float *whh_f, const float *whh_r, float *Y, float *C,
                              const int64_t *lens, int T, int B, int H, int ndir, void *xchg,
                              int xchg_prefilled, void *ws, float *Y2, int pyr_mode, int pyr_rate, int flags,
                              void *stream);
int asrk_gru_rec_fwd_f32(float *G, const float *whh_f, const float *whh_r, float *Y, int T, int B, int H,
                         int ndir, void *xchg, int xchg_prefilled, void *ws, float *Y2, int pyr_mode,
                         int pyr_rate, int flags, void *stream);
int asrk_gru_rec_bwd_f32(float *gates, const float *whh_f, const float *whh_r, const float *Y,
                         const float *dY, int T, int B, int H, int ndir, void *xchg, int xchg_prefilled,
                         void *ws, float *db, int pyr_mode, int pyr_rate, int flags, void *stream);
int asrk_lstm_rec_bwd_f32(float *gates, const float *whh_f, const float *whh_r, const float *C,
                          const float *dY, int T, int B, int H, int ndir, void *xchg,
                          int xchg_prefilled, void *ws, float *db, int flags, void *stream);
int asrk_lstm_check_error(void *ws, void *stream);

size_t asrk_ctc_prefix_beam_ws_bytes(int beam, int T);
int asrk_ctc_prefix_beam_ws_offsets(int beam, int T, int buf, int64_t *nb_off, int64_t *len_off, int64_t *tok_off,
                                    int64_t *parent_off, int64_t *last_off, int64_t *gidx_off);
int asrk_ctc_prefix_beam_f32(const float *ctc, int T, int V, const unsigned char *allowed, int beam, int cand,
                             const float *lm, float lm_weight, int t0, int t1, int cur_buf, int init,
                             int lm_step_follows, void *ws, size_t ws_bytes, void *stream);

int asrk_loc_conv_fwd_f32(const float *prev_att, const float *Wc, float *c, int B, int N, int T,
                          int K, int ks, void *stream);
int asrk_loc_conv_bwd_f32(const float *dc, const float *prev_att, const float *Wc,
                          float *dprev_att, float *dWc_acc, int B, int N, int T, int K, int ks,
                          void *stream);
int asrk_attn_energy_fwd_f32(int loc, const float *key, const float *q, const float *c,
                             const float *Wp, const float *we, const float *be,
                             const int64_t *lens, float *attn, float *e_scratch, int B, int N, int T,
                             int A, int K, float temperature, void *stream);
int asrk_attn_energy_bwd_f32(int loc, const float *key, const float *q, const float *c,
                             const float *Wp, const float *we, const int64_t *lens,
                             const float *attn, const float *dattn, float *dkey_acc, float *dq,
                             float *dc, float *dWp_acc, float *dwe_acc, float *dbe_acc, int B,
                             int N, int T, int A, int K, float temperature, void *stream);
int asrk_attn_context_fwd_f32(const float *attn, const float *value, float *ctx, int BN, int T,
                              int Dv, int64_t ctx_stride, void *stream);
int asrk_attn_context_bwd_f32(const float *dctx, const float *value, float *dattn, int BN, int T,
                              int Dv, int64_t dctx_stride, void *stream);

int asrk_lstm_cell_fwd_f32(float *gates, const float *c_prev, float *c, float *h, int B, int H,
                           void *stream);
int asrk_lstm_cell_bwd_f32(float *gates, const float *c_prev, const float *c, const float *dh,
                           const float *dc_in, float *dc_prev, int B, int H, void *stream);

int asrk_gru_cell_fwd_f32(float *gi, const float *gh, int64_t ldi, int64_t ldh, const float *h_prev,
                          int64_t ldp, float *h_new, int64_t ldn, int B, int H, void *stream);
int asrk_gru_cell_bwd_f32(float *gi, float *gh, int64_t ldi, int64_t ldh, const float *h_prev,
                          int64_t ldp, const float *dh, int64_t ldd, const float *dh2, float *dh_prev,
                          int64_t ldo, int B, int H, void *stream);

int asrk_embedding_fwd_f32(const int64_t *idx, const float *W, float *out, int64_t n, int D, int V,
                           void *stream);
int asrk_embedding_bwd_f32(const int64_t *idx, const float *dout, float *dW_acc, int64_t n, int D,
                           int V, void *stream);

typedef struct asrk_speller {
    int B, Te, A, Dv, K, ks, H, E, L;
    float temperature;
    int shared_kv;
    const float *key, *value;
    const int64_t *lens;
    const float *Wq, *bq, *Wc, *Wp, *we, *be, *W_ih, *W_hh, *b_ih, *b_hh;
    const float *eproj;
    float *q, *conv, *attn;
    int64_t attn_ld, attn_step;
    float *ctx, *gates, *h, *c, *states, *e_scratch;
    const float *prev0;
    const int *row_mem;
    int cell;
    int nlayer;
    const float *Wu_ih[2], *Wu_hh[2], *bu_ih[2], *bu_hh[2];
    float *hu[2], *cu[2], *gu[2];
    int att_mode, nhead;
    const float *Wm, *bm;
    float *ctxh;
    int row_group;
} asrk_speller_t;
#define ASRK_SPELLER_MAX_LAYERS 3

typedef struct asrk_speller_bwd {
    const float *dstates, *dattn_seq, *WT, *WqT;
    float *dkey, *dxh, *dq_pre, *dattn, *dprev, *dconv, *dq_part, *dwe_part, *dWp_part, *dbe_part,
        *dWc_part, *dc;
    int tc;
    const float *WuT[2];
    float *dxu[2], *dcu[2];
    const float *WmT;
    float *dctxh;
} asrk_speller_bwd_t;

int asrk_speller_plan(const asrk_speller_t *dims, int *tc_fwd, int *tc_bwd);
int asrk_speller_fwd_f32(const asrk_speller_t *p, void *stream);
int asrk_speller_bwd_f32(const asrk_speller_t *p, const asrk_speller_bwd_t *g, void *stream);
int asrk_speller_step_f32(const asrk_speller_t *p, int slot, const float *prev_att, int64_t prev_ld,
                          const float *emb, void *stream);
int asrk_speller_dvalue_f32(const float *attn, int64_t attn_ld, int64_t attn_step, const float *dxh,
                            int64_t step_ld, int64_t row_ld, float *dvalue, int B, int L, int Te, int Dv,
                            void *stream);
int asrk_joint_score_f32(const float *att_logp, const int64_t *cand, const float *psi,
                         const float *prev_ctc, const float *lm_logp, float *out, int n, int V, int C,
                         double ctc_weight, double lm_weight, double logzero, void *stream);
int asrk_lstm_cell_fused_f32(const float *x, int64_t ldx, int In, const float *h, const float *c,
                             const float *W_ih, const float *W_hh, const float *b_ih,
                             const float *b_hh, float *h_out, float *c_out, int B, int H, void *stream);
int asrk_transpose_ld_f32(const float *in, int64_t ldi, float *out, int64_t ldo, int rows, int cols,
                          void *stream);

int asrk_layer_norm_fwd_f32(const float *x, const float *weight, const float *bias, float *y,
                            float *mean, float *rstd, int rows, int cols, float eps, void *stream);
int asrk_layer_norm_bwd_f32(const float *x, const float *weight, const float *dy, const float *mean,
                            const float *rstd, float *dx, float *dweight, float *dbias, int rows,
                            int cols, void *stream);
int asrk_dropout_f32(const float *x, float *y, int64_t n, float p, uint64_t seed, uint64_t offset,
                     void *stream);

int asrk_beam_select_f32(const float *topv, const int64_t *topi, const float *psi, const int64_t *cand, int U, int B, int C,
                         int t, int lmax, int fcap, const int *min_len, const int *max_len, int *alive, double *ssum,
                         int *utt_done, int64_t *prev_token, int64_t *parent, int64_t *col, float *pctc, int *hist_tok,
                         float *hist_sc, int *hist_par, int *fin_count, int *fin_kind, int *fin_t, int *fin_row,
                         float *fin_term, double *fin_ssum, int *live_utts, void *stream);

int asrk_gather_rows_multi_f32(int nseg, const float *const *src, float *const *dst, const int *row_floats, const int *mul,
                               const int *use_col, const int64_t *parent, const int64_t *col, int n, void *stream);

int asrk_conv_out_size(int in, int k, int stride, int pad);
int asrk_im2col_f32(const float *x, float *col, int B, int H, int W, int C, int KH, int KW, int SH, int SW,
                    int PH, int PW, int64_t sb, int64_t sh, int64_t sw, int64_t sc, void *stream);
int asrk_col2im_f32(const float *dcol, float *dx, int B, int H, int W, int C, int KH, int KW, int SH,
                    int SW, int PH, int PW, int64_t sb, int64_t sh, int64_t sw, int64_t sc, void *stream);
int asrk_im2col_ld_f32(const float *x, float *col, int ldcol, int B, int H, int W, int C, int KH, int KW, int SH, int SW,
                       int PH, int PW, int64_t sb, int64_t sh, int64_t sw, int64_t sc, void *stream);
int asrk_im2col_cl_f32(const float *x, float *col, int B, int H, int W, int C, int KH, int KW, int SH, int SW,
                       int PH, int PW, int64_t sb, int64_t sh, int64_t sw, int64_t sc, void *stream);
int asrk_col2im_cl_f32(const float *dcol, float *dx, int B, int H, int W, int C, int KH, int KW, int SH,
                       int SW, int PH, int PW, int64_t sb, int64_t sh, int64_t sw, int64_t sc, void *stream);
int asrk_conv_weight_reorder_f32(const float *src, float *dst, int Cout, int Cin, int KK, int inverse, void *stream);
int asrk_conv3x3_supported(int H, int W, int C, int Cout);
int asrk_conv3x3_weight_f32(const float *w, float *wf, int Cout, int Cin, int transpose, void *stream);
int asrk_conv3x3_f32(const float *x, const float *xmask, const float *wf, const float *bias, float *y, int B, int H, int W,
                     int C, int Cout, int relu, void *stream);
size_t asrk_conv3x3_wgrad_ws_bytes(int B, int H, int W, int C, int Cout);
int asrk_conv3x3_wgrad_f32(const float *x, const float *dy, const float *ymask, float *dw, float *db, int B, int H, int W,
                           int C, int Cout, void *ws, size_t ws_bytes, void *stream);
int asrk_conv3x3_first_supported(int H, int W, int C, int Cout);
int asrk_conv3x3_first_f32(const float *x, const float *w, const float *bias, float *y, int B, int H, int W, int C, int Cout,
                           int64_t sb, int64_t sh, int64_t sw, int64_t sc, int relu, void *stream);
size_t asrk_conv3x3_first_wgrad_ws_bytes(int B, int H, int W, int C, int Cout);
int asrk_conv3x3_first_wgrad_f32(const float *x, const float *dy, const float *ymask, float *dw, float *db, int B, int H,
                                 int W, int C, int Cout, int64_t sb, int64_t sh, int64_t sw, int64_t sc, void *ws,
                                 size_t ws_bytes, void *stream);
int asrk_relu_fwd_f32(float *x, int64_t n, void *stream);
int asrk_relu_bwd_f32(const float *y, const float *dy, float *dx, int64_t n, void *stream);
int asrk_maxpool2x2_fwd_f32(const float *x, float *y, uint8_t *idx, int B, int H, int W, int C,
                            int64_t osb, int64_t osh, int64_t osw, int64_t osc, void *stream);
int asrk_maxpool2x2_bwd_f32(const float *dy, const uint8_t *idx, float *dx, int B, int H, int W, int C,
                            int64_t osb, int64_t osh, int64_t osw, int64_t osc, void *stream);

int asrk_adadelta_step_f32(float *param, const float *grad, float *square_avg, float *acc_delta,
                           int64_t n, double lr, double rho, double eps, const float *clip_coef,
                           void *stream);
int asrk_adam_step_f32(float *param, const float *grad, float *exp_avg, float *exp_avg_sq, int64_t n,
                       double lr, double beta1, double beta2, double eps, int64_t step,
                       const float *clip_coef, void *stream);
int asrk_adadelta_multi_f32(int count, float *const *params, const float *const *grads,
                            float *const *square_avg, float *const *acc_delta, const int64_t *numel,
                            double lr, double rho, double eps, const float *clip_coef, void *stream);
int asrk_adam_multi_f32(int count, float *const *params, const float *const *grads,
                        float *const *exp_avg, float *const *exp_avg_sq, const int64_t *numel,
                        double lr, double beta1, double beta2, double eps, int64_t step,
                        const float *clip_coef, void *stream);

size_t asrk_grad_norm_ws_bytes(int count, const int64_t *numel);
int asrk_grad_norm_multi_f32(int count, const float *const *grads, const int64_t *numel, float max_norm,
                             float *norm_out, float *coef_out, void *ws, size_t ws_bytes, void *stream);
int asrk_fill_f32(float *x, int64_t n, float value, void *stream);

int asrk_fbank_frames_f32(const float *wave, int64_t n_samples, const float *window, float *frames,
                          int m, int win, int shift, int ldf, float preemph, int remove_dc,
                          void *stream);
int asrk_power_spectrum_f32(const float *spec, float *power, int64_t m, int nb, void *stream);
int asrk_log_floor_f32(float *x, int64_t n, float eps, void *stream);
int asrk_delta_f32(const float *x, const float *filters, float *y, int C, int D, int T, int L,
                   void *stream);
int asrk_cmvn_f32(const float *x, float *y, int rows, int T, float eps, void *stream);
int asrk_transpose_f32(const float *x, float *y, int rows, int cols, void *stream);
int asrk_fbank_frames_batch_f32(const void *wave, int sample_bytes, int64_t ld_wave, const int64_t *n_samples_host,
                                const int64_t *frame_off, int B, int max_m, const float *window, float *frames,
                                int win, int shift, int ldf, float scale, float preemph, int remove_dc,
                                void *stream);
int asrk_delta_cmvn_batch_f32(const float *mel, const int64_t *frame_off, int B, int D, const float *filters, int C,
                              int L, int apply_cmvn, float eps, float *out, int Tmax, void *stream);
int asrk_fbank_logmel_batch_f32(const void *wave, int sample_bytes, int64_t ld_wave, const int64_t *n_samples_host,
                                const int64_t *frame_off, int B, int max_m, const float *window, const float *tw_fft,
                                const float *tw_unpack, const float *melT, const int *mel_range, int nmel, int ld_mel,
                                float *mel, int win, int shift, int log2n, float scale, float preemph, int remove_dc,
                                float eps, void *stream);

int asrk_ctc_loss_fwd_f32(const float *lp, int64_t stride_t, int64_t stride_b, int T, int B,
                          int V, const int64_t *targets, int64_t tgt_stride, int Lmax,
                          const int64_t *input_lengths, const int64_t *target_lengths,
                          int blank, float *alpha, float *beta, float *lpg, float *nll,
                          void *stream);
int asrk_ctc_loss_bwd_f32(const float *lp, int64_t stride_t, int64_t stride_b, int T, int B,
                          int V, const int64_t *targets, int64_t tgt_stride, int Lmax,
                          const int64_t *input_lengths, const int64_t *target_lengths,
                          int blank, const float *alpha, const float *beta, const float *lpg,
                          const float *nll, const float *gscale, float *grad, int64_t g_stride_t,
                          int64_t g_stride_b, void *stream);

int asrk_ctc_prefix_score_f32(const float *x, const float *r_prev, const int *prefix_len,
                              const int *last_char, const int *candidates, float *psi,
                              float *r_out, int n, int C, int T, int V, int blank, int eos,
                              float logzero, void *stream);
int asrk_ctc_prefix_score_multi_f32(const float *x, const int *row_mem, const int *mem_len, const float *r_prev,
                                    const int *prefix_len, const int *last_char, const int *candidates,
                                    float *psi, float *r_out, int n, int C, int T, int V, int U, int blank,
                                    int eos, float logzero, void *stream);

int asrk_flac_info(const char *path, int *sample_rate, int *channels, int *bits_per_sample,
                   int64_t *total_samples, uint8_t *md5_16);
int asrk_flac_decode_i32(const char *path, int32_t *out, int64_t capacity_samples,
                         int64_t *decoded_samples);

#ifdef __cplusplus
}
#endif
#endif
```

Measured before the change: 525,400 frames/s.

## Add split-K panel GEMM for narrow LSTM input-weight grads and skip dense dG writes

Adds a split-K variant of the bf16x3 panel GEMM. Each K-slice writes its partial tile through an LDS transpose into a workspace, and a reduce kernel then sums the slices and applies alpha, beta and bias. The LSTM backward uses it for the narrow dW_ih GEMM (small Din, such as the 80-mel input) so that layer gets enough tiles to fill the CUs, instead of falling back to a non-panel path. When the transposed dG panel already carries everything the downstream GEMMs need, the recurrent backward kernel also stops writing the dense fp32 dG tensor, saving that memory traffic. The cost is an extra workspace allocation per call, an extra reduce launch, and more complex conditions for when dG may be skipped.

Result: faster. 533,700 frames/s (median of 6 runs) (+1.6%).

```diff
diff --git a/end-to-end-asr-pytorch_amd/_lib.py b/end-to-end-asr-pytorch_amd/_lib.py
--- a/end-to-end-asr-pytorch_amd/_lib.py
+++ b/end-to-end-asr-pytorch_amd/_lib.py
@@ -25,6 +25,10 @@
     "asrk_split_panel_f32": (c_int, [c_vp, c_int, c_int, c_int, c_int, c_vp, c_int, c_vp]),
     "asrk_gemm_panels_f32": (c_int, [c_int, c_int, c_int, c_f32, c_vp, c_int, c_int, c_int, c_int,
                                      c_vp, c_int, c_int, c_int, c_int, c_f32, c_vp, c_int, c_vp, c_vp, c_int, c_vp]),
+    "asrk_gemm_panels_splitk_ws_bytes": (c_sz, [c_int, c_int, c_int]),
+    "asrk_gemm_panels_splitk_f32": (c_int, [c_int, c_int, c_int, c_f32, c_vp, c_int, c_int, c_int, c_int,
+                                            c_vp, c_int, c_int, c_int, c_int, c_f32, c_vp, c_int, c_vp, c_vp, c_int,
+                                            c_vp, c_sz, c_int, c_vp]),
     "asrk_copy3d_f32": (c_int, [c_vp, c_vp, c_int, c_int, c_int, c_i64, c_i64, c_i64, c_i64, c_int,
                                 c_vp]),
     "asrk_colsum_f32": (c_int, [c_vp, c_int, c_int, c_int, c_vp, c_int, c_vp]),
diff --git a/end-to-end-asr-pytorch_amd/csrc/gemm_split.hip b/end-to-end-asr-pytorch_amd/csrc/gemm_split.hip
--- a/end-to-end-asr-pytorch_amd/csrc/gemm_split.hip
+++ b/end-to-end-asr-pytorch_amd/csrc/gemm_split.hip
@@ -1,6 +1,7 @@
 #include "common.h"
 #include "knobs.h"
 #include <algorithm>
+#include <climits>
 
 extern "C" int asrk_cu_count_(void);
 
@@ -20,6 +21,8 @@
     int nk;
     int tiles_m, tiles_n;
     float alpha, beta;
+    int slices, ldw;
+    float *ws;
 };
 
 __device__ __forceinline__ void split8(const float (&v)[8], u32x4 (&w)[3]) {
@@ -128,10 +131,11 @@
 }
 __device__ __forceinline__ void wait_lgkm0() { __builtin_amdgcn_s_waitcnt(0xC07F); }
 
-template <int NC, int NST, bool SPEC, int WM>
+template <int NC, int NST, bool SPEC, int WM, bool SK = false>
 __global__ __launch_bounds__(SPEC ? (WM == 2 ? 512 : 704) : 256) void gemm_bf16x6_kernel(SplitGemmArgs p) {
     extern __shared__ __attribute__((aligned(1024))) unsigned char lds[];
     static_assert(WM == 2 || (WM == 4 && SPEC), "256-row tiles only with DMA waves");
+    static_assert(!SK || NST >= 2, "the split-K epilogue transposes through a stage the last k-tile does not use");
     constexpr int NPL = 3, CHUNK = NPL * PIECE;
     constexpr int NCW = 2 * WM;
     constexpr int NRG = WM + 2;
@@ -141,7 +145,10 @@
     constexpr int LPT = NC * NPL * RPD;
     const int tid = threadIdx.x, lane = tid & 63;
     const int wave = __builtin_amdgcn_readfirstlane(tid >> 6);
-    const int ntiles = p.tiles_m * p.tiles_n, bid = blockIdx.x;
+    const int ntiles = p.tiles_m * p.tiles_n;
+    const int slice = SK ? blockIdx.x / ntiles : 0, bid = SK ? blockIdx.x - slice * ntiles : blockIdx.x;
+    const int kt0 = SK ? (int)((long)slice * p.nk / p.slices) : 0;
+    const int nk = SK ? (int)((long)(slice + 1) * p.nk / p.slices) - kt0 : p.nk;
     const int q8 = ntiles >> 3, r8 = ntiles & 7, xcd = bid & 7, loc = bid >> 3;
     const int tile = (xcd < r8 ? xcd * (q8 + 1) : r8 * (q8 + 1) + (xcd - r8) * q8) + loc;
     constexpr int BAND = 8;
@@ -160,6 +167,7 @@
         const int r = r0 + q;
         gsrc[q] = (r < WM ? p.Ap + (size_t)(ltm * WM + r) * p.rb_stride_a
                           : p.Bp + (size_t)(ltn * 2 + r - WM) * p.rb_stride_b);
+        if (SK) gsrc[q] += (size_t)kt0 * REGION;
     }
     const unsigned voff = lane * 16;
     unsigned char *ldst = lds + r0 * REGION;
@@ -182,7 +190,6 @@
 #pragma unroll
             for (int r = 0; r < 16; ++r) acc[i][j][r] = 0.f;
 
-    const int nk = p.nk;
     const int frag_off = ((lane >> 5) * NPL) * PIECE + (lane & 31) * 16;
     const unsigned char *abase = lds + wr * REGION + frag_off;
     const unsigned char *bbase = lds + (WM + wc) * REGION + frag_off;
@@ -281,6 +288,37 @@
         step((S - 1) & 1, false, 0, 0);
     }
 
+    if constexpr (SK) {
+        constexpr int PITCH = 36;
+        static_assert(NCW * 32 * PITCH * 4 <= STAGE, "transposition images fit one stage");
+        int fstage = stage + 1;
+        if (fstage == NST) fstage = 0;
+        float *img = reinterpret_cast<float *>(lds + fstage * STAGE) + wave * 32 * PITCH;
+        float *wsl = p.ws + (size_t)slice * p.M * p.ldw;
+        const int wrow0 = tm * 64 * WM + wr * 64, wcol0 = tn * 128 + wc * 64;
+#pragma unroll
+        for (int i = 0; i < 2; ++i)
+#pragma unroll
+            for (int j = 0; j < 2; ++j) {
+#pragma unroll
+                for (int r = 0; r < 16; ++r)
+                    img[((r & 3) + 8 * (r >> 2) + 4 * (lane >> 5)) * PITCH + (lane & 31)] = acc[i][j][r];
+                __builtin_amdgcn_fence(__ATOMIC_RELEASE, "wavefront");
+                __builtin_amdgcn_wave_barrier();
+                __builtin_amdgcn_fence(__ATOMIC_ACQUIRE, "wavefront");
+#pragma unroll
+                for (int q = 0; q < 4; ++q) {
+                    const int idx = q * 64 + lane, rl = idx >> 3, c4 = (idx & 7) * 4;
+                    const f32x4 v = *reinterpret_cast<const f32x4 *>(img + rl * PITCH + c4);
+                    const int row = wrow0 + i * 32 + rl, col = wcol0 + j * 32 + c4;
+                    if (row < p.M && col < p.ldw) *reinterpret_cast<f32x4 *>(wsl + (size_t)row * p.ldw + col) = v;
+                }
+                __builtin_amdgcn_fence(__ATOMIC_RELEASE, "wavefront");
+                __builtin_amdgcn_wave_barrier();
+                __builtin_amdgcn_fence(__ATOMIC_ACQUIRE, "wavefront");
+            }
+        return;
+    }
     const int row0 = tm * 64 * WM + wr * 64 + 4 * (lane >> 5), col0 = tn * 128 + wc * 64 + (lane & 31);
 #pragma unroll
     for (int j = 0; j < 2; ++j) {
@@ -300,6 +338,31 @@
                 if (p.beta != 0.f) v += p.beta * *c;
                 *c = v;
             }
+    }
+}
+
+__global__ __launch_bounds__(256) void splitk_reduce_kernel(const float *__restrict__ ws, int slices, int M, int N,
+                                                            int ldw, float alpha, float beta, float *__restrict__ C,
+                                                            int ldc, const float *__restrict__ bias,
+                                                            const float *__restrict__ bias2) {
+    const int n4 = ldw >> 2;
+    const int64_t idx = (int64_t)blockIdx.x * 256 + threadIdx.x;
+    if (idx >= (int64_t)M * n4) return;
+    const int row = (int)(idx / n4), col = (int)(idx - (int64_t)row * n4) * 4;
+    const size_t plane = (size_t)M * ldw;
+    const float *w = ws + (size_t)row * ldw + col;
+    f32x4 a = *reinterpret_cast<const f32x4 *>(w);
+    for (int s = 1; s < slices; ++s) a += *reinterpret_cast<const f32x4 *>(w + (size_t)s * plane);
+#pragma unroll
+    for (int e = 0; e < 4; ++e) {
+        if (col + e >= N) break;
+        float bsum = 0.f;
+        if (bias) bsum += bias[col + e];
+        if (bias2) bsum += bias2[col + e];
+        float *c = C + (size_t)row * ldc + col + e;
+        float v = alpha * a[e] + bsum;
+        if (beta != 0.f) v += beta * *c;
+        *c = v;
     }
 }
 
@@ -489,14 +552,21 @@
     return ASRK_OK;
 }
 
-template <int NC, int NST, bool SPEC, int WM>
+template <int NC, int NST, bool SPEC, int WM, bool SK = false>
 int launch_split_gemm(const SplitGemmArgs &a, hipStream_t s) {
     constexpr int lds = NST * (WM + 2) * NC * 3 * PIECE;
-    auto kern = gemm_bf16x6_kernel<NC, NST, SPEC, WM>;
+    auto kern = gemm_bf16x6_kernel<NC, NST, SPEC, WM, SK>;
     static AsrkLdsLatch latch;
     ASRK_HIP(asrk_max_lds_once(latch, reinterpret_cast<const void *>(kern), lds));
-    hipLaunchKernelGGL(kern, dim3(a.tiles_m * a.tiles_n), dim3(SPEC ? (WM == 2 ? 512 : 704) : 256), lds, s, a);
+    hipLaunchKernelGGL(kern, dim3(a.tiles_m * a.tiles_n * (SK ? a.slices : 1)), dim3(SPEC ? (WM == 2 ? 512 : 704) : 256),
+                       lds, s, a);
     ASRK_LAUNCH_CHECK();
+    if (SK) {
+        const int64_t items = (int64_t)a.M * (a.ldw >> 2);
+        hipLaunchKernelGGL(splitk_reduce_kernel, dim3((unsigned)asrk_div_up64(items, 256)), dim3(256), 0, s, a.ws,
+                           a.slices, a.M, a.N, a.ldw, a.alpha, a.beta, a.C, a.ldc, a.bias, a.bias2);
+        ASRK_LAUNCH_CHECK();
+    }
     return ASRK_OK;
 }
 
@@ -536,15 +606,25 @@
     return ASRK_OK;
 }
 
+int auto_slices(int M, int N, int nk) {
+    if (N >= 512) return 1;
+    const int ncu = asrk_cu_count_() > 0 ? asrk_cu_count_() : 256;
+    const long tiles = (long)asrk_div_up(M, 128) * asrk_div_up(N, 128);
+    const long want = (ncu + tiles - 1) / tiles;
+    return (int)std::max(1L, std::min(want, (long)(nk / 64)));
+}
+
 int run_panel_gemm(int M, int N, int nk, float alpha, const unsigned char *Ap, size_t stride_a,
                    const unsigned char *Bp, size_t stride_b, float beta, float *C, int ldc, const float *bias,
-                   const float *bias2, hipStream_t s) {
+                   const float *bias2, hipStream_t s, int slices = 1, float *ws = nullptr) {
     const AsrkKnobs &kn = asrk_knobs_();
     SplitGemmArgs a;
     a.Ap = Ap; a.Bp = Bp; a.C = C; a.bias = bias; a.bias2 = bias2;
     a.M = M; a.N = N; a.ldc = ldc; a.KC = 0; a.nk = nk; a.rb_stride_a = stride_a; a.rb_stride_b = stride_b;
     a.tiles_m = asrk_div_up(M, 128); a.tiles_n = asrk_div_up(N, 128);
     a.alpha = alpha; a.beta = beta;
+    a.slices = std::min(slices, nk); a.ldw = (N + 3) & ~3; a.ws = ws;
+    if (a.slices > 1) return launch_split_gemm<4, 3, true, 2, true>(a, s);
     const int w256 = kn.get(kn.split_w256, 1);
     if (w256 && N >= 512) {
         const int tm = asrk_div_up(M, 128), tn = asrk_div_up(N, 256);
@@ -620,26 +700,71 @@
     return rc;
 }
 
-extern "C" int asrk_gemm_panels_f32(int M, int N, int K, float alpha, const void *A_panel, int a_rows, int a_K,
-                                    int a_row0, int a_k0, const void *B_panel, int b_rows, int b_K, int b_row0,
-                                    int b_k0, float beta, float *C, int ldc, const float *bias,
-                                    const float *bias2, int flags, void *stream) {
+namespace {
+struct PanelRange {
+    const unsigned char *Ap, *Bp;
+    size_t stride_a, stride_b;
+    int nk;
+};
+int panel_range(int M, int N, int K, const void *A_panel, int a_rows, int a_K, int a_row0, int a_k0,
+                const void *B_panel, int b_rows, int b_K, int b_row0, int b_k0, const float *C, int ldc, int flags,
+                PanelRange &r) {
     if (M <= 0 || N <= 0 || K <= 0 || !A_panel || !B_panel || !C || ldc < N || flags != 0) return ASRK_EINVAL;
     if (a_row0 < 0 || b_row0 < 0 || a_k0 < 0 || b_k0 < 0 || a_row0 % 128 || b_row0 % 128 || a_k0 % 8 || b_k0 % 8)
         return ASRK_EINVAL;
     if (a_row0 + M > a_rows || b_row0 + N > b_rows || a_k0 + K > a_K || b_k0 + K > b_K) return ASRK_EINVAL;
     if (K % 32 != 0 && a_k0 + K != a_K && b_k0 + K != b_K) return ASRK_ESHAPE;
     const PanelGeom ga = panel_geom(a_rows, a_K, true), gb = panel_geom(b_rows, b_K, true);
-    const int nk = asrk_div_up(K, 32);
-    if (a_k0 / 8 + nk * SPLIT_NC > ga.KC || b_k0 / 8 + nk * SPLIT_NC > gb.KC) return ASRK_ESHAPE;
+    r.nk = asrk_div_up(K, 32);
+    if (a_k0 / 8 + r.nk * SPLIT_NC > ga.KC || b_k0 / 8 + r.nk * SPLIT_NC > gb.KC) return ASRK_ESHAPE;
+    const unsigned char *A0 = reinterpret_cast<const unsigned char *>(A_panel);
+    const unsigned char *B0 = reinterpret_cast<const unsigned char *>(B_panel);
+    r.Ap = A0 + (size_t)(a_row0 / 64) * ga.rb_stride + (size_t)(a_k0 / 8) * NPL * PIECE;
+    r.Bp = B0 + (size_t)(b_row0 / 64) * gb.rb_stride + (size_t)(b_k0 / 8) * NPL * PIECE;
+    r.stride_a = ga.rb_stride; r.stride_b = gb.rb_stride;
+    return ASRK_OK;
+}
+}
+
+extern "C" int asrk_gemm_panels_f32(int M, int N, int K, float alpha, const void *A_panel, int a_rows, int a_K,
+                                    int a_row0, int a_k0, const void *B_panel, int b_rows, int b_K, int b_row0,
+                                    int b_k0, float beta, float *C, int ldc, const float *bias,
+                                    const float *bias2, int flags, void *stream) {
+    PanelRange r;
+    const int rc0 = panel_range(M, N, K, A_panel, a_rows, a_K, a_row0, a_k0, B_panel, b_rows, b_K, b_row0, b_k0, C, ldc,
+                                flags, r);
+    if (rc0 != ASRK_OK) return rc0;
     hipStream_t s = (hipStream_t)stream;
     asrk_prof_work_(PROF_GEMM, 2.0 * (double)M * (double)N * (double)K);
     asrk_prof_begin_(PROF_GEMM, s);
-    const unsigned char *A0 = reinterpret_cast<const unsigned char *>(A_panel);
-    const unsigned char *B0 = reinterpret_cast<const unsigned char *>(B_panel);
-    const unsigned char *Ap = A0 + (size_t)(a_row0 / 64) * ga.rb_stride + (size_t)(a_k0 / 8) * NPL * PIECE;
-    const unsigned char *Bp = B0 + (size_t)(b_row0 / 64) * gb.rb_stride + (size_t)(b_k0 / 8) * NPL * PIECE;
-    const int rc = run_panel_gemm(M, N, nk, alpha, Ap, ga.rb_stride, Bp, gb.rb_stride, beta, C, ldc, bias, bias2, s);
+    const int rc = run_panel_gemm(M, N, r.nk, alpha, r.Ap, r.stride_a, r.Bp, r.stride_b, beta, C, ldc, bias, bias2, s);
     asrk_prof_end_(PROF_GEMM, s);
     return rc;
 }
+
+extern "C" size_t asrk_gemm_panels_splitk_ws_bytes(int M, int N, int splitk) {
+    if (M <= 0 || N <= 0 || splitk < 0) return 0;
+    const int n = splitk > 0 ? splitk : auto_slices(M, N, INT_MAX);
+    return (size_t)n * (size_t)M * (size_t)((N + 3) & ~3) * sizeof(float);
+}
+
+extern "C" int asrk_gemm_panels_splitk_f32(int M, int N, int K, float alpha, const void *A_panel, int a_rows, int a_K,
+                                           int a_row0, int a_k0, const void *B_panel, int b_rows, int b_K,
+                                           int b_row0, int b_k0, float beta, float *C, int ldc, const float *bias,
+                                           const float *bias2, int splitk, void *ws, size_t ws_bytes, int flags,
+                                           void *stream) {
+    if (splitk < 0 || !ws || (reinterpret_cast<uintptr_t>(ws) & 15) != 0) return ASRK_EINVAL;
+    PanelRange r;
+    const int rc0 = panel_range(M, N, K, A_panel, a_rows, a_K, a_row0, a_k0, B_panel, b_rows, b_K, b_row0, b_k0, C, ldc,
+                                flags, r);
+    if (rc0 != ASRK_OK) return rc0;
+    const int slices = splitk > 0 ? splitk : auto_slices(M, N, r.nk);
+    if (ws_bytes < asrk_gemm_panels_splitk_ws_bytes(M, N, slices)) return ASRK_EWORKSPACE;
+    hipStream_t s = (hipStream_t)stream;
+    asrk_prof_work_(PROF_GEMM, 2.0 * (double)M * (double)N * (double)K);
+    asrk_prof_begin_(PROF_GEMM, s);
+    const int rc = run_panel_gemm(M, N, r.nk, alpha, r.Ap, r.stride_a, r.Bp, r.stride_b, beta, C, ldc, bias, bias2, s,
+                                  slices, reinterpret_cast<float *>(ws));
+    asrk_prof_end_(PROF_GEMM, s);
+    return rc;
+}
diff --git a/end-to-end-asr-pytorch_amd/csrc/lstm_rec.hip b/end-to-end-asr-pytorch_amd/csrc/lstm_rec.hip
--- a/end-to-end-asr-pytorch_amd/csrc/lstm_rec.hip
+++ b/end-to-end-asr-pytorch_amd/csrc/lstm_rec.hip
@@ -458,6 +458,7 @@
     }
     const bool one_launch = pl.ndir_l >= ndir && pl.nbg_l >= pl.nbg;
     a.rearm = (flags & ASRK_REC_REARM) && one_launch ? 1 : 0;
+    a.no_dg = (flags & ASRK_REC_BWD_NO_DG) && (dg_panel || dgt_panel) ? 1 : 0;
     if (db) ASRK_HIP(hipMemsetAsync(db, 0, (size_t)ndir * 4 * H * sizeof(float), s));
     asrk_prof_begin_(PROF_LSTM_BWD, s);
     int rc = ASRK_OK;
diff --git a/end-to-end-asr-pytorch_amd/csrc/lstm_rec_bwd_bf.hip b/end-to-end-asr-pytorch_amd/csrc/lstm_rec_bwd_bf.hip
--- a/end-to-end-asr-pytorch_amd/csrc/lstm_rec_bwd_bf.hip
+++ b/end-to-end-asr-pytorch_amd/csrc/lstm_rec_bwd_bf.hip
@@ -303,7 +303,7 @@
             }
         }
         REC_STAMP(5);
-        if (c_valid) {
+        if (c_valid && !p.no_dg) {
             float *g = p.G + ((size_t)t * p.B + c_b) * p.ldg + dir * 4 * H + c_unit;
 #pragma unroll
             for (int r = 0; r < 4; ++r) g[(size_t)r * H] = dgs[r];
diff --git a/end-to-end-asr-pytorch_amd/csrc/lstm_rec_common.h b/end-to-end-asr-pytorch_amd/csrc/lstm_rec_common.h
--- a/end-to-end-asr-pytorch_amd/csrc/lstm_rec_common.h
+++ b/end-to-end-asr-pytorch_amd/csrc/lstm_rec_common.h
@@ -43,6 +43,7 @@
     float *db;
     int pyr_mode, pyr_rate;
     int rearm;
+    int no_dg;
     unsigned char *PG;
     size_t pg_stride;
     unsigned char *PT;
diff --git a/end-to-end-asr-pytorch_amd/ops.py b/end-to-end-asr-pytorch_amd/ops.py
--- a/end-to-end-asr-pytorch_amd/ops.py
+++ b/end-to-end-asr-pytorch_amd/ops.py
@@ -73,6 +73,7 @@
 
 
 ASRK_REC_REARM = 2
+ASRK_REC_BWD_NO_DG = 4
 _XCHG_REARM = _os.environ.get("ASRK_XCHG_REARM", "1") != "0"
 _XCHG_POOL_CAP = int(float(_os.environ.get("ASRK_XCHG_POOL_GB", "24")) * (1 << 30))
 _xchg_pool = {"free": {}, "bytes": 0, "tick": 0, "stats": {"hit": 0, "miss": 0, "evicted": 0}}
@@ -337,6 +338,7 @@
 
 import weakref as _weakref
 _REC_PANELS = _os.environ.get("ASRK_REC_PANELS", "1") != "0"
+_REC_SKIP_DG = True
 _panel_pool = {"free": {}, "bytes": 0, "tick": 0, "seen": {}, "stats": {"hit": 0, "miss": 0, "skipped": 0, "evicted": 0}}
 _panel_state = {"hint": False, "handover": None, "stats": {"emitted": 0, "consumed": 0, "dg": 0}}
 
@@ -394,16 +396,25 @@
     return None
 
 
-def gemm_panels(M, N, K, A, a_row0, a_k0, B, b_row0, b_k0, C, ldc, alpha=1.0, beta=0.0, bias=None, bias2=None):
+def gemm_panels(M, N, K, A, a_row0, a_k0, B, b_row0, b_k0, C, ldc, alpha=1.0, beta=0.0, bias=None, bias2=None,
+                splitk=None):
     _require_gpu(C)
     avail = C.untyped_storage().nbytes() // C.element_size() - C.storage_offset()
     if ldc < N or avail < (M - 1) * ldc + N:
         raise _lib.AsrkError("gemm_panels: C too small for {}x{} with ld {}".format(M, N, ldc))
     if A.flags != B.flags:
         raise _lib.AsrkError("gemm_panels: the two panels were built in different layouts")
-    _lib.check(_L().asrk_gemm_panels_f32(M, N, K, alpha, _p(A.buf), A.rows, A.K, a_row0, a_k0, _p(B.buf), B.rows,
-                                         B.K, b_row0, b_k0, beta, _p(C), ldc, _p(bias), _p(bias2), A.flags,
-                                         _stream()), "gemm_panels")
+    L = _L()
+    if splitk is None:
+        _lib.check(L.asrk_gemm_panels_f32(M, N, K, alpha, _p(A.buf), A.rows, A.K, a_row0, a_k0, _p(B.buf), B.rows,
+                                          B.K, b_row0, b_k0, beta, _p(C), ldc, _p(bias), _p(bias2), A.flags,
+                                          _stream()), "gemm_panels")
+        return
+    nws = int(L.asrk_gemm_panels_splitk_ws_bytes(M, N, splitk))
+    ws = torch.empty((nws,), dtype=torch.uint8, device=C.device)
+    _lib.check(L.asrk_gemm_panels_splitk_f32(M, N, K, alpha, _p(A.buf), A.rows, A.K, a_row0, a_k0, _p(B.buf), B.rows,
+                                             B.K, b_row0, b_k0, beta, _p(C), ldc, _p(bias), _p(bias2), splitk, _p(ws),
+                                             nws, A.flags, _stream()), "gemm_panels")
 
 
 def zeros(shape, device):
@@ -785,12 +796,24 @@
         if bf_bwd and share0 and B % 16 == 0 and not _defer_beside_bptt() and ldg == ndir * 4 * H:
             pGT = _BlankPanel.take(ndir * 4 * H, M, dev)
             _panel_state["stats"]["dgt"] = _panel_state["stats"].get("dgt", 0) + (pGT is not None)
+        w_ih, w_hh = (w_ih_f, w_ih_r), (w_hh_f, w_hh_r)
+        can_defer = _can_defer(w_ih_f, w_hh_f, w_ih_r, w_hh_r, *ctx.bias_refs)
+        to_scratch = not grad_has_destination(*w_ih[:ndir])
+        stack_dw = (ctx.needs_input_grad[0] or not can_defer) and to_scratch
+        rows_ih = 8 * H if (w_stack is not None and stack_dw) else 4 * H
+        narrow_ih = pGT is not None and Din % 4 == 0 and not gemm_takes_split(rows_ih, Din, M)
+        if narrow_ih and w_stack is not None and to_scratch:
+            rows_ih = 8 * H
+        skip_dg = (_REC_SKIP_DG and pGT is not None and Din % 4 == 0 and (not ctx.needs_input_grad[0] or pG is not None)
+                   and (db_in_kernel or not ctx.has_bias))
         if pG is not None or pGT is not None:
+            _panel_state["stats"]["no_dg"] = _panel_state["stats"].get("no_dg", 0) + skip_dg
             _lib.check(L.asrk_lstm_rec_bwd_pyr_panel_f32(_p(G), _p(w_hh_f), _p(w_hh_r), _p(C), _p(dYc), T, B, H,
                                                          ndir, _p(xc_.buf), xc_.prefilled, _p(ws),
                                                          _p(db_all if db_in_kernel else None), mode, rate,
                                                          _p(pG.buf if pG is not None else None),
-                                                         _p(pGT.buf if pGT is not None else None), xc_.flags, _stream()),
+                                                         _p(pGT.buf if pGT is not None else None),
+                                                         xc_.flags | (ASRK_REC_BWD_NO_DG if skip_dg else 0), _stream()),
                        "lstm_rec_bwd")
         else:
             _lib.check(L.asrk_lstm_rec_bwd_pyr_f32(_p(G), _p(w_hh_f), _p(w_hh_r), _p(C), _p(dYc), T, B, H,
@@ -829,25 +852,28 @@
                 panels[name] = SplitPanel(src, ld, rows, M, True)
             return panels[name]
 
-        def dg_gemm(Mo, No, Ko, m0, k0, pB, b_row0, b_k0, out, ldo):
-            gemm_panels(Mo, No, Ko, panel("dGT", dG, ldg, ndir * 4 * H), m0, k0, pB, b_row0, b_k0, out, ldo)
+        def dg_gemm(Mo, No, Ko, m0, k0, pB, b_row0, b_k0, out, ldo, splitk=None):
+            gemm_panels(Mo, No, Ko, panel("dGT", dG, ldg, ndir * 4 * H), m0, k0, pB, b_row0, b_k0, out, ldo,
+                        splitk=splitk)
 
         def param_grads_panels(d):
             pY = panel("YT", Y, ldy, ndir * H)
             Mh = (T - 1) * B
             dw_hh = grad_out(w_hh[d], (4 * H, H), dev)
             dg_gemm(4 * H, H, Mh, d * 4 * H, B if d == 0 else 0, pY, d * H, 0 if d == 0 else B, dw_hh, H)
-            rows_ih = 8 * H if (w_stack is not None and stack_dw) else 4 * H
-            if gemm_takes_split(rows_ih, Din, M) and Din % 4 == 0:
+            if (gemm_takes_split(rows_ih, Din, M) or narrow_ih) and Din % 4 == 0:
                 pX = panel("XT", xc, Din, Din)
+                sk = 0 if narrow_ih else None
                 if rows_ih == 8 * H:
                     if dw_ih_stack[0] is None:
                         dw_ih_stack[0] = torch.empty((8 * H, Din), **f32)
-                        dg_gemm(8 * H, Din, M, 0, 0, pX, 0, 0, dw_ih_stack[0], Din)
+                        dg_gemm(8 * H, Din, M, 0, 0, pX, 0, 0, dw_ih_stack[0], Din, sk)
+                        _panel_state["stats"]["dw_ih_splitk"] = _panel_state["stats"].get("dw_ih_splitk", 0) + narrow_ih
                     dw_ih = dw_ih_stack[0][d * 4 * H:(d + 1) * 4 * H]
                 else:
                     dw_ih = grad_out(w_ih[d], (4 * H, Din), dev)
-                    dg_gemm(4 * H, Din, M, d * 4 * H, 0, pX, 0, 0, dw_ih, Din)
+                    dg_gemm(4 * H, Din, M, d * 4 * H, 0, pX, 0, 0, dw_ih, Din, sk)
+                    _panel_state["stats"]["dw_ih_splitk"] = _panel_state["stats"].get("dw_ih_splitk", 0) + narrow_ih
             elif rows_ih == 8 * H:
                 if dw_ih_stack[0] is None:
                     dw_ih_stack[0] = torch.empty((8 * H, Din), **f32)
@@ -887,17 +913,14 @@
                 db2 = db.clone()
             return dw_ih, dw_hh, db, db2
 
-        w_ih, w_hh = (w_ih_f, w_ih_r), (w_hh_f, w_hh_r)
-        stack_dw = ((ctx.needs_input_grad[0] or not _can_defer(w_ih_f, w_hh_f, w_ih_r, w_hh_r, *ctx.bias_refs))
-                    and not grad_has_destination(*w_ih[:ndir]))
         beside = _defer_beside_bptt() or not ctx.needs_input_grad[0]
-        if _can_defer(w_ih_f, w_hh_f, w_ih_r, w_hh_r, *ctx.bias_refs) and beside:
+        if can_defer and beside:
             if ctx.needs_input_grad[0] or ndir == 1:
                 with _SideStream(dev, (dG, xc, Y, db_all)) as side:
                     share[1] = True
                     grads = [param_grads(d) for d in range(ndir)]
                     side.keep(*[t for g in grads for t in g])
-            elif pGT is not None and gemm_takes_split(4 * H, Din, M) and Din % 4 == 0:
+            elif pGT is not None and Din % 4 == 0:
                 share[1] = True
                 grads = [param_grads(d) for d in range(ndir)]
             elif pGT is not None:
diff --git a/include/asrk.h b/include/asrk.h
--- a/include/asrk.h
+++ b/include/asrk.h
@@ -56,6 +56,11 @@
                          int a_row0, int a_k0, const void *B_panel, int b_rows, int b_K, int b_row0, int b_k0,
                          float beta, float *C, int ldc, const float *bias, const float *bias2, int flags,
                          void *stream);
+size_t asrk_gemm_panels_splitk_ws_bytes(int M, int N, int splitk);
+int asrk_gemm_panels_splitk_f32(int M, int N, int K, float alpha, const void *A_panel, int a_rows, int a_K,
+                                int a_row0, int a_k0, const void *B_panel, int b_rows, int b_K, int b_row0, int b_k0,
+                                float beta, float *C, int ldc, const float *bias, const float *bias2, int splitk,
+                                void *ws, size_t ws_bytes, int flags, void *stream);
 
 int asrk_copy3d_f32(const float *src, float *dst, int n0, int n1, int n2,
                     int64_t s_stride0, int64_t s_stride1, int64_t d_stride0, int64_t d_stride1,
@@ -90,6 +95,7 @@
 size_t asrk_lstm_ws_bytes(void);
 #define ASRK_REC_F32_MFMA 1
 #define ASRK_REC_REARM 2
+#define ASRK_REC_BWD_NO_DG 4
 size_t asrk_lstm_xchg_bytes(int T, int B, int H, int ndir, int backward, int flags);
 int asrk_lstm_plan_workgroups(int T, int B, int H, int ndir, int backward, int flags);
 int asrk_lstm_rec_fwd_f32(float *G, const float *whh_f, const float *whh_r, float *Y, float *C,
```
